# iden3/circom-witnesscalc

Measured on AMD Instinct MI355X. Metric: witnesses/sec, higher is better.
Workload: dtype u32

## Files before the change

circom-witnesscalc_amd/__init__.py:

```python
import ctypes
import os
import subprocess

import numpy as np

_HERE = os.path.dirname(os.path.abspath(__file__))
LIB_PATH = os.environ.get("CWC_LIB_PATH") or os.path.join(_HERE, "libcircom_witnesscalc_amd.so")
_lib = None


class GwStatus(ctypes.Structure):
    _fields_ = [("code", ctypes.c_int), ("error_msg", ctypes.c_void_p)]


class GraphInfo(ctypes.Structure):
    _fields_ = [(n, ctypes.c_uint64) for n in ("n_nodes", "n_op", "n_input_nodes", "n_const", "n_inputs",
                                                "n_witness", "depth", "algorithmic_bytes_per_set")]


class Timing(ctypes.Structure):
    _fields_ = [("tile_width", ctypes.c_uint32), ("n_launches", ctypes.c_uint32), ("n_bundles", ctypes.c_uint64),
                ("n_slots", ctypes.c_uint64), ("interp_ms", ctypes.c_float), ("pack_ms", ctypes.c_float),
                ("divider", ctypes.c_uint32), ("streams", ctypes.c_uint32)]


class ProgramStats(ctypes.Structure):
    _fields_ = [("tile_width", ctypes.c_uint32), ("divider", ctypes.c_uint32), ("streams", ctypes.c_uint32), ("n_classes", ctypes.c_uint32),
                ("n_bundles", ctypes.c_uint64), ("n_fused_nodes", ctypes.c_uint64), ("class_bundles", ctypes.c_uint64 * 16),
                ("class_nodes", ctypes.c_uint64 * 16), ("model_wave_cycles", ctypes.c_double), ("lanes_active_mean", ctypes.c_double),
                ("values_per_bundle_mean", ctypes.c_double), ("chain_floor_cycles", ctypes.c_double), ("n_scan_steps", ctypes.c_uint64), ("n_conv_products", ctypes.c_uint64)]


CLASS_NAMES = ["INPUT", "MUL", "LIN", "DIV", "CMPZ", "CMPS", "BIT", "IDIVMOD", "TERN", "DIVREQ", "DIVGET", "MULQ", "SYNC", "MULF", "SCAN"]


class E2eStats(ctypes.Structure):
    _fields_ = [("n_sets", ctypes.c_size_t), ("sub_batch", ctypes.c_size_t), ("parse_threads", ctypes.c_uint32), ("write_threads", ctypes.c_uint32),
                ("parse_seconds", ctypes.c_double), ("wait_for_drain_seconds", ctypes.c_double), ("total_seconds", ctypes.c_double),
                ("witness_bytes", ctypes.c_uint64), ("failed_sets", ctypes.c_uint64)]


class Handoff(ctypes.Structure):
    _fields_ = [("struct_size", ctypes.c_uint32), ("form", ctypes.c_uint32), ("hip_stream", ctypes.c_void_p), ("done_event", ctypes.c_void_p)]


FORM_CANONICAL, FORM_MONTGOMERY = 0, 1


class WitnessCalcError(RuntimeError):
    pass


def pinned_rows(shape):
    import weakref
    n = int(np.prod(shape))
    ptr = lib().gwb_host_alloc(n)
    if not ptr:
        raise WitnessCalcError("gwb_host_alloc(%d) failed" % n)
    buf = (ctypes.c_uint8 * max(n, 1)).from_address(ptr)
    weakref.finalize(buf, lib().gwb_host_free, ptr)
    return np.frombuffer(buf, dtype=np.uint8, count=n).reshape(shape)


EXPORTED_SYMBOLS = [
    "gw_calc_witness", "gwb_graph_load", "gwb_graph_free", "gwb_graph_info", "gwb_graph_serialize",
    "gwb_inputs_from_json", "gwb_set_tile_width", "gwb_calc_witness_batch_device", "gwb_calc_witness_batch_host",
    "gwb_last_timing", "gwb_wtns_size", "gwb_wtns_from_witness", "gwb_graph_export", "gwb_graph_import",
    "gwb_free_status", "gwb_profile_classes", "gwb_pick_tile_width", "gwb_inputs_from_json_batch", "gwb_wtns_save_batch",
    "gwb_host_alloc", "gwb_host_free", "gwb_timing_history", "gwb_calc_witness_batch_handoff", "gwb_ubench_modmul", "gwb_graph_pick_tile_width", "gwb_graph_broadcast",
    "gwb_builder_new", "gwb_builder_free", "gwb_builder_input", "gwb_builder_constant", "gwb_builder_uno", "gwb_builder_duo", "gwb_builder_tres",
    "gwb_builder_witness", "gwb_builder_input_signal", "gwb_builder_node_count", "gwb_builder_finish",
    "gwb_ubench_modmul_block", "gwb_program_stats", "gwb_calc_witness_json_to_wtns", "gwb_model_class_cycles",
    "gwb_graphgen_bigint_class", "gwb_graphgen_rsa_long_div_class", "gwb_graph_op_histogram",
    "gwb_kernel_source_hash", "gwb_pack_schedule", "gwb_pack_schedule_of_blob", "gwb_rccl_unique_id", "gwb_rccl_comm_init", "gwb_rccl_comm_ranks", "gwb_rccl_comm_destroy",
    "gwb_wave_census",
]


def build(verbose=False, diag=False):
    cmd = ["make", "-C", os.path.join(_HERE, "csrc"), "-j4"] + (["all", "diag"] if diag else [])
    if not verbose:
        cmd.insert(1, "-s")
    subprocess.check_call(cmd)
    subprocess.check_call(["make"] + ([] if verbose else ["-s"]) + ["-C", os.path.join(_HERE, "r1cs"), "-j4"])


DIAG_LIB_PATH = os.path.join(_HERE, "libcircom_witnesscalc_amd_diag.so")


def lib():
    global _lib
    if _lib is None:
        if not os.path.exists(LIB_PATH):
            raise WitnessCalcError("HIP extension %s is missing: run __graft_entry__.build() "
                                   "(there is no CPU fallback)" % LIB_PATH)
        try:
            import torch
        except ImportError:
            pass
        L = ctypes.CDLL(LIB_PATH)
        vp, sz, u32p = ctypes.c_void_p, ctypes.c_size_t, ctypes.POINTER(ctypes.c_uint32)
        stp = ctypes.POINTER(GwStatus)
        L.gw_calc_witness.restype = ctypes.c_int
        L.gw_calc_witness.argtypes = [ctypes.c_char_p, vp, sz, ctypes.POINTER(vp), ctypes.POINTER(sz), stp]
        L.gwb_graph_load.restype = ctypes.c_int
        L.gwb_graph_load.argtypes = [vp, sz, ctypes.POINTER(vp), stp]
        L.gwb_graph_free.argtypes = [vp]
        L.gwb_graph_info.argtypes = [vp, ctypes.POINTER(GraphInfo)]
        L.gwb_graph_serialize.argtypes = [vp, ctypes.POINTER(vp), ctypes.POINTER(sz), stp]
        L.gwb_inputs_from_json.argtypes = [vp, ctypes.c_char_p, vp, stp]
        L.gwb_set_tile_width.argtypes = [vp, ctypes.c_uint32]
        L.gwb_calc_witness_batch_device.argtypes = [vp, vp, sz, vp, vp, vp, stp]
        L.gwb_calc_witness_batch_host.argtypes = [vp, vp, sz, vp, vp, stp]
        L.gwb_last_timing.argtypes = [vp, ctypes.POINTER(Timing)]
        L.gwb_host_alloc.restype = ctypes.c_void_p
        L.gwb_host_alloc.argtypes = [sz]
        L.gwb_host_free.restype = None
        L.gwb_host_free.argtypes = [ctypes.c_void_p]
        L.gwb_timing_history.restype = ctypes.c_int
        L.gwb_timing_history.argtypes = [ctypes.c_void_p, sz, ctypes.c_void_p, ctypes.c_void_p, ctypes.POINTER(sz)]
        L.gwb_wtns_size.restype = sz
        L.gwb_wtns_size.argtypes = [sz]
        L.gwb_wtns_from_witness.argtypes = [vp, sz, vp]
        L.gwb_graph_export.argtypes = [vp, ctypes.c_uint32, ctypes.POINTER(vp), ctypes.POINTER(sz), stp]
        L.gwb_graph_import.argtypes = [vp, sz, ctypes.POINTER(vp), stp]
        L.gwb_free_status.argtypes = [stp]
        if hasattr(L, "gwb_graphgen_bigint_class"):
            L.gwb_graphgen_bigint_class.argtypes = [ctypes.c_uint32, ctypes.c_uint32, ctypes.c_uint32, ctypes.POINTER(vp), ctypes.POINTER(sz), stp]
            L.gwb_graphgen_rsa_long_div_class.argtypes = [ctypes.c_uint32, ctypes.c_uint32, ctypes.c_uint32, ctypes.c_int, ctypes.POINTER(vp), ctypes.POINTER(sz), stp]
            L.gwb_graph_op_histogram.argtypes = [vp, ctypes.POINTER(ctypes.c_uint64), sz]
        L.gwb_profile_classes.argtypes = [vp, vp, sz, vp, vp, vp, stp]
        if hasattr(L, "gwb_wave_census"):
            L.gwb_wave_census.argtypes = [vp, vp, sz, vp, vp, vp, sz, stp]
        L.gwb_inputs_from_json_batch.argtypes = [vp, ctypes.c_char_p, sz, vp, sz, ctypes.POINTER(sz), stp]
        L.gwb_wtns_save_batch.argtypes = [vp, sz, sz, ctypes.c_char_p, stp]
        L.gwb_calc_witness_batch_handoff.argtypes = [vp, vp, sz, vp, vp, ctypes.POINTER(Handoff), stp]
        L.gwb_ubench_modmul.restype = ctypes.c_double
        L.gwb_ubench_modmul.argtypes = [ctypes.c_uint32, ctypes.c_uint32]
        L.gwb_ubench_modmul_block.restype = ctypes.c_double
        L.gwb_model_class_cycles.restype = ctypes.c_double
        L.gwb_kernel_source_hash.restype = ctypes.c_char_p
        L.gwb_kernel_source_hash.argtypes = []
        L.gwb_model_class_cycles.argtypes = [ctypes.c_uint32]
        L.gwb_ubench_modmul_block.argtypes = [ctypes.c_uint32, ctypes.c_uint32]
        L.gwb_program_stats.argtypes = [vp, ctypes.c_uint32, ctypes.POINTER(ProgramStats)]
        if hasattr(L, "gwb_pack_schedule"):
            L.gwb_pack_schedule.argtypes = [vp, ctypes.c_uint32, vp, sz, vp, sz, u32p, u32p, u32p, stp]
            L.gwb_pack_schedule_of_blob.argtypes = [vp, sz, vp, sz, vp, sz, u32p, u32p, u32p, stp]
        L.gwb_calc_witness_json_to_wtns.argtypes = [vp, ctypes.c_char_p, sz, ctypes.c_char_p, sz, ctypes.POINTER(sz), vp, sz, ctypes.POINTER(E2eStats), stp]
        L.gwb_graph_pick_tile_width.restype = ctypes.c_uint32
        L.gwb_graph_pick_tile_width.argtypes = [vp, sz]
        L.gwb_pick_tile_width.restype = ctypes.c_uint32
        L.gwb_pick_tile_width.argtypes = [sz]
        u32 = ctypes.c_uint32
        L.gwb_builder_new.restype = vp
        L.gwb_builder_new.argtypes = []
        L.gwb_builder_free.restype = None
        L.gwb_builder_free.argtypes = [vp]
        for name, args in (("input", [u32]), ("constant", [ctypes.c_char_p, sz]), ("uno", [u32, u32]), ("duo", [u32, u32, u32]), ("tres", [u32, u32, u32, u32])):
            f = getattr(L, "gwb_builder_" + name)
            f.restype = u32
            f.argtypes = [vp] + args
        L.gwb_builder_witness.argtypes = [vp, u32]
        L.gwb_builder_input_signal.argtypes = [vp, ctypes.c_char_p, u32, u32]
        L.gwb_builder_node_count.restype = ctypes.c_uint64
        L.gwb_builder_node_count.argtypes = [vp]
        L.gwb_builder_finish.argtypes = [vp, ctypes.POINTER(vp), ctypes.POINTER(sz), stp]
        _lib = L
    return _lib


_libc = ctypes.CDLL(None)
_libc.free.argtypes = [ctypes.c_void_p]


def _take_status(st):
    msg = ctypes.string_at(st.error_msg).decode("utf-8", "replace") if st.error_msg else ""
    lib().gwb_free_status(ctypes.byref(st))
    return msg


def _check(rc, st):
    msg = _take_status(st)
    if rc != 0:
        raise WitnessCalcError(msg or "call failed")


def wtns_save_batch(witness, path_pattern):
    witness = np.ascontiguousarray(witness, dtype=np.uint8)
    st = GwStatus()
    rc = lib().gwb_wtns_save_batch(witness.ctypes.data, witness.shape[1], witness.shape[0], path_pattern.encode(), ctypes.byref(st))
    _check(rc, st)


def ubench_modmul(waves_per_simd=4, iters=2000, block=False):
    if block:
        return float(lib().gwb_ubench_modmul_block(waves_per_simd, iters))
    return float(lib().gwb_ubench_modmul(waves_per_simd, iters))


def kernel_source_hash():
    return lib().gwb_kernel_source_hash().decode()


def model_cycles():
    return {n: float(lib().gwb_model_class_cycles(c)) for c, n in enumerate(CLASS_NAMES)}


def graphgen_native(kind, **kw):
    out, n, st = ctypes.c_void_p(), ctypes.c_size_t(), GwStatus()
    L = lib()
    if kind == "bigint":
        rc = L.gwb_graphgen_bigint_class(int(kw.get("k", 8)), int(kw.get("n_bits", 64)), int(kw.get("rounds", 4)), ctypes.byref(out), ctypes.byref(n), ctypes.byref(st))
    elif kind == "rsa":
        rc = L.gwb_graphgen_rsa_long_div_class(int(kw.get("n", 121)), int(kw.get("k", 17)), int(kw.get("muls", 2)), 1 if kw.get("range_checks", True) else 0,
                                               ctypes.byref(out), ctypes.byref(n), ctypes.byref(st))
    else:
        raise ValueError(kind)
    _check(rc, st)
    data = ctypes.string_at(out.value, n.value)
    _libc.free(out)
    return data


def pick_tile_width(batch):
    return int(lib().gwb_pick_tile_width(batch))


def calc_witness_wtns(inputs_json, graph_data):
    if isinstance(inputs_json, str):
        inputs_json = inputs_json.encode("utf-8")
    graph_data = bytes(graph_data)
    out, n, st = ctypes.c_void_p(), ctypes.c_size_t(), GwStatus()
    rc = lib().gw_calc_witness(inputs_json, graph_data, len(graph_data), ctypes.byref(out), ctypes.byref(n),
                               ctypes.byref(st))
    _check(rc, st)
    data = ctypes.string_at(out.value, n.value)
    _libc.free(out)
    return data


def calc_witness(inputs_json, graph_data):
    w = calc_witness_wtns(inputs_json, graph_data)
    body = w[76:]
    return [int.from_bytes(body[i:i + 32], "little") for i in range(0, len(body), 32)]


def wtns_from_witness(witness):
    if not isinstance(witness, np.ndarray):
        witness = np.frombuffer(b"".join(int(x).to_bytes(32, "little") for x in witness), dtype=np.uint8)
    witness = np.ascontiguousarray(witness, dtype=np.uint8).reshape(-1, 32)
    n = witness.shape[0]
    out = np.zeros(lib().gwb_wtns_size(n), dtype=np.uint8)
    if lib().gwb_wtns_from_witness(witness.ctypes.data, n, out.ctypes.data) != 0:
        raise WitnessCalcError("gwb_wtns_from_witness failed")
    return out.tobytes()


class Graph:

    def __init__(self, graph_data=None, _handle=None):
        self._h = ctypes.c_void_p()
        if _handle is not None:
            self._h = _handle
        else:
            graph_data = bytes(graph_data)
            st = GwStatus()
            rc = lib().gwb_graph_load(graph_data, len(graph_data), ctypes.byref(self._h), ctypes.byref(st))
            _check(rc, st)
        info = GraphInfo()
        lib().gwb_graph_info(self._h, ctypes.byref(info))
        for name, _ in GraphInfo._fields_:
            setattr(self, name, int(getattr(info, name)))

    def close(self):
        if getattr(self, "_h", None) and _lib is not None:
            _lib.gwb_graph_free(self._h)
            self._h = None

    __del__ = close

    @classmethod
    def from_blob(cls, blob):
        blob = bytes(blob)
        h, st = ctypes.c_void_p(), GwStatus()
        rc = lib().gwb_graph_import(blob, len(blob), ctypes.byref(h), ctypes.byref(st))
        _check(rc, st)
        return cls(_handle=h)

    def op_histogram(self):
        h = (ctypes.c_uint64 * 24)()
        if lib().gwb_graph_op_histogram(self._h, h, 24) != 0:
            raise WitnessCalcError("gwb_graph_op_histogram failed")
        names = ["Mul", "Div", "Add", "Sub", "Pow", "Idiv", "Mod", "Eq", "Neq", "Lt", "Gt", "Leq", "Geq", "Land", "Lor", "Shl", "Shr", "Bor", "Band", "Bxor",
                 "Neg", "TernCond", "Input", "Const"]
        return dict(sorted(((nm, int(h[i])) for i, nm in enumerate(names) if h[i]), key=lambda kv: -kv[1]))

    def export_blob(self, tile_width):
        out, n, st = ctypes.c_void_p(), ctypes.c_size_t(), GwStatus()
        rc = lib().gwb_graph_export(self._h, tile_width, ctypes.byref(out), ctypes.byref(n), ctypes.byref(st))
        _check(rc, st)
        data = ctypes.string_at(out.value, n.value)
        _libc.free(out)
        return data

    def serialize(self):
        out, n, st = ctypes.c_void_p(), ctypes.c_size_t(), GwStatus()
        rc = lib().gwb_graph_serialize(self._h, ctypes.byref(out), ctypes.byref(n), ctypes.byref(st))
        _check(rc, st)
        data = ctypes.string_at(out.value, n.value)
        _libc.free(out)
        return data

    def pick_tile_width(self, batch):
        key = int(lib().gwb_graph_pick_tile_width(self._h, batch))
        if key == 0:
            raise WitnessCalcError("gwb_graph_pick_tile_width failed")
        return key

    def set_tile_width(self, t):
        if lib().gwb_set_tile_width(self._h, t) != 0:
            raise WitnessCalcError("tile width must be 0 or a power of two in 1..64")

    def inputs_from_json(self, inputs_json):
        if isinstance(inputs_json, str):
            inputs_json = inputs_json.encode("utf-8")
        row = np.zeros((self.n_inputs, 32), dtype=np.uint8)
        st = GwStatus()
        rc = lib().gwb_inputs_from_json(self._h, inputs_json, row.ctypes.data, ctypes.byref(st))
        _check(rc, st)
        return row

    def inputs_from_json_batch(self, text):
        if isinstance(text, str):
            text = text.encode("utf-8")
        n = ctypes.c_size_t()
        st = GwStatus()
        lib().gwb_inputs_from_json_batch(self._h, text, len(text), None, 0, ctypes.byref(n), ctypes.byref(st))
        msg = _take_status(st)
        if "rows buffer too small" not in msg and msg:
            raise WitnessCalcError(msg)
        rows = np.zeros((n.value, self.n_inputs, 32), dtype=np.uint8)
        st = GwStatus()
        rc = lib().gwb_inputs_from_json_batch(self._h, text, len(text), rows.ctypes.data, n.value, ctypes.byref(n), ctypes.byref(st))
        _check(rc, st)
        return rows

    def json_to_wtns(self, text, path_pattern, first_index=0, with_status=True):
        if isinstance(text, str):
            text = text.encode("utf-8")
        n = ctypes.c_size_t()
        cap = max(1, text.count(b"\n") + 1, text.count(b"{"))
        status = np.zeros(cap, dtype=np.uint32)
        es, st = E2eStats(), GwStatus()
        rc = lib().gwb_calc_witness_json_to_wtns(self._h, text, len(text), path_pattern.encode(), first_index, ctypes.byref(n),
                                                  status.ctypes.data if with_status else None, cap if with_status else 0,
                                                  ctypes.byref(es), ctypes.byref(st))
        _check(rc, st)
        return status[:n.value], {k: getattr(es, k) for k, _ in E2eStats._fields_}

    def calc_witness_batch(self, inputs, out=None):
        inputs = np.ascontiguousarray(inputs, dtype=np.uint8)
        b = inputs.shape[0]
        assert inputs.shape[1:] == (self.n_inputs, 32), inputs.shape
        if out is None:
            wit = np.empty((b, self.n_witness, 32), dtype=np.uint8)
        else:
            wit = out
            assert wit.dtype == np.uint8 and wit.shape == (b, self.n_witness, 32) and wit.flags["C_CONTIGUOUS"]
        status = np.zeros(b, dtype=np.uint32)
        st = GwStatus()
        rc = lib().gwb_calc_witness_batch_host(self._h, inputs.ctypes.data, b, wit.ctypes.data, status.ctypes.data,
                                               ctypes.byref(st))
        _check(rc, st)
        return wit, status

    def calc_witness_batch_device(self, d_inputs, d_witness, d_status, stream=None, montgomery=False, done_event=None):
        import torch
        b = d_inputs.shape[0]
        assert d_inputs.is_cuda and d_witness.is_cuda and d_status.is_cuda
        assert d_inputs.is_contiguous() and d_witness.is_contiguous() and d_status.is_contiguous()
        assert tuple(d_inputs.shape[1:]) == (self.n_inputs, 32) and tuple(d_witness.shape) == (b, self.n_witness, 32)
        s = stream if stream is not None else torch.cuda.current_stream()
        st = GwStatus()
        if montgomery or done_event is not None:
            if done_event is not None:
                done_event.record(s)
            h = Handoff(ctypes.sizeof(Handoff), FORM_MONTGOMERY if montgomery else FORM_CANONICAL, s.cuda_stream,
                        done_event.cuda_event if done_event is not None else None)
            rc = lib().gwb_calc_witness_batch_handoff(self._h, d_inputs.data_ptr(), b, d_witness.data_ptr(), d_status.data_ptr(),
                                                      ctypes.byref(h), ctypes.byref(st))
        else:
            rc = lib().gwb_calc_witness_batch_device(self._h, d_inputs.data_ptr(), b, d_witness.data_ptr(),
                                                     d_status.data_ptr(), s.cuda_stream, ctypes.byref(st))
        _check(rc, st)

    def timing_history(self, max_launches):
        a = np.zeros(max_launches, dtype=np.float32)
        b = np.zeros(max_launches, dtype=np.float32)
        n = ctypes.c_size_t(0)
        if lib().gwb_timing_history(self._h, max_launches, a.ctypes.data, b.ctypes.data, ctypes.byref(n)) != 0:
            raise WitnessCalcError("gwb_timing_history failed")
        return a[:n.value], b[:n.value]

    def profile_classes(self, d_inputs, d_witness, d_status):
        out = np.zeros(96, dtype=np.uint64)
        st = GwStatus()
        rc = lib().gwb_profile_classes(self._h, d_inputs.data_ptr(), d_inputs.shape[0], d_witness.data_ptr(),
                                       d_status.data_ptr(), out.ctypes.data, ctypes.byref(st))
        _check(rc, st)
        names = ["INPUT", "MUL", "LIN", "DIV", "CMPZ", "CMPS", "BIT", "IDIVMOD", "TERN", "DIVREQ", "DIVGET", "MULQ"]
        res = {n: tuple(int(x) for x in out[4 * i:4 * i + 4]) for i, n in enumerate(names)}
        res["MULF"] = tuple(int(x) for x in out[64:68])
        res["SCAN"] = tuple(int(x) for x in out[68:72])
        res["_scan_kinds"] = {k: tuple(int(x) for x in out[72 + 4 * i:76 + 4 * i]) for i, k in enumerate(("carry", "division", "convolution", "borrow", "comparison"))}
        res["_sections"] = {"MUL": tuple(int(x) for x in out[48:54]), "LIN": tuple(int(x) for x in out[56:62])}
        res["_issue_part"] = {"MUL": int(out[92]), "LIN": int(out[93])}
        res["_pack"] = {"cycles": int(out[94]), "passes": int(out[95])}
        n = int(out[63])
        res["_waves"] = {"n": n, "max_cycles": int(out[54]), "min_cycles": (1 << 40) - int(out[55]) if n else 0,
                         "mean_cycles": int(out[62]) // n if n else 0}
        return res

    def wave_census(self, d_inputs, d_witness, d_status):
        out = np.zeros(3 * 8192, dtype=np.uint64)
        st = GwStatus()
        rc = lib().gwb_wave_census(self._h, d_inputs.data_ptr(), d_inputs.shape[0], d_witness.data_ptr(),
                                   d_status.data_ptr(), out.ctypes.data, out.size, ctypes.byref(st))
        _check(rc, st)
        rec = out.reshape(-1, 3)
        idx = [i for i in range(rec.shape[0]) if rec[i, 1]]
        res = []
        for i in idx:
            w0 = int(rec[i, 0])
            role, wpw = (w0 >> 40) & 255, (w0 >> 48) & 255
            res.append({"workgroup": i // wpw, "wave": i % wpw, "xcc": (w0 >> 32) & 15, "se": (w0 >> 13) & 7, "sh": (w0 >> 12) & 1, "cu": (w0 >> 8) & 15, "simd": (w0 >> 4) & 3,
                        "divider": role & 1, "stream": (role >> 1) & 7, "has_tile": (role >> 4) & 1, "start": int(rec[i, 1]), "end": int(rec[i, 2])})
        return res

    def program_stats(self, key=0):
        ps = ProgramStats()
        if lib().gwb_program_stats(self._h, key, ctypes.byref(ps)) != 0:
            raise WitnessCalcError("gwb_program_stats: no such program")
        n = ps.n_classes
        return {"tile_width": ps.tile_width, "divider": ps.divider, "streams": ps.streams, "n_bundles": ps.n_bundles,
                "n_fused_nodes": ps.n_fused_nodes, "n_scan_steps": ps.n_scan_steps, "n_conv_products": ps.n_conv_products, "chain_floor_cycles": ps.chain_floor_cycles, "model_wave_cycles": ps.model_wave_cycles, "lanes_active_mean": ps.lanes_active_mean, "values_per_bundle_mean": ps.values_per_bundle_mean,
                "class_bundles": {CLASS_NAMES[c]: int(ps.class_bundles[c]) for c in range(n) if ps.class_bundles[c]},
                "class_nodes": {CLASS_NAMES[c]: int(ps.class_nodes[c]) for c in range(n) if ps.class_nodes[c]}}

    def pack_schedule(self, key):
        return _pack_schedule(lambda *a: lib().gwb_pack_schedule(self._h, key, *a))

    def last_timing(self):
        t = Timing()
        if lib().gwb_last_timing(self._h, ctypes.byref(t)) != 0:
            raise WitnessCalcError("gwb_last_timing failed")
        return {n: getattr(t, n) for n, _ in Timing._fields_}


def _pack_schedule(call):
    nw, nr, ni, st = ctypes.c_uint32(), ctypes.c_uint32(), ctypes.c_uint32(), GwStatus()
    _check(call(None, 0, None, 0, ctypes.byref(nw), ctypes.byref(nr), ctypes.byref(ni), ctypes.byref(st)), st)
    order, ready = np.zeros(nw.value, dtype=np.uint32), np.zeros(nr.value, dtype=np.uint32)
    _check(call(order.ctypes.data, order.size, ready.ctypes.data, ready.size, ctypes.byref(nw), ctypes.byref(nr), ctypes.byref(ni), ctypes.byref(st)), st)
    return order, ready, int(ni.value)


def pack_schedule_of_blob(blob):
    blob = bytes(blob)
    return _pack_schedule(lambda *a: lib().gwb_pack_schedule_of_blob(blob, len(blob), *a))


R1CS_LIB_PATH = os.environ.get("CWC_R1CS_LIB_PATH") or os.path.join(_HERE, "libcwc_r1cs.so")
R1CS_SATISFIED = 0xFFFFFFFF
_r1cs_lib = None


class R1csInfo(ctypes.Structure):
    _fields_ = [(n, ctypes.c_uint32) for n in ("n_wires", "n_pub_out", "n_pub_in", "n_prv_in", "n_constraints")] + \
               [(n, ctypes.c_uint64) for n in ("n_labels", "n_factors_a", "n_factors_b", "n_factors_c")]


class R1csQapInfo(ctypes.Structure):
    _fields_ = [("n_rows", ctypes.c_uint64), ("domain_power", ctypes.c_uint32), ("domain_size", ctypes.c_uint64),
                ("workspace_bytes_per_row", ctypes.c_uint64)]


class ZkeyInfo(ctypes.Structure):
    _fields_ = [("n_vars", ctypes.c_uint32), ("n_public", ctypes.c_uint32), ("domain_size", ctypes.c_uint32), ("n_coefs", ctypes.c_uint64)]


class PtauInfo(ctypes.Structure):
    _fields_ = [("power", ctypes.c_uint32), ("ceremony_power", ctypes.c_uint32), ("prepared", ctypes.c_uint32),
                ("n_contributions", ctypes.c_uint32)]


def r1cs_lib():
    global _r1cs_lib
    if _r1cs_lib is None:
        if not os.path.exists(R1CS_LIB_PATH):
            raise WitnessCalcError("R1CS library %s is missing: run __graft_entry__.build()" % R1CS_LIB_PATH)
        try:
            import torch
        except ImportError:
            pass
        L = ctypes.CDLL(R1CS_LIB_PATH)
        vp, sz, u32 = ctypes.c_void_p, ctypes.c_size_t, ctypes.c_uint32
        stp = ctypes.POINTER(GwStatus)
        L.gwb_r1cs_load.argtypes = [vp, sz, ctypes.POINTER(vp), stp]
        L.gwb_r1cs_free.restype = None
        L.gwb_r1cs_free.argtypes = [vp]
        L.gwb_r1cs_info.argtypes = [vp, ctypes.POINTER(R1csInfo)]
        L.gwb_r1cs_set_tile_width.argtypes = [vp, u32]
        L.gwb_r1cs_check_batch_device.argtypes = [vp, vp, sz, sz, u32, vp, vp, vp, stp]
        L.gwb_r1cs_check_batch_host.argtypes = [vp, vp, sz, sz, vp, vp, stp]
        L.gwb_r1cs_check_wtns.argtypes = [vp, vp, sz, vp, vp, stp]
        L.gwb_r1cs_qap_info.argtypes = [vp, ctypes.POINTER(R1csQapInfo), stp]
        L.gwb_r1cs_qap_batch_device.argtypes = [vp, vp, sz, sz, u32, vp, u32, vp, stp]
        L.gwb_r1cs_qap_batch_host.argtypes = [vp, vp, sz, sz, vp, u32, stp]
        L.gwb_r1cs_qap_wtns.argtypes = [vp, vp, sz, vp, u32, stp]
        L.gwb_r1cs_qap_time_phases.argtypes = [vp, ctypes.c_int]
        L.gwb_r1cs_qap_phase_ms.argtypes = [vp, ctypes.POINTER(ctypes.c_float)]
        L.gwb_r1cs_modmul_rate.argtypes = [ctypes.POINTER(ctypes.c_double)]
        L.gwb_zkey_load.argtypes = [vp, sz, ctypes.POINTER(vp), stp]
        L.gwb_zkey_free.restype = None
        L.gwb_zkey_free.argtypes = [vp]
        L.gwb_zkey_info.argtypes = [vp, ctypes.POINTER(ZkeyInfo)]
        L.gwb_groth16_prove_batch_device.argtypes = [vp, vp, vp, sz, sz, u32, vp, vp, vp, stp]
        L.gwb_groth16_prove_batch_host.argtypes = [vp, vp, vp, sz, sz, vp, vp, stp]
        L.gwb_groth16_prove_wtns.argtypes = [vp, vp, vp, sz, vp, vp, stp]
        L.gwb_groth16_time_phases.argtypes = [vp, ctypes.c_int]
        L.gwb_groth16_phase_ms.argtypes = [vp, ctypes.POINTER(ctypes.c_float)]
        L.gwb_zkey_qap_info.argtypes = [vp, ctypes.POINTER(R1csQapInfo), stp]
        L.gwb_zkey_qap_batch_device.argtypes = [vp, vp, sz, sz, u32, vp, u32, vp, stp]
        L.gwb_zkey_qap_batch_host.argtypes = [vp, vp, sz, sz, vp, u32, stp]
        L.gwb_zkey_set_tile_width.argtypes = [vp, u32]
        L.gwb_zkey_check_r1cs.argtypes = [vp, vp, stp]
        L.gwb_g16vk_from_zkey.argtypes = [vp, ctypes.POINTER(vp), stp]
        L.gwb_g16vk_load.argtypes = [vp, sz, u32, ctypes.POINTER(vp), stp]
        L.gwb_g16vk_info.argtypes = [vp, ctypes.POINTER(ctypes.c_uint32)]
        L.gwb_g16vk_points.argtypes = [vp, vp, sz]
        L.gwb_g16vk_alphabeta.argtypes = [vp, vp, stp]
        L.gwb_g16vk_free.restype = None
        L.gwb_g16vk_free.argtypes = [vp]
        L.gwb_groth16_verify_batch_device.argtypes = [vp, vp, vp, sz, sz, vp, vp, stp]
        L.gwb_groth16_verify_batch_host.argtypes = [vp, vp, vp, sz, sz, vp, stp]
        L.gwb_bn254_pairing_batch_device.argtypes = [vp, vp, sz, vp, vp, stp]
        L.gwb_groth16_setup.argtypes = [vp, vp, ctypes.POINTER(vp), ctypes.POINTER(sz), stp]
        L.gwb_groth16_setup_free.restype = None
        L.gwb_groth16_setup_free.argtypes = [vp]
        L.gwb_bn254_gen_mul_batch_device.argtypes = [vp, sz, u32, vp, vp, stp]
        L.gwb_groth16_setup_phase_ms.argtypes = [ctypes.POINTER(ctypes.c_float)]
        L.gwb_ptau_info.argtypes = [vp, sz, ctypes.POINTER(PtauInfo), stp]
        L.gwb_ptau_check.argtypes = [vp, sz, u32, u32, stp]
        L.gwb_groth16_setup_ptau.argtypes = [vp, vp, sz, vp, u32, ctypes.POINTER(vp), ctypes.POINTER(sz), stp]
        L.gwb_bn254_point_idft_batch_device.argtypes = [vp, u32, u32, vp, vp, stp]
        L.gwb_groth16_setup_ptau_phase_ms.argtypes = [ctypes.POINTER(ctypes.c_float)]
        L.gwb_bn254_g2_check_batch_device.argtypes = [vp, sz, u32, u32, vp, vp, stp]
        L.gwb_zkey_check_g2.argtypes = [vp, stp]
        L.gwb_zkey_check_wtns.argtypes = [vp, vp, sz, stp]
        L.gwb_ptau_check_g2.argtypes = [vp, sz, u32, u32, stp]
        L.gwb_groth16_contribute.argtypes = [vp, sz, ctypes.c_char_p, vp, ctypes.POINTER(vp), ctypes.POINTER(sz), vp, stp]
        L.gwb_groth16_contribute_phase_ms.argtypes = [ctypes.POINTER(ctypes.c_float)]
        L.gwb_zkey_verify_contributions.argtypes = [vp, sz, vp, ctypes.POINTER(sz), stp]
        L.gwb_zkey_verify_step.argtypes = [vp, sz, vp, sz, vp, stp]
        L.gwb_zkey_contributions.argtypes = [vp, sz, ctypes.POINTER(vp), ctypes.POINTER(sz), stp]
        L.gwb_blake2b512.restype = None
        L.gwb_blake2b512.argtypes = [vp, sz, vp]
        L.gwb_zkey_contribution_challenge.restype = None
        L.gwb_zkey_contribution_challenge.argtypes = [vp, vp]
        L.gwb_bn254_g1_scale_batch_device.argtypes = [vp, sz, vp, vp, vp, stp]
        L.gwb_bn254_g1_lincomb128_device.argtypes = [vp, vp, sz, vp, vp, stp]
        _r1cs_lib = L
    return _r1cs_lib


def _r1cs_check(rc, st):
    msg = ctypes.string_at(st.error_msg).decode("utf-8", "replace") if st.error_msg else ""
    if st.error_msg:
        _libc.free(st.error_msg)
    if rc != 0:
        raise WitnessCalcError(msg or "call failed")


def modmul_rate():
    rate = ctypes.c_double()
    if r1cs_lib().gwb_r1cs_modmul_rate(ctypes.byref(rate)) != 0:
        raise WitnessCalcError("gwb_r1cs_modmul_rate failed")
    return rate.value


def _qap_info(h, src):
    info = R1csQapInfo()
    st = GwStatus()
    rc = getattr(r1cs_lib(), "gwb_%s_qap_info" % src)(h, ctypes.byref(info), ctypes.byref(st))
    _r1cs_check(rc, st)
    return {n: int(getattr(info, n)) for n, _ in R1csQapInfo._fields_}


def _qap_batch(h, src, witness_rows, montgomery_out):
    if isinstance(witness_rows, tuple):
        witness_rows = witness_rows[0]
    w = np.ascontiguousarray(witness_rows, dtype=np.uint8)
    assert w.ndim == 3 and w.shape[2] == 32, w.shape
    b = w.shape[0]
    out = np.zeros((b, _qap_info(h, src)["domain_size"], 32), dtype=np.uint8)
    st = GwStatus()
    rc = getattr(r1cs_lib(), "gwb_%s_qap_batch_host" % src)(h, w.ctypes.data, w.shape[1], b, out.ctypes.data,
                                                            FORM_MONTGOMERY if montgomery_out else FORM_CANONICAL, ctypes.byref(st))
    _r1cs_check(rc, st)
    return out


def _qap_batch_device(h, src, d_witness, stream, montgomery, montgomery_out):
    import torch
    assert d_witness.is_cuda and d_witness.is_contiguous() and d_witness.dtype == torch.uint8
    assert d_witness.dim() == 3 and d_witness.shape[2] == 32, tuple(d_witness.shape)
    b = d_witness.shape[0]
    n = _qap_info(h, src)["domain_size"]
    s = stream if stream is not None else torch.cuda.current_stream(d_witness.device)
    out = torch.empty((b, n, 32), dtype=torch.uint8, device=d_witness.device)
    st = GwStatus()
    with torch.cuda.device(d_witness.device):
        rc = getattr(r1cs_lib(), "gwb_%s_qap_batch_device" % src)(h, d_witness.data_ptr(), d_witness.shape[1], b,
                                                                  FORM_MONTGOMERY if montgomery else FORM_CANONICAL, out.data_ptr(),
                                                                  FORM_MONTGOMERY if montgomery_out else FORM_CANONICAL, s.cuda_stream,
                                                                  ctypes.byref(st))
    _r1cs_check(rc, st)
    if b:
        out.record_stream(s)
    return out


class R1cs:

    def __init__(self, data):
        self._h = ctypes.c_void_p()
        data = bytes(data)
        st = GwStatus()
        rc = r1cs_lib().gwb_r1cs_load(data, len(data), ctypes.byref(self._h), ctypes.byref(st))
        _r1cs_check(rc, st)
        info = R1csInfo()
        r1cs_lib().gwb_r1cs_info(self._h, ctypes.byref(info))
        self.info = {n: int(getattr(info, n)) for n, _ in R1csInfo._fields_}

    def close(self):
        if getattr(self, "_h", None) and _r1cs_lib is not None:
            _r1cs_lib.gwb_r1cs_free(self._h)
            self._h = None

    __del__ = close

    def set_tile_width(self, t):
        if r1cs_lib().gwb_r1cs_set_tile_width(self._h, t) != 0:
            raise WitnessCalcError("tile width must be 0 or a power of two in 1..64")

    def check_batch(self, witness_rows):
        if isinstance(witness_rows, tuple):
            witness_rows = witness_rows[0]
        w = np.ascontiguousarray(witness_rows, dtype=np.uint8)
        assert w.ndim == 3 and w.shape[2] == 32, w.shape
        b = w.shape[0]
        first = np.zeros(b, dtype=np.uint32)
        nfail = np.zeros(b, dtype=np.uint32)
        st = GwStatus()
        rc = r1cs_lib().gwb_r1cs_check_batch_host(self._h, w.ctypes.data, w.shape[1], b, first.ctypes.data, nfail.ctypes.data, ctypes.byref(st))
        _r1cs_check(rc, st)
        return first, nfail

    def check_batch_device(self, d_witness, stream=None, montgomery=False):
        import torch
        assert d_witness.is_cuda and d_witness.is_contiguous() and d_witness.dtype == torch.uint8
        assert d_witness.dim() == 3 and d_witness.shape[2] == 32, tuple(d_witness.shape)
        b = d_witness.shape[0]
        s = stream if stream is not None else torch.cuda.current_stream(d_witness.device)
        first = torch.empty(b, dtype=torch.int32, device=d_witness.device)
        nfail = torch.empty(b, dtype=torch.int32, device=d_witness.device)
        st = GwStatus()
        with torch.cuda.device(d_witness.device):
            rc = r1cs_lib().gwb_r1cs_check_batch_device(self._h, d_witness.data_ptr(), d_witness.shape[1], b,
                                                        FORM_MONTGOMERY if montgomery else FORM_CANONICAL, first.data_ptr(),
                                                        nfail.data_ptr(), s.cuda_stream, ctypes.byref(st))
        _r1cs_check(rc, st)
        return first, nfail

    def check_wtns(self, wtns):
        wtns = bytes(wtns)
        first, nfail = ctypes.c_uint32(), ctypes.c_uint32()
        st = GwStatus()
        rc = r1cs_lib().gwb_r1cs_check_wtns(self._h, wtns, len(wtns), ctypes.byref(first), ctypes.byref(nfail), ctypes.byref(st))
        _r1cs_check(rc, st)
        return int(first.value), int(nfail.value)

    def qap_info(self):
        return _qap_info(self._h, "r1cs")

    def qap_batch(self, witness_rows, montgomery_out=False):
        return _qap_batch(self._h, "r1cs", witness_rows, montgomery_out)

    def qap_batch_device(self, d_witness, stream=None, montgomery=False, montgomery_out=False):
        return _qap_batch_device(self._h, "r1cs", d_witness, stream, montgomery, montgomery_out)

    def qap_time_phases(self, on=True):
        if r1cs_lib().gwb_r1cs_qap_time_phases(self._h, 1 if on else 0) != 0:
            raise WitnessCalcError("gwb_r1cs_qap_time_phases failed")

    def qap_phase_ms(self):
        ms = (ctypes.c_float * 4)()
        if r1cs_lib().gwb_r1cs_qap_phase_ms(self._h, ms) != 0:
            raise WitnessCalcError("no QAP phase times (qap_time_phases not on, or no QAP call yet)")
        return dict(zip(("evaluation", "inverse_outer", "fused_inner", "forward_outer"), (float(x) for x in ms)))

    def qap_wtns(self, wtns, montgomery_out=False):
        wtns = bytes(wtns)
        h = np.zeros((self.qap_info()["domain_size"], 32), dtype=np.uint8)
        st = GwStatus()
        rc = r1cs_lib().gwb_r1cs_qap_wtns(self._h, wtns, len(wtns), h.ctypes.data,
                                          FORM_MONTGOMERY if montgomery_out else FORM_CANONICAL, ctypes.byref(st))
        _r1cs_check(rc, st)
        return h



GROTH16_PROOF_BYTES = 256
GROTH16_PHASES = ("witness_map", "scalars_sort", "g1_msms", "g2_msm", "assembly")


def _rs_array(rs, b):
    if rs is None:
        return None
    if isinstance(rs, np.ndarray):
        a = np.ascontiguousarray(rs, dtype=np.uint8)
    else:
        a = np.frombuffer(b"".join(int(x).to_bytes(32, "little") for pair in rs for x in pair), dtype=np.uint8).copy()
    assert a.size == b * 64, "rs must hold [batch][2][32 B]"
    return a


def _dec(b):
    return str(int.from_bytes(bytes(b), "little"))


def proof_json(proof):
    p = bytes(proof)
    c = [_dec(p[32 * k:32 * k + 32]) for k in range(8)]
    z = lambda lo, hi: "1" if any(p[lo:hi]) else "0"
    return {"pi_a": [c[0], c[1], z(0, 64)], "pi_b": [[c[2], c[3]], [c[4], c[5]], [z(64, 192), "0"]],
            "pi_c": [c[6], c[7], z(192, 256)], "protocol": "groth16", "curve": "bn128"}


class Groth16:

    def __init__(self, zkey_bytes, r1cs=None, check_g2=False):
        self._h = ctypes.c_void_p()
# ... 596 lines not shown
```

circom-witnesscalc_amd/csrc/kernels.hip:

```cpp
#include <hip/hip_runtime.h>
#include <stdlib.h>

#include "fr_gfx950.hpp"
#include "scan_gfx950.hpp"
#include "program_dev.h"

namespace cwc {

__device__ __forceinline__ Fr fr_from_u4(const uint4& lo, const uint4& hi) {
    return Fr{{lo.x, lo.y, lo.z, lo.w, hi.x, hi.y, hi.z, hi.w}};
}

__device__ __forceinline__ bool wave_any(bool p) { return __ballot(p) != 0ull; }

struct InterpDims {
    uint32_t n_bundles, n_slots, n_inputs, batch, n_const, n_div_requests, trash_off;
    const uint32_t* div_lanes;
    uint32_t n_streams, stream_first[MAX_STREAMS], stream_count[MAX_STREAMS], stream_div_requests[MAX_STREAMS], stream_cref_first[MAX_STREAMS];
    uint4* pack_out;
    const uint2* pack_entries;
    const uint32_t* pack_ready;
    uint32_t n_inline, pack_mont, n_witness;
};
static const uint32_t ST_DIVIDER_TIMEOUT = 0x80000000u;
static const uint32_t ST_SYNC_TIMEOUT = 0x40000000u;

__device__ __forceinline__ bool mbox_wait(const volatile uint32_t* seq, uint32_t need) {
    for (uint32_t spins = 0; spins < (1u << 22); ++spins) {
        if (*seq >= need) return true;
        __builtin_amdgcn_s_sleep(8);
    }
    return false;
}
__device__ __noinline__ bool post_wait(uint32_t* word, uint32_t need) {
#pragma nounroll
    for (uint32_t spins = 0; spins < (1u << 22); ++spins) {
        if (__hip_atomic_load(word, __ATOMIC_ACQUIRE, __HIP_MEMORY_SCOPE_AGENT) >= need) return true;
        __builtin_amdgcn_s_sleep(8);
    }
    return false;
}
typedef uint32_t u32x4 __attribute__((ext_vector_type(4)));
typedef int i32x4 __attribute__((ext_vector_type(4)));
typedef __attribute__((address_space(3))) char lds_char;

__device__ __forceinline__ void dma16(uint32_t lds_addr, uint32_t voff, const i32x4& rsrc, uint32_t soff) {
    asm volatile("s_mov_b32 m0, %0\n\ts_nop 0\n\tbuffer_load_dwordx4 %1, %2, %3 offen lds"
                 :: "s"(lds_addr), "v"(voff), "s"(rsrc), "s"(soff) : "memory");
}
__device__ __forceinline__ i32x4 make_rsrc_words(const void* base, uint32_t bytes) {
    const uint64_t a = (uint64_t)base;
    return i32x4{(int)(uint32_t)a, (int)((uint32_t)(a >> 32) & 0xffffu), (int)bytes, 0x00020000};
}

template <int T, bool PROF, int W, int PACK, int MODE = 0>
__global__ __launch_bounds__((W > 0 ? (W + 1) * PACK : PACK) * 64) void interp_kernel(const uint32_t* __restrict__ hdr, const uint4* __restrict__ recs,
                                                    const uint32_t* __restrict__ crefs, InterpDims p, WsTable wst,
                                                    const uint4* __restrict__ inputs, uint32_t* __restrict__ status,
                                                    unsigned long long* __restrict__ prof) {
    constexpr int G = 64 / T;
    constexpr bool M2 = MODE == 2 || MODE == 3, WIDE = MODE == 3;
    constexpr uint32_t HI = 16u * T;
    constexpr bool DIVIDER = W > 0;
    constexpr uint32_t NW = (W > 0 ? (uint32_t)W : 1u) * (uint32_t)PACK;
    constexpr uint32_t WD = W > 0 ? (uint32_t)W : 1u;
    constexpr uint32_t AREA = lds_area_bytes((uint32_t)W, LDS_BYTES);
    constexpr uint32_t ML = mbox_lanes((uint32_t)W), MB = mbox_bytes((uint32_t)W);
    const uint32_t batch = p.batch;
    const uint32_t lane = threadIdx.x & 63u;
    const uint32_t wave = (uint32_t)__builtin_amdgcn_readfirstlane((int)(threadIdx.x >> 6));
    const uint32_t n_tiles = (batch + T - 1) / T;
    const uint32_t t = lane % T;
    const uint32_t j = (G == 1) ? 0u : lane / T;
    const uint32_t NS = p.n_streams;
    const uint32_t stream = wave < NW ? wave % NS : 0u;
    const uint32_t tile_raw = blockIdx.x * (NW / NS) + (wave < NW ? wave : 0u) / NS;
    const uint32_t tile = tile_raw < n_tiles ? tile_raw : n_tiles - 1;
    const uint32_t set = tile * T + t;
    const uint32_t set_c = set < batch ? set : batch - 1;
    [[maybe_unused]] auto census_slot = [&]() -> unsigned long long* {
        const uint32_t wv = blockIdx.x * (blockDim.x >> 6) + wave;
        return lane == 0 && wv < CENSUS_MAX_WAVES ? prof + PROF_WORDS + CENSUS_WORDS * wv : nullptr;
    };
    if constexpr (PROF) {
        if (unsigned long long* c = census_slot()) {
            const uint32_t w_of = wave < NW ? wave : (wave - NW) * WD;
            const uint32_t has_tile = blockIdx.x * (NW / NS) + w_of / NS < n_tiles ? 1u : 0u;
            const unsigned long long role = (wave >= NW ? 1u : 0u) | (w_of % NS) << 1 | has_tile << 4 | (blockDim.x >> 6) << 8;
            constexpr int HWREG_HW_ID = 4 | 31 << 11, HWREG_XCC_ID = 20 | 31 << 11;
            c[0] = (unsigned long long)__builtin_amdgcn_s_getreg(HWREG_HW_ID) | (unsigned long long)(__builtin_amdgcn_s_getreg(HWREG_XCC_ID) & 15u) << 32 | role << 40;
            c[1] = __builtin_amdgcn_s_memtime();
        }
    }
    const uint64_t tile_bytes = ws_tile_bytes(p.n_const, p.n_slots, T);
    const uint32_t chunk = tile / wst.tiles_per_chunk, tile_in_chunk = tile % wst.tiles_per_chunk;
    char* tile_base = reinterpret_cast<char*>(wst.base[chunk]) + (uint64_t)tile_in_chunk * tile_bytes;
    const __amdgpu_buffer_rsrc_t rsrc = __builtin_amdgcn_make_buffer_rsrc(tile_base, 0, (int)(uint32_t)tile_bytes, 0x00020000);
    const i32x4 rsrc_rec = make_rsrc_words(recs, (p.n_bundles + REC_AHEAD) * (uint32_t)G * 16u);
    uint32_t* const sync_words = reinterpret_cast<uint32_t*>(tile_base + ws_sync_offset(p.n_const, p.n_slots, T));
    static_assert(NW + PACK <= 16, "sequence words: 64 bytes");
    __shared__ uint4 lds[(NW * AREA + (DIVIDER ? NW * MB + 64u : 0u)) / 16];
    const uint32_t area = wave * AREA;
    const uint32_t lds0 = (uint32_t)(uintptr_t)(lds_char*)(char*)lds + area;
    const uint32_t t16 = 16u * t, lane16 = 16u * lane, j16 = 16u * j;
    char* const ldsb = reinterpret_cast<char*>(lds) + area;
    char* const mbox_all = reinterpret_cast<char*>(lds) + NW * AREA;
    char* const mbox = mbox_all + (wave < NW ? wave : 0u) * MB;
    volatile uint32_t* const seq = reinterpret_cast<volatile uint32_t*>(mbox_all + NW * MB);
    if (DIVIDER || NW > 1) {
        if (DIVIDER && threadIdx.x < NW + (uint32_t)PACK) seq[threadIdx.x] = 0;
        if (NS > 1 && wave < NW && stream == 0 && lane < MAX_STREAMS && tile_raw < n_tiles) {
            __hip_atomic_store(sync_words + lane, 0u, __ATOMIC_RELAXED, __HIP_MEMORY_SCOPE_AGENT);
            __builtin_amdgcn_fence(__ATOMIC_RELEASE, "agent");
        }
        if (wave < NW && stream == 0 && j == 0 && tile_raw < n_tiles && set < batch) status[set] = 0;
        __syncthreads();
    } else {
        if (j == 0 && tile_raw < n_tiles && set < batch) status[set] = 0;
    }
    if (DIVIDER) {
        if (wave >= NW) {
            const uint32_t first_w = (wave - NW) * WD, first_tile = blockIdx.x * (NW / NS) + first_w / NS;
            if (first_tile >= n_tiles) return;
            const uint32_t n_active = NS > 1 ? 1u : n_tiles - first_tile < WD ? n_tiles - first_tile : WD;
            char* const mbox_d = mbox_all + first_w * MB;
            const uint32_t n_requests = NS > 1 ? p.stream_div_requests[first_w % NS] : p.n_div_requests;
            uint32_t div_lanes_base = 0;
            for (uint32_t q = 0; NS > 1 && q < first_w % NS; ++q) div_lanes_base += p.stream_div_requests[q];
            [[maybe_unused]] uint32_t pk_next = 0;
            [[maybe_unused]] uint2 pk_e0 = make_uint2(0u, 0u), pk_e1 = pk_e0;
            [[maybe_unused]] unsigned long long pk_cycles = 0, pk_passes = 0;
            const bool inl = W == 1 && NS == 1 && p.n_inline > 0;
            const char* const pk_tile = reinterpret_cast<const char*>(wst.base[first_tile / wst.tiles_per_chunk]) + (uint64_t)(first_tile % wst.tiles_per_chunk) * tile_bytes;
            const uint32_t pk_set = first_tile * T + t;
            auto pk_load = [&](const uint2& e, uint4& lo, uint4& hi) {
                const uint32_t ref = e.y & ~REF_CANON;
                const uint32_t slot = (ref & REF_CONST) ? (ref & ~REF_CONST) : p.n_const + ref;
                const uint4* q = reinterpret_cast<const uint4*>(pk_tile) + (size_t)slot * (2 * T);
                lo = q[t];
                hi = q[T + t];
            };
            auto pk_store = [&](const uint2& e, const uint4& lo, const uint4& hi, uint32_t limit) {
                const bool valid = pk_next + j < limit && pk_set < batch, canon = (e.y & REF_CANON) != 0;
                const Fr v = fr_from_u4(lo, hi);
                Fr c = v;
                if (p.pack_mont) {
                    if (wave_any(both(valid, canon))) c = u256_select(canon, fr_mul(v, fr_r2()), v);
                } else {
                    if (wave_any(both(valid, !canon))) c = u256_select(canon, v, fr_from_mont(v));
                }
                if (valid) {
                    uint4* o = p.pack_out + ((size_t)pk_set * p.n_witness + e.x) * 2;
                    o[0] = make_uint4(c.v[0], c.v[1], c.v[2], c.v[3]);
                    o[1] = make_uint4(c.v[4], c.v[5], c.v[6], c.v[7]);
                }
            };
            auto pk_run = [&](uint32_t limit, uint32_t need) {
                if (pk_next >= limit) return;
                unsigned long long t0 = 0;
                if (PROF) t0 = __builtin_amdgcn_s_memtime();
                uint4 lo, hi;
                pk_load(pk_e0, lo, hi);
                for (;;) {
                    const uint32_t nb = pk_next + (uint32_t)G;
                    const bool more = nb < limit && seq[first_w] < need;
                    uint4 lo1 = lo, hi1 = hi;
                    if (more) pk_load(pk_e1, lo1, hi1);
                    const uint2 e2 = p.pack_entries[nb + (uint32_t)G + j];
                    pk_store(pk_e0, lo, hi, limit);
                    pk_next = nb;
                    pk_e0 = pk_e1;
                    pk_e1 = e2;
                    if (PROF) ++pk_passes;
                    if (!more) break;
                    lo = lo1;
                    hi = hi1;
                }
                if (PROF) pk_cycles += __builtin_amdgcn_s_memtime() - t0;
            };
            if constexpr (W == 1) {
                if (inl) {
                    pk_e0 = p.pack_entries[j];
                    pk_e1 = p.pack_entries[(uint32_t)G + j];
                }
            }
            for (uint32_t k = 0; k < n_requests; ++k) {
                if constexpr (W == 1) {
                    if (inl) {
                        const uint32_t lim = p.pack_ready[k] < p.n_inline ? p.pack_ready[k] : p.n_inline;
                        pk_run(lim / (uint32_t)G * (uint32_t)G, k + 1);
                    }
                }
                bool ok = true;
                for (uint32_t w = 0; w < n_active; ++w) ok = ok && mbox_wait(seq + first_w + w, k + 1);
                if (!ok) {
                    if (first_tile * T + t < batch) atomicOr(&status[first_tile * T + t], ST_DIVIDER_TIMEOUT);
                    break;
                }
                __builtin_amdgcn_fence(__ATOMIC_ACQUIRE, "workgroup");
                const uint32_t lanes_k = p.div_lanes[div_lanes_base + k];
                const uint32_t total = n_active * lanes_k;
                for (uint32_t g0 = 0; g0 < total; g0 += 64u) {
                    const uint32_t g = g0 + lane;
                    const bool valid = g < total;
                    const uint32_t w = valid ? g / lanes_k : 0u, i = valid ? g % lanes_k : 0u;
                    char* mb = mbox_d + w * MB + 16u * i;
                    const uint4* qa = reinterpret_cast<const uint4*>(mb);
                    const uint4* qb = reinterpret_cast<const uint4*>(mb + 32u * ML);
                    Fr a = fr_from_u4(qa[0], qa[ML]), b = fr_from_u4(qb[0], qb[ML]);
                    if (!valid) b = fr_zero();
                    const Fr inv = fr_inv(b);
                    const Fr r = u256_select(u256_is_zero(b), fr_zero(), fr_mul(a, inv));
                    if (valid) {
                        uint4* qr = reinterpret_cast<uint4*>(mb);
                        qr[0] = make_uint4(r.v[0], r.v[1], r.v[2], r.v[3]);
                        qr[ML] = make_uint4(r.v[4], r.v[5], r.v[6], r.v[7]);
                    }
                }
                __builtin_amdgcn_fence(__ATOMIC_RELEASE, "workgroup");
                if (lane == 0) seq[wave] = k + 1;
            }
            if constexpr (W == 1) {
                if (inl) {
                    pk_run(p.pack_ready[n_requests] < p.n_inline ? p.pack_ready[n_requests] : p.n_inline, 0xffffffffu);
                    if (PROF && lane == 0 && first_tile % 64u == 0) {
                        atomicAdd(&prof[94], pk_cycles);
                        atomicAdd(&prof[95], pk_passes);
                    }
                }
            }
            if constexpr (PROF) {
                if (unsigned long long* c = census_slot()) c[2] = __builtin_amdgcn_s_memtime();
            }
            return;
        }
    }
    if (tile_raw >= n_tiles) return;
    uint32_t div_seq = 0;
    uint32_t n_posts = 0, n_waits = 0;
    uint32_t cref_row = p.stream_cref_first[stream];

    auto ld = [&](uint32_t off) -> Fr {
        const u32x4 lo = __builtin_amdgcn_raw_buffer_load_b128(rsrc, (int)off, 0, 0);
        const u32x4 hi = __builtin_amdgcn_raw_buffer_load_b128(rsrc, (int)off + (int)HI, 0, 0);
        return Fr{{lo.x, lo.y, lo.z, lo.w, hi.x, hi.y, hi.z, hi.w}};
    };
    auto ld_lds = [&](uint32_t addr) -> Fr {
        const uint4* q = reinterpret_cast<const uint4*>(ldsb + addr);
        const uint4 lo = q[0], hi = q[LDS_HALF_BYTES / 16];
        return fr_from_u4(lo, hi);
    };
    auto ld_rec2 = [&](uint32_t bundle, uint32_t half) -> uint2 {
        return *reinterpret_cast<const uint2*>(ldsb + LDS_REC_OFF + (bundle % REC_AHEAD) * REC_BYTES + lane16 + 8u * half);
    };
    const uint32_t B0 = p.stream_first[stream], NBND = B0 + p.stream_count[stream];
    if (NBND == B0) return;
    auto clampb = [&](uint32_t b) { return b < NBND ? b : NBND - 1; };
    auto stage_rec = [&](uint32_t bundle) {
        dma16(lds0 + LDS_REC_OFF + (bundle % REC_AHEAD) * REC_BYTES, j16, rsrc_rec, bundle * (uint32_t)G * 16u);
    };
    constexpr uint32_t DMA_BIAS = 3u * LDS_HALF_BYTES;
    const i32x4 rsrc_dma = make_rsrc_words(tile_base - DMA_BIAS, (uint32_t)tile_bytes + DMA_BIAS);
    const uint32_t dma_soff0 = DMA_BIAS, dma_soff1 = DMA_BIAS + HI - LDS_HALF_BYTES, dma_soff2 = DMA_BIAS - 2u * LDS_HALF_BYTES,
                   dma_soff3 = DMA_BIAS + HI - 3u * LDS_HALF_BYTES;
    static_assert(LDS_HALF_BYTES == 1024, "instruction offsets below are written out");
    auto stage_operands = [&](uint32_t bundle, const uint2& offs) {
        const uint32_t s = lds0 + LDS_STAGE_OFF + (bundle % OPND_AHEAD) * STAGE_BYTES;
        const uint32_t ao = offs.x + t16, bo = offs.y + t16;
        asm volatile("s_mov_b32 m0, %0\n\ts_nop 0\n\t"
                     "buffer_load_dwordx4 %1, %3, %4 offen lds\n\t"
                     "buffer_load_dwordx4 %1, %3, %5 offen offset:1024 lds\n\t"
                     "buffer_load_dwordx4 %2, %3, %6 offen offset:2048 lds\n\t"
                     "buffer_load_dwordx4 %2, %3, %7 offen offset:3072 lds"
                     :: "s"(s), "v"(ao), "v"(bo), "s"(rsrc_dma), "s"(dma_soff0), "s"(dma_soff1), "s"(dma_soff2), "s"(dma_soff3) : "memory");
    };
    uint32_t err_bits = 0;
    Fr pv = fr_p();
#pragma unroll
    for (int i = 0; i < 8; ++i) asm volatile("" : "+v"(pv.v[i]));
    constexpr bool COOP = (uint32_t)T <= COOP_MAX_T;
    const uint32_t cq = lane & 3u, cv = lane >> 2;
    const uint32_t t16c = 16u * (cv % T);
    const uint32_t coop_chunk = (cq >> 1) * LDS_HALF_BYTES + (cq & 1u) * 8u;
    const uint32_t coop_ring_off = 16u * cv + coop_chunk;
    const uint32_t coop_dst_off = t16c + (cq >> 1) * HI + (cq & 1u) * 8u;
    uint32_t nq0 = cq == 0 ? CWC_P0 : cq == 1 ? CWC_P2 : cq == 2 ? CWC_P4 : CWC_P6;
    uint32_t nq1 = cq == 0 ? CWC_P1 : cq == 1 ? CWC_P3 : cq == 2 ? CWC_P5 : CWC_P7;
    asm volatile("" : "+v"(nq0), "+v"(nq1));
    const uint32_t trash_doff = p.trash_off | t16;
    constexpr int C_PROF = 12;
    unsigned long long pf[C_PROF][2], psec[2][7] = {{0, 0, 0, 0, 0, 0, 0}, {0, 0, 0, 0, 0, 0, 0}};
    unsigned long long pf_fused[2] = {0, 0};
    unsigned long long pf_scan[5][2] = {{0, 0}, {0, 0}, {0, 0}, {0, 0}, {0, 0}};
    if (PROF) {
#pragma unroll
        for (int c = 0; c < C_PROF; ++c) pf[c][0] = pf[c][1] = 0;
    }
#define CWC_STAMP(var) unsigned long long var = 0; if (PROF) asm volatile("s_memtime %0\n\ts_waitcnt lgkmcnt(0)" : "=s"(var)::"memory")
#define CWC_SHADOW_ISSUE()                                                                                                                  \
    stage_rec(b + 4);                                                                                                                       \
    __builtin_amdgcn_raw_buffer_store_b128(u32x4{r_prev.v[0], r_prev.v[1], r_prev.v[2], r_prev.v[3]}, rsrc, (int)doff_prev, 0, 0);          \
    __builtin_amdgcn_raw_buffer_store_b128(u32x4{r_prev.v[4], r_prev.v[5], r_prev.v[6], r_prev.v[7]}, rsrc, (int)doff_prev + (int)HI, 0, 0)
#define CWC_NEXT_HEADER(var)                                                                                                                 \
    asm volatile("s_mov_b32 %0, xnack_mask_lo\n\ts_load_dword xnack_mask_lo, %1, %2" : "=&s"(var) : "s"(hdr), "s"(hdr_off_n2) : "memory"); \
    hdr_off_n2 += 4u

    static_assert(OPND_AHEAD == 2 && REC_AHEAD == 4, "the counted waits below are written for this pipeline depth");
#pragma unroll
    for (uint32_t q = 0; q < REC_AHEAD; ++q) stage_rec(B0 + q);
    asm volatile("s_waitcnt vmcnt(0)" ::: "memory");
    stage_operands(B0, ld_rec2(B0, 0));
    stage_operands(B0 + 1, ld_rec2(B0 + 1, 0));
    uint2 rec_hi = ld_rec2(B0, 1);
    uint2 rec_hi_n1 = ld_rec2(B0 + 1, 1);
    uint32_t h_cur = hdr[B0], h_n1 = hdr[clampb(B0 + 1)];
    asm volatile("s_waitcnt vmcnt(0)" ::: "memory");
    const unsigned long long t_wave0 = PROF ? __builtin_amdgcn_s_memtime() : 0ull;
    asm volatile("s_load_dword xnack_mask_lo, %0, %1\n\ts_waitcnt lgkmcnt(0)" :: "s"(hdr), "s"(4u * B0 + 8u) : "memory");
    uint32_t hdr_off_n2 = 4u * B0 + 12u;
    Fr r_prev = fr_zero();
    uint32_t doff_prev = trash_doff;
    for (uint32_t b = B0; b < NBND; ++b) {
        CWC_STAMP(st0);
        const uint32_t h = h_cur;
        asm volatile("s_waitcnt vmcnt(7)" ::: "memory");
        CWC_STAMP(st1);
        if constexpr (COOP) {
            uint32_t cls_q = h & HDR_CLASS_MASK;
            asm volatile("" : "+s"(cls_q));
            static_assert(C_MULQ == 11 && C_SYNC == 12 && C_MULF == 13 && C_SCAN == 14 && C_COUNT == 15, "one compare (class >= C_MULQ) leads to the narrow classes");
            const bool narrow_cls = MODE == 1 ? cls_q >= C_MULQ : cls_q == C_MULQ;
            if (M2 ? __builtin_expect(narrow_cls, 0) : narrow_cls) {
            if (MODE != 1 || cls_q == C_MULQ) {
                const uint32_t la = rec_hi.y + (t16c | (t16c << 16));
                const Fr a_op = ld_lds(la & 0xffffu);
                const uint2 bq = *reinterpret_cast<const uint2*>(ldsb + (la >> 16) + coop_chunk);
                const uint2 aq = *reinterpret_cast<const uint2*>(ldsb + (la & 0xffffu) + coop_chunk);
                const uint4 rec_full_n2 = *reinterpret_cast<const uint4*>(ldsb + LDS_REC_OFF + ((b + 2) % REC_AHEAD) * REC_BYTES + lane16);
                const uint2 rec_n2 = make_uint2(rec_full_n2.x, rec_full_n2.y), rec_hi_n2 = make_uint2(rec_full_n2.z, rec_full_n2.w);
                CWC_SHADOW_ISSUE();
                asm volatile("s_waitcnt lgkmcnt(0)" :: "v"(a_op.v[0]), "v"(a_op.v[4]), "v"(bq.x), "v"(aq.x), "v"(rec_n2.x), "v"(rec_hi_n2.x) : "memory");
                uint32_t h_n2;
                CWC_NEXT_HEADER(h_n2);
                CWC_STAMP(st2);
                stage_operands(b + 2, rec_n2);
                CWC_STAMP(st3);
                uint32_t out[2];
                if (h & (HDR_LIN_ADD | HDR_LIN_SUB)) {
                    fr_mul_coop4r(a_op, aq.x, aq.y, bq.x, bq.y, nq0, nq1, rec_hi.x & CTRL_SUB_MASK, out);
                } else {
                    fr_mul_coop4(a_op, bq.x, bq.y, nq0, nq1, out);
                }
                CWC_STAMP(st4);
                *reinterpret_cast<uint2*>(ldsb + LDS_RING_OFF + (b % RING_BUNDLES) * RING_SLOT_BYTES + coop_ring_off) = make_uint2(out[0], out[1]);
                {
                    typedef uint32_t u32x2 __attribute__((ext_vector_type(2)));
                    __builtin_amdgcn_raw_buffer_store_b64(u32x2{out[0], out[1]}, rsrc, (int)((rec_hi.x & ~CTRL_MASK) + coop_dst_off), 0, 0);
                }
                doff_prev = trash_doff;
                rec_hi = rec_hi_n1;
                rec_hi_n1 = rec_hi_n2;
                h_cur = h_n1;
                h_n1 = h_n2;
                __builtin_amdgcn_fence(__ATOMIC_ACQ_REL, "wavefront");
                if (PROF) {
                    asm volatile("s_waitcnt lgkmcnt(0)" ::: "memory");
                    const unsigned long long t_now = __builtin_amdgcn_s_memtime();
                    pf[C_MULQ][0] += t_now - st0;
                    pf[C_MULQ][1] += 1;
                    (void)st2; (void)st3; (void)st4;
                }
                continue;
            }
            if constexpr (MODE == 1 && (uint32_t)T <= COOP_FUSE_MAX_T) {
            if (cls_q == C_MULF) {
                constexpr int QP_MAIN = T == 1 ? 0xA0  : 0x00 , QP_EXTRA = T == 1 ? 0xF5  : 0xAA ;
                const uint32_t mx = (uint32_t)__builtin_amdgcn_mov_dpp((int)rec_hi.x, QP_MAIN, 0xf, 0xf, false);
                const uint32_t my = (uint32_t)__builtin_amdgcn_mov_dpp((int)rec_hi.y, QP_MAIN, 0xf, 0xf, false);
                const uint32_t xx = (uint32_t)__builtin_amdgcn_mov_dpp((int)rec_hi.x, QP_EXTRA, 0xf, 0xf, false);
                const uint32_t xy = (uint32_t)__builtin_amdgcn_mov_dpp((int)rec_hi.y, QP_EXTRA, 0xf, 0xf, false);
                const uint32_t la = my + (t16c | (t16c << 16)), lx = xy + (t16c | (t16c << 16));
                const Fr a_op = ld_lds(la & 0xffffu);
                const uint2 bq = *reinterpret_cast<const uint2*>(ldsb + (la >> 16) + coop_chunk);
                const Fr x2_full = ld_lds(lx & 0xffffu);
                const uint2 x2q = *reinterpret_cast<const uint2*>(ldsb + (lx & 0xffffu) + coop_chunk);
                const uint2 x3q = *reinterpret_cast<const uint2*>(ldsb + (lx >> 16) + coop_chunk);
                const uint4 rec_full_n2 = *reinterpret_cast<const uint4*>(ldsb + LDS_REC_OFF + ((b + 2) % REC_AHEAD) * REC_BYTES + lane16);
                const uint2 rec_n2 = make_uint2(rec_full_n2.x, rec_full_n2.y), rec_hi_n2 = make_uint2(rec_full_n2.z, rec_full_n2.w);
                CWC_SHADOW_ISSUE();
                asm volatile("s_waitcnt lgkmcnt(0)" :: "v"(a_op.v[0]), "v"(a_op.v[4]), "v"(bq.x), "v"(x2_full.v[0]), "v"(x2_full.v[4]), "v"(x2q.x), "v"(x3q.x), "v"(rec_n2.x), "v"(rec_hi_n2.x) : "memory");
                uint32_t h_n2;
                CWC_NEXT_HEADER(h_n2);
                stage_operands(b + 2, rec_n2);
                uint32_t out[2];
                fr_mul_coop4(a_op, bq.x, bq.y, nq0, nq1, out);
                const uint32_t op2 = mx & CTRL_SUB_MASK, op3 = xx & CTRL_SUB_MASK;
                if (h & HDR_F_S2MUL) {
                    uint32_t o2[2];
                    fr_mul_coop4(x2_full, out[0], out[1], nq0, nq1, o2);
                    out[0] = op2 == FOP_MUL ? o2[0] : out[0];
                    out[1] = op2 == FOP_MUL ? o2[1] : out[1];
                }
                auto lin_stage = [&](uint32_t op, const uint2& xq) {
                    const bool rs = op == FOP_RSUB;
                    uint32_t o[2];
                    fr_addsub_coop4(rs ? xq.x : out[0], rs ? xq.y : out[1], rs ? out[0] : xq.x, rs ? out[1] : xq.y, nq0, nq1, op == FOP_ADD ? 0u : 1u, o);
                    out[0] = op >= FOP_ADD ? o[0] : out[0];
                    out[1] = op >= FOP_ADD ? o[1] : out[1];
                };
                if (h & HDR_F_S2LIN) lin_stage(op2, x2q);
                if (h & HDR_F_S3LIN) lin_stage(op3, x3q);
                *reinterpret_cast<uint2*>(ldsb + LDS_RING_OFF + (b % RING_BUNDLES) * RING_SLOT_BYTES + coop_ring_off) = make_uint2(out[0], out[1]);
                {
// ... 374 lines not shown
                        ds.v[0] |= dz ? 1u : 0u;
                        const bool small = !wave_any((x.v[2] | x.v[3] | x.v[4] | x.v[5] | x.v[6] | x.v[7] | acc0.v[2] | acc0.v[3] | acc0.v[4] | acc0.v[5] | acc0.v[6] | acc0.v[7] |
                                                      d.v[2] | d.v[3] | d.v[4] | d.v[5] | d.v[6] | d.v[7]) != 0u) && sh >= 1u && sh <= 64u;
                        Fr quo = fr_zero(), rem = fr_zero();
                        if (small) {
                            const uint64_t dv = ((uint64_t)ds.v[1] << 32) | ds.v[0];
                            const uint32_t s = clz64_nonzero(dv);
                            const uint64_t dn = dv << s, rv = recip64(dn);
                            const uint64_t xl = ((uint64_t)x.v[1] << 32) | x.v[0];
                            const uint64_t a0 = ((uint64_t)acc0.v[1] << 32) | acc0.v[0];
                            uint64_t r64 = 0, qh = 0, ql = 0;
                            const bool seg = start || !active;
                            const uint64_t d_prev = ((uint64_t)wave_shr_lanes<D>((uint32_t)(dv >> 32)) << 32) | wave_shr_lanes<D>((uint32_t)dv);
                            if (sh == 64u && iters > 2u && !wave_any(both(active, either(dz, start ? a0 >= dv : dv != d_prev)))) {
                                scan_div_parallel<T>(seg, lane, iters, active ? dv : 1ull, active ? xl : 0ull, active ? a0 : 0ull, ql, r64);
                            } else if (sh == 64u) {
                                const uint64_t xn = xl << s, xh = (xl >> 1) >> (63u - s);
                                for (uint32_t it = 0; it < iters; ++it) {
                                    const uint32_t s0 = wave_shr_lanes<D>((uint32_t)r64), s1 = wave_shr_lanes<D>((uint32_t)(r64 >> 32));
                                    const uint64_t in = start ? a0 : (((uint64_t)s1 << 32) | s0);
                                    uint64_t q_h = 0, q_l, rr;
                                    if (wave_any(in >= dv)) {
                                        u128_divrem_64_recip(in, xl, dv, s, dn, rv, true, q_h, q_l, rr);
                                    } else {
                                        uint64_t rn;
                                        div2by1((in << s) | xh, xn, dn, rv, q_l, rn);
                                        rr = rn >> s;
                                    }
                                    qh = dz ? 0ull : q_h;
                                    ql = dz ? 0ull : q_l;
                                    r64 = dz ? 0ull : rr;
                                }
                            } else {
                                for (uint32_t it = 0; it < iters; ++it) {
                                    const uint32_t s0 = wave_shr_lanes<D>((uint32_t)r64), s1 = wave_shr_lanes<D>((uint32_t)(r64 >> 32));
                                    const uint64_t in = start ? a0 : (((uint64_t)s1 << 32) | s0);
                                    const uint64_t lo = in << sh, hi = (in >> 1) >> (63u - sh);
                                    const uint64_t tl = lo + xl, th = hi + (tl < lo ? 1ull : 0ull);
                                    uint64_t q_h, q_l, rr;
                                    u128_divrem_64_recip(th, tl, dv, s, dn, rv, wave_any(th >= dv), q_h, q_l, rr);
                                    qh = dz ? 0ull : q_h;
                                    ql = dz ? 0ull : q_l;
                                    r64 = dz ? 0ull : rr;
                                }
                            }
                            quo.v[0] = (uint32_t)ql; quo.v[1] = (uint32_t)(ql >> 32); quo.v[2] = (uint32_t)qh; quo.v[3] = (uint32_t)(qh >> 32);
                            rem.v[0] = (uint32_t)r64; rem.v[1] = (uint32_t)(r64 >> 32);
                        } else {
                            for (uint32_t it = 0; it < iters; ++it) {
                                Fr in;
#pragma unroll
                                for (int k = 0; k < 8; ++k) {
                                    const uint32_t sft = wave_shr_lanes<D>(rem.v[k]);
                                    in.v[k] = start ? acc0.v[k] : sft;
                                }
                                const Fr t = fr_add_wave(fr_mul_wave(in, bm, pv), x, pv);
                                const uint32_t lx = u256_bitlen(t), ly = u256_bitlen(ds);
                                const uint32_t my_dig = lx >= ly ? (lx - ly + 32u) >> 5 : 0u;
                                uint32_t dig = 0;
#pragma unroll
                                for (uint32_t dd = 1; dd <= 8; ++dd) dig = wave_any(my_dig >= dd) ? dd : dig;
                                Fr q1, r1;
                                u256_divrem_digits(q1, r1, t, ds, dig, ly);
                                quo = u256_select(dz, fr_zero(), q1);
                                rem = u256_select(dz, fr_zero(), r1);
                            }
                        }
                        r = u256_select(role_acc, rem, quo);
                    }
                }
                finish(r);
                continue;
            }
        }
        switch (cls) {
            case C_INPUT: {
                const uint32_t idx = crefs[(size_t)cref_row * G + j];
                ++cref_row;
                const uint4* q = inputs + ((size_t)set_c * p.n_inputs + idx) * 2;
                r = fr_mul_wave(fr_from_u4(q[0], q[1]), (h & HDR_OUT_CANON) ? fr_one() : fr_r2(), pv);
                break;
            }
            case C_DIVREQ: {
                if (DIVIDER) {
                    if (lane < ML) {
                        uint4* qa = reinterpret_cast<uint4*>(mbox + lane16);
                        uint4* qb = reinterpret_cast<uint4*>(mbox + 32u * ML + lane16);
                        qa[0] = make_uint4(a_op.v[0], a_op.v[1], a_op.v[2], a_op.v[3]);
                        qa[ML] = make_uint4(a_op.v[4], a_op.v[5], a_op.v[6], a_op.v[7]);
                        qb[0] = make_uint4(b_op.v[0], b_op.v[1], b_op.v[2], b_op.v[3]);
                        qb[ML] = make_uint4(b_op.v[4], b_op.v[5], b_op.v[6], b_op.v[7]);
                    }
                    __builtin_amdgcn_fence(__ATOMIC_RELEASE, "workgroup");
                    if (lane == 0) seq[wave] = div_seq + 1;
                }
                r = fr_zero();
                break;
            }
            case C_DIVGET: {
                r = fr_zero();
                if (DIVIDER) {
                    ++div_seq;
                    if (!mbox_wait(seq + NW + wave / WD, div_seq)) err_bits |= ST_DIVIDER_TIMEOUT;
                    __builtin_amdgcn_fence(__ATOMIC_ACQUIRE, "workgroup");
                    if (lane < ML) {
                        const uint4* qr = reinterpret_cast<const uint4*>(mbox + lane16);
                        r = fr_from_u4(qr[0], qr[ML]);
                    }
                }
                break;
            }
            case C_DIV: {
                const Fr inv = fr_inv(b_op);
                r = u256_select(u256_is_zero(b_op), fr_zero(), fr_mul(a_op, inv));
                break;
            }
            case C_CMPZ: {
                const bool az = u256_is_zero(a_op), cz = u256_is_zero(b_op), eq = u256_eq(a_op, b_op);
                const bool v = either(either(both(sub == SUB_EQ, eq), both(sub == SUB_NEQ, !eq)), either(both(sub == SUB_LAND, !either(az, cz)), both(both(sub != SUB_EQ, both(sub != SUB_NEQ, sub != SUB_LAND)), !both(az, cz))));
                r = u256_select(v, one_out(), fr_zero());
                break;
            }
            case C_CMPS: {
                const Fr x = (h & HDR_A_CANON) ? a_op : fr_from_mont(a_op), y = (h & HDR_B_CANON) ? b_op : fr_from_mont(b_op);
                auto less = [](const Fr& a, const Fr& b) {
                    Fr t;
                    const uint32_t borrow = u256_sub(t, a, b);
                    if constexpr (M2) asm volatile("" ::"v"(t.v[7]));
                    return borrow != 0;
                };
                bool lt, gt;
                bool limb_sized = false;
                if constexpr (M2) limb_sized = !wave_any(both(active, (x.v[4] | x.v[5] | x.v[6] | x.v[7] | y.v[4] | y.v[5] | y.v[6] | y.v[7]) != 0u));
                if (M2 && limb_sized) {
                    uint32_t d[4], bw = 0;
#pragma unroll
                    for (int k = 0; k < 4; ++k) d[k] = sbb32(x.v[k], y.v[k], bw);
                    lt = bw != 0u;
                    gt = both(bw == 0u, (d[0] | d[1] | d[2] | d[3]) != 0u);
                } else {
                    const bool xn = less(fr_half(), x), yn = less(fr_half(), y);
                    const bool same = xn == yn, xy = less(x, y), yx = less(y, x);
                    lt = same ? xy : xn;
                    gt = same ? yx : yn;
                }
                const bool v = either(either(both(sub == SUB_LT, lt), both(sub == SUB_GT, gt)), either(both(sub == SUB_LEQ, !gt), both(both(sub != SUB_LT, both(sub != SUB_GT, sub != SUB_LEQ)), !lt)));
                r = u256_select(v, one_out(), fr_zero());
                break;
            }
            case C_BIT: {
                const Fr x = (h & HDR_A_CANON) ? a_op : fr_from_mont(a_op);
                const uint32_t kx = rec_hi.y >> 20;
                const bool is_x = sub == SUB_BITX;
                if (h & HDR_BITX_ALL) {
                    const Fr e = u256_shr(x, kx);
                    r = u256_select((e.v[0] & 1u) != 0u, one_out(), fr_zero());
                    break;
                }
                const Fr y = (h & HDR_B_CANON) ? b_op : fr_from_mont(b_op);
                auto bit_result = [&](const Fr& d) -> Fr {
                    if (h & HDR_OUT_CANON) return d;
                    const bool small = both(d.v[0] < 2u, (d.v[1] | d.v[2] | d.v[3] | d.v[4] | d.v[5] | d.v[6] | d.v[7]) == 0u);
                    if (wave_any(!small)) return fr_mul_wave(d, fr_r2(), pv);
                    return u256_select(d.v[0] != 0u, fr_one(), fr_zero());
                };
                if (h & (HDR_BIT_ALL_SHR | HDR_BIT_ALL_BAND)) {
                    Fr d;
#pragma unroll
                    for (int i = 0; i < 8; ++i) d.v[i] = x.v[i] & y.v[i];
                    if (h & HDR_BIT_ALL_SHR) {
                        const bool big = either((y.v[1] | y.v[2] | y.v[3] | y.v[4] | y.v[5] | y.v[6] | y.v[7]) != 0u, y.v[0] >= 254u);
                        const Fr sh = u256_select(big, fr_zero(), u256_shr(x, big ? 0u : y.v[0]));
                        d = u256_select(sub == SUB_SHR, sh, d);
                    }
                    r = bit_result(d);
                    break;
                }
                uint32_t hi_or = 0;
#pragma unroll
                for (int i = 1; i < 8; ++i) hi_or |= y.v[i];
                const bool big = either(hi_or != 0u, y.v[0] >= 254u);
                const uint32_t n = is_x ? kx : big ? 0u : y.v[0];
                const bool shifts = either(either(sub == SUB_SHL, sub == SUB_SHR), is_x);
                Fr d = u256_shr(x, n);
                if (wave_any(sub == SUB_SHL)) d = u256_select(sub == SUB_SHL, u256_shl(x, n), d);
                d = u256_select(both(big, !is_x), fr_zero(), d);
                d.v[0] &= is_x ? 1u : 0xffffffffu;
#pragma unroll
                for (int i = 1; i < 8; ++i) d.v[i] = is_x ? 0u : d.v[i];
                {
                    const bool over = both(sub == SUB_SHL, !u256_lt(d, fr_p()));
                    err_bits |= both(over, active) ? ST_SHL_OVERFLOW : 0u;
                    d = u256_select(over, fr_zero(), d);
                }
                {
                    const uint32_t m_and = sub == SUB_BAND ? 0xffffffffu : 0u, m_or = sub == SUB_BAND ? 0u : 0xffffffffu, m_xor = (sub == SUB_BAND || sub == SUB_BOR) ? 0u : 0xffffffffu;
                    Fr e;
#pragma unroll
                    for (int i = 0; i < 8; ++i) {
                        const uint32_t a = x.v[i] & y.v[i], o = x.v[i] | y.v[i];
                        e.v[i] = (a & m_and) | ((o & m_or) & ~(a & m_xor));
                    }
                    Fr em;
                    const uint32_t br = u256_sub(em, e, fr_p());
                    err_bits |= both(both(br == 0u, u256_is_zero(em)), both(active, !shifts)) ? ST_BITOP_EQ_R : 0u;
                    e = u256_select(br == 0u, em, e);
                    d = u256_select(shifts, d, e);
                }
                r = bit_result(d);
                break;
            }
            case C_IDIVMOD: {
                const Fr x = (h & HDR_A_CANON) ? a_op : fr_from_mont(a_op), y = (h & HDR_B_CANON) ? b_op : fr_from_mont(b_op);
                const bool yz = u256_is_zero(y);
                Fr ys = y;
                ys.v[0] |= yz ? 1u : 0u;
                Fr q, rem;
                bool two_words = false;
                if constexpr (WIDE) two_words = !wave_any(both(both(active, !yz), either((ys.v[2] | ys.v[3]) == 0u, (ys.v[4] | ys.v[5] | ys.v[6] | ys.v[7]) != 0u)));
                if (!wave_any((x.v[4] | x.v[5] | x.v[6] | x.v[7] | ys.v[2] | ys.v[3] | ys.v[4] | ys.v[5] | ys.v[6] | ys.v[7]) != 0u)) {
                    u128_divrem_64(q, rem, x, ys);
                } else if (WIDE && two_words) {
                    const bool sub = either(yz, !active);
                    Fr yy = ys;
                    yy.v[0] = sub ? 0u : ys.v[0];
                    yy.v[1] = sub ? 0u : ys.v[1];
                    yy.v[2] = sub ? 1u : ys.v[2];
                    yy.v[3] = sub ? 0u : ys.v[3];
#pragma unroll
                    for (int k = 4; k < 8; ++k) yy.v[k] = 0u;
                    u256_divrem_128(q, rem, x, yy);
                } else {
                    const uint32_t lx = u256_bitlen(x), ly = u256_bitlen(ys);
                    const uint32_t my_dig = lx >= ly ? (lx - ly + 32u) >> 5 : 0u;
                    uint32_t dig = 0;
#pragma unroll
                    for (uint32_t dd = 1; dd <= 8; ++dd) dig = wave_any(my_dig >= dd) ? dd : dig;
                    u256_divrem_digits(q, rem, x, ys, dig, ly);
                }
                const Fr d = u256_select(yz, fr_zero(), u256_select(sub == SUB_IDIV, q, rem));
                r = (h & HDR_OUT_CANON) ? d : fr_mul_wave(d, fr_r2(), pv);
                break;
            }
            case C_TERN: {
                const uint32_t cr = crefs[(size_t)cref_row * G + j];
                ++cref_row;
                const Fr y = ld(cr + t16);
                r = u256_select(u256_is_zero(a_op), y, b_op);
                break;
            }
            case C_SYNC: {
                r = fr_zero();
                if (h & HDR_POST) {
                    asm volatile("s_waitcnt vmcnt(0)" ::: "memory");
                    ++n_posts;
                    if (lane == 0) __hip_atomic_store(sync_words + stream, n_posts, __ATOMIC_RELEASE, __HIP_MEMORY_SCOPE_AGENT);
                }
                if (h & HDR_WAIT) {
                    ++n_waits;
                    if (!post_wait(sync_words, n_waits)) err_bits |= ST_SYNC_TIMEOUT;
                }
                break;
            }
            case C_SCAN: r = fr_zero(); break;
            default: r = fr_zero(); break;
        }
        finish(r);
    }
    __builtin_amdgcn_raw_buffer_store_b128(u32x4{r_prev.v[0], r_prev.v[1], r_prev.v[2], r_prev.v[3]}, rsrc, (int)doff_prev, 0, 0);
    __builtin_amdgcn_raw_buffer_store_b128(u32x4{r_prev.v[4], r_prev.v[5], r_prev.v[6], r_prev.v[7]}, rsrc, (int)doff_prev + (int)HI, 0, 0);
    if (PROF && lane == 0) {
        const unsigned long long cyc = __builtin_amdgcn_s_memtime() - t_wave0;
        atomicMax(&prof[54], cyc);
        atomicMax(&prof[55], (1ull << 40) - cyc);
        atomicAdd(&prof[62], cyc);
        atomicAdd(&prof[63], 1ull);
    }
    if constexpr (PROF) {
        if (unsigned long long* c = census_slot()) c[2] = __builtin_amdgcn_s_memtime();
    }
    if (PROF && lane == 0 && (tile % 64u) == 0u) {
#pragma unroll
        for (int c = 0; c < C_PROF; ++c) {
            atomicAdd(&prof[c * 4 + 0], pf[c][0]);
            atomicAdd(&prof[c * 4 + 3], pf[c][1]);
        }
        atomicAdd(&prof[M2 ? 68 : 64], pf_fused[0]);
        atomicAdd(&prof[M2 ? 71 : 67], pf_fused[1]);
        if (M2) {
#pragma unroll
            for (int q = 0; q < 5; ++q) {
                atomicAdd(&prof[72 + 4 * q], pf_scan[q][0]);
                atomicAdd(&prof[75 + 4 * q], pf_scan[q][1]);
            }
        }
#pragma unroll
        for (int k = 0; k < 2; ++k)
#pragma unroll
            for (int q = 0; q < 6; ++q) atomicAdd(&prof[48 + 8 * k + q], psec[k][q]);
        atomicAdd(&prof[92], psec[0][6]);
        atomicAdd(&prof[93], psec[1][6]);
    }
    if (err_bits && set < batch) atomicOr(&status[set], err_bits);
}

__global__ __launch_bounds__(256) void fill_consts_kernel(ProgramDev p, WsTable wst, uint32_t n_tiles, uint32_t T) {
    const uint32_t e = blockIdx.x * 256u + threadIdx.x;
    const uint32_t pieces = p.n_const * 2u * T;
    if (e >= pieces) return;
    const uint4 v = reinterpret_cast<const uint4*>(p.consts)[(size_t)(e / (2u * T)) * 2u + (e / T) % 2u];
    const uint64_t tile_bytes = ws_tile_bytes(p.n_const, p.n_slots, T);
    for (uint32_t tile = blockIdx.y; tile < n_tiles; tile += gridDim.y) {
        char* tb = reinterpret_cast<char*>(wst.base[tile / wst.tiles_per_chunk]) + (uint64_t)(tile % wst.tiles_per_chunk) * tile_bytes;
        reinterpret_cast<uint4*>(tb)[e] = v;
    }
}

template <bool MONT>
__device__ __forceinline__ Fr pack_form(const Fr& v, bool canon) {
    if (MONT) return canon ? fr_mul(v, fr_r2()) : v;
    return canon ? v : fr_from_mont(v);
}

template <bool MONT, int TT>
__global__ __launch_bounds__(256) void pack_kernel(ProgramDev p, WsTable wst, uint4* __restrict__ out, uint32_t batch, uint32_t T_, uint32_t first) {
    const uint32_t T = TT ? (uint32_t)TT : T_;
    const uint32_t wi = first + blockIdx.x * 256u + threadIdx.x;
    if (wi >= p.n_witness) return;
    const uint32_t w = first ? p.pack_order[wi] : wi;
    const uint32_t ref_raw = p.witness_refs[w];
    const bool canon = (ref_raw & REF_CANON) != 0;
    const uint32_t ref = ref_raw & ~REF_CANON;
    const uint32_t n_tiles = (batch + T - 1) / T;
    const uint64_t tile_bytes = ws_tile_bytes(p.n_const, p.n_slots, T);
    const uint32_t slot = (ref & REF_CONST) ? (ref & ~REF_CONST) : p.n_const + ref;
    for (uint32_t tile = blockIdx.y; tile < n_tiles; tile += gridDim.y) {
        const char* tb = reinterpret_cast<const char*>(wst.base[tile / wst.tiles_per_chunk]) + (uint64_t)(tile % wst.tiles_per_chunk) * tile_bytes;
        const uint4* q = reinterpret_cast<const uint4*>(tb) + (size_t)slot * (2 * T);
        if (TT != 0 && TT <= 4) {
            uint4 lo[TT ? TT : 1], hi[TT ? TT : 1];
#pragma unroll
            for (int t = 0; t < TT; ++t) {
                lo[t] = q[t];
                hi[t] = q[TT + t];
            }
#pragma unroll
            for (int t = 0; t < TT; ++t) {
                const uint32_t set = tile * TT + t;
                if (set >= batch) break;
                const Fr c = pack_form<MONT>(fr_from_u4(lo[t], hi[t]), canon);
                uint4* o = out + ((size_t)set * p.n_witness + w) * 2;
                o[0] = make_uint4(c.v[0], c.v[1], c.v[2], c.v[3]);
                o[1] = make_uint4(c.v[4], c.v[5], c.v[6], c.v[7]);
            }
        } else {
            for (uint32_t t = 0; t < T; ++t) {
                const uint32_t set = tile * T + t;
                if (set >= batch) break;
                const Fr c = pack_form<MONT>(fr_from_u4(q[t], q[T + t]), canon);
                uint4* o = out + ((size_t)set * p.n_witness + w) * 2;
                o[0] = make_uint4(c.v[0], c.v[1], c.v[2], c.v[3]);
                o[1] = make_uint4(c.v[4], c.v[5], c.v[6], c.v[7]);
            }
        }
    }
}

template <bool MONT, int TT>
__global__ __launch_bounds__(256) void pack_kernel_v3(ProgramDev p, WsTable wst, uint4* __restrict__ out, uint32_t batch, uint32_t first) {
    constexpr uint32_t T = TT, WPB = 256u / T;
    const uint32_t t = threadIdx.x % T, wi = first + blockIdx.x * WPB + threadIdx.x / T;
    if (wi >= p.n_witness) return;
    const uint32_t w = first ? p.pack_order[wi] : wi;
    const uint32_t ref_raw = p.witness_refs[w];
    const bool canon = (ref_raw & REF_CANON) != 0;
    const uint32_t ref = ref_raw & ~REF_CANON;
    const uint32_t n_tiles = (batch + T - 1) / T;
    const uint64_t tile_bytes = ws_tile_bytes(p.n_const, p.n_slots, T);
    const uint32_t slot = (ref & REF_CONST) ? (ref & ~REF_CONST) : p.n_const + ref;
    for (uint32_t tile = blockIdx.y; tile < n_tiles; tile += gridDim.y) {
        const uint32_t set = tile * T + t;
        if (set >= batch) continue;
        const char* tb = reinterpret_cast<const char*>(wst.base[tile / wst.tiles_per_chunk]) + (uint64_t)(tile % wst.tiles_per_chunk) * tile_bytes;
        const uint4* q = reinterpret_cast<const uint4*>(tb) + (size_t)slot * (2 * T);
        const Fr c = pack_form<MONT>(fr_from_u4(q[t], q[T + t]), canon);
        uint4* o = out + ((size_t)set * p.n_witness + w) * 2;
        o[0] = make_uint4(c.v[0], c.v[1], c.v[2], c.v[3]);
        o[1] = make_uint4(c.v[4], c.v[5], c.v[6], c.v[7]);
    }
}

template <bool MONT>
__global__ __launch_bounds__(256) void pack_kernel_v1(ProgramDev p, WsTable wst, uint4* __restrict__ out, uint32_t batch, uint32_t T, uint32_t first) {
    const uint32_t wi = first + blockIdx.x * 64u + threadIdx.x;
    if (wi >= p.n_witness) return;
    const uint32_t w = first ? p.pack_order[wi] : wi;
    const uint32_t ref_raw = p.witness_refs[w];
    const bool canon = (ref_raw & REF_CANON) != 0;
    const uint32_t ref = ref_raw & ~REF_CANON;
    const uint32_t n_tiles = (batch + T - 1) / T;
    const uint64_t tile_bytes = ws_tile_bytes(p.n_const, p.n_slots, T);
    const uint32_t slot = (ref & REF_CONST) ? (ref & ~REF_CONST) : p.n_const + ref;
    for (uint32_t tile = blockIdx.y; tile < n_tiles; tile += gridDim.y) {
        const char* tb = reinterpret_cast<const char*>(wst.base[tile / wst.tiles_per_chunk]) + (uint64_t)(tile % wst.tiles_per_chunk) * tile_bytes;
        const uint4* q0 = reinterpret_cast<const uint4*>(tb) + (size_t)slot * (2 * T);
        for (uint32_t t = threadIdx.y; t < T; t += blockDim.y) {
            const uint32_t set = tile * T + t;
            if (set >= batch) break;
            const uint4* q = q0 + t;
            const Fr c = pack_form<MONT>(fr_from_u4(q[0], q[T]), canon);
            uint4* o = out + ((size_t)set * p.n_witness + w) * 2;
            o[0] = make_uint4(c.v[0], c.v[1], c.v[2], c.v[3]);
            o[1] = make_uint4(c.v[4], c.v[5], c.v[6], c.v[7]);
        }
    }
}

hipError_t launch_interp(uint32_t T, uint32_t W, uint32_t pack, uint32_t n_div_requests, const uint32_t* div_lanes, const ProgramDev& p,
                         const WsTable& wst, const void* inputs, uint32_t* status, uint32_t batch, hipStream_t stream, unsigned long long* prof,
                         void* out, uint32_t n_inline, bool montgomery) {
    const uint32_t tiles = (batch + T - 1) / T, nw = (W ? W : 1u) * pack, ns = p.n_streams ? p.n_streams : 1u;
    if (nw == 0 || nw % ns != 0 || (ns > 1 && W > 1)) return hipErrorInvalidValue;
    const uint32_t tiles_per_wg = nw / ns;
    dim3 grid((tiles + tiles_per_wg - 1) / tiles_per_wg), block((W ? (W + 1) * pack : pack) * 64);
    const uint4* in = (const uint4*)inputs;
    InterpDims dims{p.n_bundles, p.n_slots, p.n_inputs, batch, p.n_const, n_div_requests, p.trash_off, div_lanes, ns, {0, 0, 0, 0}, {0, 0, 0, 0}, {0, 0, 0, 0}, {0, 0, 0, 0},
                    (uint4*)out, reinterpret_cast<const uint2*>(p.pack_entries), p.pack_ready, 0u, montgomery ? 1u : 0u, p.n_witness};
    if (W == 1 && ns == 1 && out && p.pack_entries && p.pack_ready) dims.n_inline = n_inline < p.n_ready_last ? n_inline : p.n_ready_last;
    for (uint32_t s = 0; s < MAX_STREAMS; ++s) {
        dims.stream_first[s] = p.stream_first[s];
        dims.stream_count[s] = p.stream_count[s];
        dims.stream_div_requests[s] = p.stream_div_requests[s];
        dims.stream_cref_first[s] = p.stream_cref_first[s];
    }
    if (ns == 1) {
        dims.stream_first[0] = 0;
        dims.stream_count[0] = p.n_bundles;
        dims.stream_div_requests[0] = n_div_requests;
    }
    const uint4* recs = reinterpret_cast<const uint4*>(p.recs);
    const uint32_t mode = p.has_fused;
    static_assert(SCAN_MAX_T == COOP_FUSE_MAX_T, "the instances with a MODE are made for tile widths up to COOP_FUSE_MAX_T");
    if (mode > 3 || (mode && (T > COOP_FUSE_MAX_T || W > 1))) return hipErrorInvalidValue;
#define CWC_LAUNCH3(TT, PP, WW, KK)                                                                                                     \
    do {                                                                                                                                \
        if constexpr ((uint32_t)(TT) <= COOP_FUSE_MAX_T && (WW) <= 1) {                                                                 \
            if (mode == 3) interp_kernel<TT, PP, WW, KK, 3><<<grid, block, 0, stream>>>(p.hdr, recs, p.crefs, dims, wst, in, status, prof); \
            else if (mode == 2) interp_kernel<TT, PP, WW, KK, 2><<<grid, block, 0, stream>>>(p.hdr, recs, p.crefs, dims, wst, in, status, prof); \
            else if (mode == 1) interp_kernel<TT, PP, WW, KK, 1><<<grid, block, 0, stream>>>(p.hdr, recs, p.crefs, dims, wst, in, status, prof); \
            else interp_kernel<TT, PP, WW, KK, 0><<<grid, block, 0, stream>>>(p.hdr, recs, p.crefs, dims, wst, in, status, prof);     \
        } else {                                                                                                                        \
            interp_kernel<TT, PP, WW, KK, 0><<<grid, block, 0, stream>>>(p.hdr, recs, p.crefs, dims, wst, in, status, prof);          \
        }                                                                                                                               \
    } while (0)
#define CWC_LAUNCH2(TT, PP)                                  \
    if (W == 0 && pack == 1) CWC_LAUNCH3(TT, PP, 0, 1);      \
    else if (W == 0 && pack == 4) CWC_LAUNCH3(TT, PP, 0, 4); \
    else if (W == 1 && pack == 1) CWC_LAUNCH3(TT, PP, 1, 1); \
    else if (W == 1 && pack == 2) CWC_LAUNCH3(TT, PP, 1, 2); \
    else if (W == 1 && pack == 4) CWC_LAUNCH3(TT, PP, 1, 4); \
    else if (W == 3 && pack == 1) CWC_LAUNCH3(TT, PP, 3, 1); \
    else if (W == 4 && pack == 1) CWC_LAUNCH3(TT, PP, 4, 1); \
    else return hipErrorInvalidValue;
#ifdef CWC_DIAG
#define CWC_LAUNCH_PROF(TT, WW, KK) CWC_LAUNCH3(TT, true, WW, KK)
#define CWC_LAUNCH2_PROF(TT) CWC_LAUNCH2(TT, true)
#else
#define CWC_LAUNCH_PROF(TT, WW, KK) return hipErrorNotSupported
#define CWC_LAUNCH2_PROF(TT) return hipErrorNotSupported;
#endif
#define CWC_LAUNCH(TT)                                    \
    case TT:                                              \
        if (prof) { CWC_LAUNCH2_PROF(TT) } else { CWC_LAUNCH2(TT, false) } \
        break;
    switch (T) {
        CWC_LAUNCH(1) CWC_LAUNCH(2) CWC_LAUNCH(4) CWC_LAUNCH(8) CWC_LAUNCH(16) CWC_LAUNCH(32)
        case 64:
            if (W != 0) return hipErrorInvalidValue;
            if (pack == 4) { if (prof) { CWC_LAUNCH_PROF(64, 0, 4); } else CWC_LAUNCH3(64, false, 0, 4); }
            else if (pack == 1) { if (prof) { CWC_LAUNCH_PROF(64, 0, 1); } else CWC_LAUNCH3(64, false, 0, 1); }
            else return hipErrorInvalidValue;
            break;
        default: return hipErrorInvalidValue;
    }
#undef CWC_LAUNCH_PROF
#undef CWC_LAUNCH2_PROF
#undef CWC_LAUNCH
#undef CWC_LAUNCH2
#undef CWC_LAUNCH3
    return hipGetLastError();
}

#ifndef CWC_KSRC_HASH
#define CWC_KSRC_HASH "unstamped"
#endif
extern "C" const char* gwb_kernel_source_hash() { return CWC_KSRC_HASH; }
extern "C" int gwb_kernels_have_diagnostics() {
#ifdef CWC_DIAG
    return 1;
#else
    return 0;
#endif
}

__global__ void warm_kernel() {}
hipError_t launch_warm(hipStream_t stream) {
    warm_kernel<<<1, 64, 0, stream>>>();
    return hipGetLastError();
}

hipError_t launch_fill_consts(uint32_t T, const ProgramDev& p, const WsTable& wst, uint32_t n_tiles, hipStream_t stream) {
    if (n_tiles == 0 || p.n_const == 0) return hipSuccess;
    dim3 grid((p.n_const * 2u * T + 255u) / 256u, n_tiles < 16384u ? n_tiles : 16384u), block(256);
    fill_consts_kernel<<<grid, block, 0, stream>>>(p, wst, n_tiles, T);
    return hipGetLastError();
}

hipError_t launch_pack(uint32_t T, const ProgramDev& p, const WsTable& wst, void* out, uint32_t batch, hipStream_t stream, bool montgomery, uint32_t first) {
    if (p.n_witness == 0 || batch == 0 || first >= p.n_witness) return hipSuccess;
    const uint32_t count = p.n_witness - first;
    const uint32_t n_tiles = (batch + T - 1) / T;
    static const bool v1 = getenv("CWC_PACK_V1") != nullptr;
    if (v1 || T > 4) {
        dim3 grid((count + 63) / 64, n_tiles < 32768u ? n_tiles : 32768u), block(64, T < 4 ? T : 4);
        if (montgomery) pack_kernel_v1<true><<<grid, block, 0, stream>>>(p, wst, (uint4*)out, batch, T, first);
        else pack_kernel_v1<false><<<grid, block, 0, stream>>>(p, wst, (uint4*)out, batch, T, first);
        return hipGetLastError();
    }
    static const int pack_shape = getenv("CWC_PACK") ? atoi(getenv("CWC_PACK")) : 3;
    if (pack_shape == 3 && T >= 2) {
        dim3 grid3((count + 256 / T - 1) / (256 / T), n_tiles < 32768u ? n_tiles : 32768u), block3(256);
#define CWC_PACK3(MM, TT) pack_kernel_v3<MM, TT><<<grid3, block3, 0, stream>>>(p, wst, (uint4*)out, batch, first)
        if (montgomery) {
            if (T == 2) CWC_PACK3(true, 2); else CWC_PACK3(true, 4);
        } else {
            if (T == 2) CWC_PACK3(false, 2); else CWC_PACK3(false, 4);
        }
#undef CWC_PACK3
        return hipGetLastError();
    }
    dim3 grid((count + 255) / 256, n_tiles < 32768u ? n_tiles : 32768u), block(256);
#define CWC_PACK(MM, TT) pack_kernel<MM, TT><<<grid, block, 0, stream>>>(p, wst, (uint4*)out, batch, T, first)
    if (montgomery) {
        if (T == 1) CWC_PACK(true, 1); else if (T == 2) CWC_PACK(true, 2); else CWC_PACK(true, 4);
    } else {
        if (T == 1) CWC_PACK(false, 1); else if (T == 2) CWC_PACK(false, 2); else CWC_PACK(false, 4);
    }
#undef CWC_PACK
    return hipGetLastError();
}

__global__ __launch_bounds__(1024) void modmul_ubench_kernel(uint32_t* sink, uint32_t iters) {
    Fr a = fr_r2(), b = fr_one();
    a.v[0] ^= threadIdx.x + blockIdx.x * 977u;
    for (uint32_t it = 0; it < iters; ++it) {
        a = fr_mul(a, b);
        b = fr_mul(b, a);
    }
    if (a.v[0] == 0x1234567u && b.v[3] == 7u) sink[0] = a.v[1];
}
__global__ __launch_bounds__(512) void modmul_block_ubench_kernel(uint32_t* sink, uint32_t iters) {
    Fr a = fr_r2(), b = fr_one(), pv = fr_p();
#pragma unroll
    for (int i = 0; i < 8; ++i) asm volatile("" : "+v"(pv.v[i]));
    a.v[0] ^= threadIdx.x + blockIdx.x * 977u;
    for (uint32_t it = 0; it < iters; ++it) {
        a = fr_mul_wave(a, b, pv);
        b = fr_mul_wave(b, a, pv);
    }
    if (a.v[0] == 0x1234567u && b.v[3] == 7u) sink[0] = a.v[1];
}
hipError_t launch_modmul_ubench(uint32_t n_cus, uint32_t waves_per_simd, uint32_t iters, uint32_t* sink, hipStream_t stream, bool block_multiplier) {
    if (block_multiplier) {
        if (waves_per_simd > 2) return hipErrorInvalidValue;
        modmul_block_ubench_kernel<<<n_cus, 256 * waves_per_simd, 0, stream>>>(sink, iters);
    } else {
        modmul_ubench_kernel<<<n_cus, 256 * waves_per_simd, 0, stream>>>(sink, iters);
    }
    return hipGetLastError();
}

}
```

circom-witnesscalc_amd/csrc/pack_schedule.cc:

```cpp
#include "runtime_internal.hpp"

namespace cwcrt {

static const double kCyclesDividerServe = 52200, kCyclesPackPass = 2300;

std::string make_pack_schedule(const Program& p, PackSchedule& out) {
    const uint32_t nw = p.n_witness, G = p.G, nreq = p.n_div_requests;
    out.order.resize(nw);
    out.ready.assign((size_t)nreq + 1, 0u);
    out.n_inline = 0;
    for (uint32_t i = 0; i < nw; ++i) out.order[i] = i;
    if (p.divider != 1 || p.n_streams != 1 || nreq == 0 || nw == 0 || G == 0) return "";
    if (p.hdr.size() < p.n_bundles || p.recs.size() < (size_t)p.n_bundles * G * 4 || p.witness_refs.size() < nw) return "pack schedule: truncated program";
    const uint64_t slot_bytes = 32ull * p.T, first_off = (uint64_t)p.n_const * slot_bytes, end_off = ((uint64_t)p.n_const + p.n_slots) * slot_bytes;
    const uint32_t kNever = 0xffffffffu;
    std::vector<uint32_t> producer(p.n_slots, kNever), req_bundle;
    req_bundle.reserve(nreq);
    for (uint32_t b = 0; b < p.n_bundles; ++b) {
        if ((p.hdr[b] & HDR_CLASS_MASK) == C_DIVREQ) req_bundle.push_back(b);
        for (uint32_t i = 0; i < G; ++i) {
            const uint64_t dst = p.recs[((size_t)b * G + i) * 4 + 2] & ~CTRL_MASK;
            if (dst >= first_off && dst < end_off) producer[(dst - first_off) / slot_bytes] = b;
        }
    }
    if (req_bundle.size() != nreq) return "pack schedule: the program has " + std::to_string(req_bundle.size()) + " request bundles, its header says " + std::to_string(nreq);
    std::vector<uint32_t> at(nw);
    for (uint32_t w = 0; w < nw; ++w) {
        const uint32_t ref = p.witness_refs[w];
        if (ref & REF_CONST) {
            at[w] = 0;
            continue;
        }
        const uint32_t slot = ref & ~REF_CANON;
        if (slot >= p.n_slots || producer[slot] == kNever) return "pack schedule: witness " + std::to_string(w) + " names a slot that no bundle writes";
        const uint32_t k = (uint32_t)(std::upper_bound(req_bundle.begin(), req_bundle.end(), producer[slot]) - req_bundle.begin());
        at[w] = k + 2;
    }
    std::stable_sort(out.order.begin(), out.order.end(), [&](uint32_t a, uint32_t b) { return at[a] < at[b]; });
    for (uint32_t w = 0; w < nw; ++w)
        if (at[w] <= nreq) out.ready[at[w]]++;
    for (uint32_t k = 1; k <= nreq; ++k) out.ready[k] += out.ready[k - 1];
    double pass_cycles = kCyclesPackPass;
    if (const char* e = getenv("CWC_PACK_PASS_CYCLES")) pass_cycles = std::max(1.0, atof(e));
    double clock = 0, div_free = 0, served = 0;
    uint32_t next = 0, k = 0;
    for (uint32_t b = 0; b < p.n_bundles && k <= nreq; ++b) {
        const uint32_t cls = p.hdr[b] & HDR_CLASS_MASK;
        clock += model_class_cycles((int)cls);
        if (cls == C_DIVREQ) {
            const uint32_t limit = std::min(out.ready[k], nw) / G * G;
            const double gap = clock - div_free;
            if (gap > 0 && limit > next) next += (uint32_t)std::min<double>(std::floor(gap / pass_cycles) * G, limit - next);
            served = std::max(clock, div_free) + kCyclesDividerServe;
            div_free = served;
            ++k;
        } else if (cls == C_DIVGET) {
            clock = std::max(clock, served);
        }
    }
    out.n_inline = std::min(next, out.ready[nreq]);
    return "";
}

}

static int schedule_out(const Program& p, uint32_t* pack_order, size_t order_cap, uint32_t* pack_ready, size_t ready_cap, uint32_t* n_witness, uint32_t* n_ready,
                        uint32_t* n_inline, gw_status_t* status) {
    PackSchedule s;
    const std::string err = make_pack_schedule(p, s);
    if (!err.empty()) return fail(status, err);
    if (n_witness) *n_witness = (uint32_t)s.order.size();
    if (n_ready) *n_ready = (uint32_t)s.ready.size();
    if (n_inline) *n_inline = s.n_inline;
    if (pack_order && order_cap >= s.order.size() && !s.order.empty()) memcpy(pack_order, s.order.data(), s.order.size() * 4);
    if (pack_ready && ready_cap >= s.ready.size()) memcpy(pack_ready, s.ready.data(), s.ready.size() * 4);
    set_status(status, OK, "");
    return 0;
}

extern "C" int gwb_pack_schedule_of_blob(const void* blob, size_t len, uint32_t* pack_order, size_t order_cap, uint32_t* pack_ready, size_t ready_cap,
                                         uint32_t* n_witness, uint32_t* n_ready, uint32_t* n_inline, gw_status_t* status) {
    return guarded(status, [&]() -> int {
        if (!blob) return fail(status, "null argument");
        if (len < 24 + 8) return fail(status, "bad blob: too short");
        const uint8_t* b = (const uint8_t*)blob;
        uint64_t tr[3];
        memcpy(tr, b + len - 24, 24);
        if (tr[2] != blob_checksum(b, len - 24)) return fail(status, "bad blob: checksum mismatch (truncated or corrupted)");
        if (tr[0] > tr[1] || tr[1] > len - 24) return fail(status, "bad blob trailer");
        Program p;
        std::string err;
        if (!program_from_blob(b, (size_t)tr[0], p, err) || !validate_program(p, err)) return fail(status, "bad program blob: " + err);
        return schedule_out(p, pack_order, order_cap, pack_ready, ready_cap, n_witness, n_ready, n_inline, status);
    });
}

extern "C" int gwb_pack_schedule(gwb_graph_t* g, uint32_t program_key, uint32_t* pack_order, size_t order_cap, uint32_t* pack_ready, size_t ready_cap,
                                 uint32_t* n_witness, uint32_t* n_ready, uint32_t* n_inline, gw_status_t* status) {
    return guarded(status, [&]() -> int {
        if (!g) return fail(status, "null argument");
        std::lock_guard<std::mutex> lk(g->mu);
        Program tmp;
        const Program* p = nullptr;
        if ((program_key & ~KEY_MODE_MASK) == 64) program_key = 64;
        auto it = g->progs.find(program_key);
        auto pre = g->compiled.find(program_key);
        std::string err;
        if (it != g->progs.end()) {
            p = &it->second->host;
        } else if (pre != g->compiled.end()) {
            p = pre->second.get();
        } else {
            if (!g->has_graph) return fail(status, "imported handle has no program for that key");
            if (!compile_program(g->graph, program_key & ~KEY_MODE_MASK, key_divider_waves(program_key), tmp, err, key_streams(program_key))) return fail(status, err);
            p = &tmp;
        }
        return schedule_out(*p, pack_order, order_cap, pack_ready, ready_cap, n_witness, n_ready, n_inline, status);
    });
}
```

circom-witnesscalc_amd/csrc/pipeline.cc:

```cpp
#include "runtime_internal.hpp"

namespace cwcrt {


void set_status(gw_status_t* st, GW_ERROR_CODE code, const std::string& msg) {
    if (!st) return;
    st->code = code;
    if (code == OK && msg.empty()) {
        st->error_msg = nullptr;
        return;
    }
    st->error_msg = (char*)malloc(msg.size() + 1);
    if (st->error_msg) memcpy(st->error_msg, msg.c_str(), msg.size() + 1);
}
int fail(gw_status_t* st, const std::string& msg) {
    set_status(st, ERROR, msg);
    return 1;
}
std::string upload_program(DeviceProgram& dp) {
    const Program& p = dp.host;
    auto al = [](size_t x) { return (x + 255) & ~(size_t)255; };
    const size_t o_hdr = 0, o_recs = o_hdr + al(p.hdr.size() * 4 + 16), o_crefs = o_recs + al(p.recs.size() * 4 + REC_AHEAD * 1024u),
                 o_consts = o_crefs + al(p.crefs.size() * 4 + 256), o_wit = o_consts + al(p.consts.size() * 4 + 32),
                 o_div = o_wit + al(p.witness_refs.size() * 4 + 4), o_order = o_div + al(p.div_lanes.size() * 4 + 4),
                 o_entries = o_order + al(p.witness_refs.size() * 4 + 4), o_ready = o_entries + al((p.witness_refs.size() + PACK_ENTRY_PAD) * 8),
                 total = o_ready + al(((size_t)p.n_div_requests + 1) * 4);
    {
        const std::string serr = make_pack_schedule(p, dp.sched);
        if (!serr.empty()) return serr;
    }
    HIP_TRY(hipMalloc(&dp.d_blob, total));
    char* d = (char*)dp.d_blob;
    HIP_TRY(hipMemset(d, 0, total));
    if (!p.hdr.empty()) HIP_TRY(hipMemcpy(d + o_hdr, p.hdr.data(), p.hdr.size() * 4, hipMemcpyHostToDevice));
    if (!p.recs.empty()) HIP_TRY(hipMemcpy(d + o_recs, p.recs.data(), p.recs.size() * 4, hipMemcpyHostToDevice));
    if (!p.crefs.empty()) HIP_TRY(hipMemcpy(d + o_crefs, p.crefs.data(), p.crefs.size() * 4, hipMemcpyHostToDevice));
    if (!p.consts.empty()) HIP_TRY(hipMemcpy(d + o_consts, p.consts.data(), p.consts.size() * 4, hipMemcpyHostToDevice));
    if (!p.witness_refs.empty()) HIP_TRY(hipMemcpy(d + o_wit, p.witness_refs.data(), p.witness_refs.size() * 4, hipMemcpyHostToDevice));
    dp.dev.hdr = (const uint32_t*)(d + o_hdr);
    dp.dev.recs = (const uint32_t*)(d + o_recs);
    dp.dev.crefs = (const uint32_t*)(d + o_crefs);
    dp.dev.consts = (const uint32_t*)(d + o_consts);
    if (!p.div_lanes.empty()) HIP_TRY(hipMemcpy(d + o_div, p.div_lanes.data(), p.div_lanes.size() * 4, hipMemcpyHostToDevice));
    dp.dev.witness_refs = (const uint32_t*)(d + o_wit);
    dp.dev.div_lanes = (const uint32_t*)(d + o_div);
    dp.dev.n_bundles = p.n_bundles;
    dp.dev.n_slots = p.n_slots;
    dp.dev.n_inputs = p.n_inputs;
    dp.dev.n_witness = p.n_witness;
    dp.dev.n_const = p.n_const;
    dp.dev.trash_off = p.trash_off;
    dp.dev.has_fused = 0;
    for (uint32_t h : p.hdr) dp.dev.has_fused |= (h & HDR_CLASS_MASK) == C_MULF ? 1u : ((h & HDR_CLASS_MASK) == C_SCAN || ((h & HDR_CLASS_MASK) == C_MUL && (h & HDR_MUL_CC))) ? 2u : 0u;
    if (dp.dev.has_fused == 2u && getenv("CWC_FORCE_MODE3")) dp.dev.has_fused = 3u;
    if (dp.dev.has_fused == 2u)
        for (uint32_t h : p.hdr)
            if ((h & HDR_CLASS_MASK) == C_SCAN && !(h & HDR_SCAN_CONV) &&
                ((h & (HDR_SCAN_BORROW | HDR_SCAN_LEX)) || (!(h & HDR_SCAN_DIV) && ((h >> HDR_SCAN_SHIFT_SHIFT) & 0xffu) != 64u))) {
                dp.dev.has_fused = 3u;
                break;
            }
    {
        const PackSchedule& sc = dp.sched;
        std::vector<uint32_t> entries(sc.order.size() * 2);
        for (size_t i = 0; i < sc.order.size(); ++i) {
            entries[2 * i] = sc.order[i];
            entries[2 * i + 1] = p.witness_refs[sc.order[i]];
        }
        if (!sc.order.empty()) HIP_TRY(hipMemcpy(d + o_order, sc.order.data(), sc.order.size() * 4, hipMemcpyHostToDevice));
        if (!entries.empty()) HIP_TRY(hipMemcpy(d + o_entries, entries.data(), entries.size() * 4, hipMemcpyHostToDevice));
        HIP_TRY(hipMemcpy(d + o_ready, sc.ready.data(), sc.ready.size() * 4, hipMemcpyHostToDevice));
        dp.dev.pack_order = (const uint32_t*)(d + o_order);
        dp.dev.pack_entries = (const uint32_t*)(d + o_entries);
        dp.dev.pack_ready = (const uint32_t*)(d + o_ready);
        dp.dev.n_inline = sc.n_inline;
        dp.dev.n_ready_last = sc.ready.back();
    }
    dp.dev.n_streams = p.n_streams;
    for (uint32_t s = 0; s < MAX_STREAMS; ++s) {
        dp.dev.stream_first[s] = p.stream_first[s];
        dp.dev.stream_count[s] = p.stream_count[s];
        dp.dev.stream_div_requests[s] = p.stream_div_requests[s];
        dp.dev.stream_cref_first[s] = p.stream_cref_first[s];
    }
    return "";
}

static bool stream_pair_workgroups(uint32_t divider, uint64_t tiles, uint32_t streams) {
    if (streams != 2 || divider != 1) return false;
    if (const char* e = getenv("CWC_STREAM_TILES_PER_WORKGROUP")) return atoi(e) == 2;
    return tiles > 256;
}
uint32_t waves_per_workgroup(uint32_t divider, uint64_t tiles, uint32_t streams) {
    if (stream_pair_workgroups(divider, tiles, streams)) return 4u;
    if (streams > 1) return divider ? streams : 4u;
    const char* e = getenv("CWC_WAVES_PER_WORKGROUP");
    if (divider == 1) return e ? (atoi(e) >= 4 ? 2u : 1u) : (tiles > 256 ? 2u : 1u);
    if (divider) return 1;
    if (e) return atoi(e) == 4 ? 4u : 1u;
    return tiles > 512 ? 4u : 1u;
}

uint64_t workspace_budget() {
    const char* e = getenv("CWC_WORKSPACE_GB");
    double gb = e ? atof(e) : 8.0;
    if (gb < 1e-4) gb = 1e-4;
    return (uint64_t)(gb * (double)(1ull << 30));
}
}

extern "C" uint32_t gwb_pick_tile_width(size_t batch) {
    size_t target = 2048, divider_tiles = 1024;
    if (const char* e = getenv("CWC_TARGET_WAVES")) {
        long v = atol(e);
        if (v > 0) target = (size_t)v;
    }
    if (const char* e = getenv("CWC_DIVIDER_TILES")) divider_tiles = (size_t)atol(e);
    uint32_t t = batch <= 256 ? 1 : batch <= 1024 ? 2 : 4;
    while (t < 64 && (batch + t - 1) / t > target) t *= 2;
    const size_t tiles = (batch + t - 1) / t;
    return t | (tiles <= divider_tiles && t < 64 ? KEY_DIVIDER : 0u);
}

namespace cwcrt {

std::string check_device() {
    int n = 0;
    hipError_t e = hipGetDeviceCount(&n);
    if (e != hipSuccess || n <= 0)
        return std::string("no HIP device available (") + (e != hipSuccess ? hipGetErrorString(e) : "device count 0") +
               "); this library has no CPU fallback";
    static const std::string xnack_refusal = []() -> std::string {
        int dev = 0;
        hipDeviceProp_t prop;
        if (hipGetDevice(&dev) != hipSuccess || hipGetDeviceProperties(&prop, dev) != hipSuccess) {
            (void)hipGetLastError();
            return "";
        }
        return strstr(prop.gcnArchName, "xnack+") ? std::string("device ") + prop.gcnArchName + ": XNACK-enabled devices are not supported (run with HSA_XNACK=0)" : "";
    }();
    return xnack_refusal;
}

double estimate_cycles(const Program& p, size_t batch) {
    const double wide = p.T >= 8 ? 1.10 : 1.0;
    if (p.n_streams > 1) {
        const double tiles = (double)((batch + p.T - 1) / p.T);
        if (stream_pair_workgroups(p.divider, (uint64_t)tiles, p.n_streams)) {
            constexpr double kTwoWaves = 0.62, kPackCyclesPerValue = 0.028;
            double t = 0;
            for (uint32_t s = 0; s < p.n_streams; ++s) {
                const double own = std::max(p.stream_cycles[s], p.stream_chain_cycles[s]);
                const double simd = (p.stream_cycles[s] + model_class_cycles(C_DIV) * p.stream_div_requests[s]) * kTwoWaves;
                t = std::max(t, std::max(own, simd));
            }
            const double rounds = std::max(1.0, tiles / 512.0);
            return t * (p.T >= 4 ? 1.2 * wide : 1.0) * rounds + kPackCyclesPerValue * (double)p.n_witness * (double)batch;
        }
        const double t = program_wave_cycles(p);
        double busy = 0;
        for (uint32_t s = 0; s < p.n_streams; ++s) busy += (p.stream_cycles[s] + model_class_cycles(C_DIV) * p.stream_div_requests[s]) / t;
        const double wgs = p.divider ? tiles : std::ceil(tiles * p.n_streams / 4.0);
        const double wg_per_cu = p.divider ? (p.n_streams == 4 ? 1.0 : 3.0) : 2.0;
        const double rounds = std::max(1.0, wgs / (256.0 * wg_per_cu));
        const double crowd = std::max(1.0, 1.1 * (tiles / rounds) * busy / 1024.0);
        return t * (p.T >= 4 ? 1.2 * wide : p.T == 2 ? 1.08 : 1.0) * crowd * rounds;
    }
    const double per_wave = program_wave_cycles(p) * wide;
    const double heavy = program_wave_cycles_mul_div(p) * wide;
    const double waves = (double)((batch + p.T - 1) / p.T);
    const double two_per_simd = (1.3 * heavy + 1.9 * (per_wave - heavy)) / per_wave;
    if (p.divider == 4) return per_wave * 1.30 * (waves <= 1024 ? 1.0 : waves / 1024);
    if (p.divider == 3) return per_wave * 1.08 * (waves <= 768 ? 1.0 : two_per_simd * (waves <= 1536 ? 1.0 : waves / 1536));
    const double resident = waves * (p.divider == 1 ? 2.0 : 1.0);
    double crowd = resident <= 1024 ? 1.0 : two_per_simd;
    if (p.divider == 1 && resident > 1024) crowd = 1.0 + 0.75 * (crowd - 1.0);
    const double rounds = resident <= 2048 ? 1.0 : resident / 2048;
    return per_wave * crowd * rounds;
}

std::vector<uint32_t> candidate_keys(const ProgramStats& stats, size_t batch, uint32_t rule, uint32_t min_t) {
    size_t divider_tiles = 1024;
    if (const char* e = getenv("CWC_DIVIDER_TILES")) divider_tiles = (size_t)atol(e);
    const bool has_div = stats.class_nodes[C_DIV] > 0;
    const uint32_t t0 = rule & ~KEY_MODE_MASK;
    std::vector<uint32_t> keys;
    for (uint32_t t = std::max(min_t, t0 >= 4 ? t0 / 4 : 1u); t <= t0 * 2 && t <= 32 && (batch >= 64 || t == t0); t *= 2)
        for (uint32_t mode : {0u, KEY_DIVIDER, KEY_TRIPLE, KEY_GROUP}) {
            const size_t tiles = (batch + t - 1) / t;
            if (tiles > 4 * 2048) continue;
            const bool divider_fits = has_div && tiles <= divider_tiles;
            if (mode == 0 && divider_fits) continue;
            if (mode == KEY_DIVIDER && !divider_fits) continue;
            if (mode == KEY_TRIPLE && !(has_div && tiles > 512 && tiles <= 768 && !getenv("CWC_NO_GROUP_DIVIDER"))) continue;
            if (mode == KEY_GROUP && !(has_div && tiles > 512 && tiles <= 1024 && !getenv("CWC_NO_GROUP_DIVIDER"))) continue;
            keys.push_back(t | mode);
            if ((mode == 0 || mode == KEY_DIVIDER) && t < 64 && !getenv("CWC_NO_STREAMS")) {
                if (tiles <= 256) keys.push_back(t | mode | KEY_STREAMS4);
                else if (tiles <= 340) keys.push_back(t | mode | KEY_STREAMS2);
                else if (mode == KEY_DIVIDER && t >= 2 && tiles <= 512 && !getenv("CWC_INLINE_PACK") && !getenv("CWC_INLINE_PACK_ROWS"))
                    keys.push_back(t | mode | KEY_STREAMS2);
            }
        }
    return keys;
}

gwb_graph::Refined refine_choice(const Graph& graph, const ProgramStats& stats, size_t batch, uint32_t rule, uint32_t min_t) {
    gwb_graph::Refined r;
    try {
        double best_cost = -1;
        std::unique_ptr<SharedRewrites, void (*)(SharedRewrites*)> rewrites(make_shared_rewrites(), free_shared_rewrites);
        for (uint32_t key : candidate_keys(stats, batch, rule, min_t)) {
            std::unique_ptr<Program> p(new Program());
            std::string err;
            if (!compile_program(graph, key & ~KEY_MODE_MASK, key_divider_waves(key), *p, err, key_streams(key), false, rewrites.get())) continue;
            const double cost = estimate_cycles(*p, batch);
            if (best_cost < 0 || cost < best_cost) {
                best_cost = cost;
                r.best = key;
            }
            r.programs[key] = std::move(p);
        }
    } catch (...) {
        r.best = 0;
        r.programs.clear();
    }
    return r;
}

uint32_t pick_tile_width(gwb_graph* g, size_t batch, bool allow_quick) {
    if (!g->has_graph && !g->progs.empty()) return g->progs.begin()->first;
    if (g->forced_T) return g->forced_T;
    if (const char* e = getenv("CWC_TILE_WIDTH")) {
        const uint32_t key = (uint32_t)atoi(e), t = key & ~KEY_MODE_MASK;
        if (t >= 1 && t <= 64 && !(t & (t - 1))) return key;
    }
    uint32_t rule = gwb_pick_tile_width(batch);
    uint32_t min_t = 1;
    {
        double budget = 960.0;
        if (const char* e = getenv("CWC_PROGRAM_MB")) budget = atof(e);
        const double per_bundle_t1 = 4.0 + 64.0 * 16.0;
        auto levels = [&](uint32_t t) { return (double)(t <= SCAN_MAX_T && !getenv("CWC_NO_SCAN") && g->stats.depth_scan ? g->stats.depth_scan : g->stats.depth); };
        while (min_t < 16 && levels(min_t) * 1.25 * (4.0 + (per_bundle_t1 - 4.0) / min_t) > budget * 1048576.0) min_t *= 2;
        if ((rule & ~KEY_MODE_MASK) < min_t) rule = min_t | ((rule & KEY_MODE_MASK) && min_t < 64 ? (rule & KEY_MODE_MASK) : 0u);
    }
    if (getenv("CWC_STATIC_TILE_RULE") || !g->has_graph) return rule;
    auto hit = g->chosen.find(batch);
    if (hit != g->chosen.end()) return hit->second;
    if (batch < 64 && g->graph.nodes.size() <= 2000000 && !getenv("CWC_NO_QUICK_FIRST_CALL")) {
        auto job = g->refining.find(batch);
        if (job != g->refining.end()) {
            if (!allow_quick) {
                if (g->refine_gate) g->refine_gate->store(true);
                job->second.wait();
            }
            if (job->second.wait_for(std::chrono::seconds(0)) != std::future_status::ready) return g->provisional[batch];
            gwb_graph::Refined r = job->second.get();
            g->refining.erase(job);
            const uint32_t quick_key = g->provisional[batch];
            g->provisional.erase(batch);
            if (r.best == 0) {
                g->chosen[batch] = quick_key;
                return quick_key;
            }
            for (auto& kv : r.programs) {
                if (g->progs.count(kv.first)) {
                    if (g->filled_prog == g->progs[kv.first].get()) g->filled_prog = nullptr;
                    g->progs.erase(kv.first);
                }
                g->compiled[kv.first] = std::move(kv.second);
            }
            g->chosen[batch] = r.best;
            return r.best;
        }
        const bool has_div0 = g->stats.class_nodes[C_DIV] > 0;
        const uint32_t t1 = std::max(1u, min_t);
        const uint32_t quick_key = t1 | (has_div0 && t1 < 64 ? KEY_DIVIDER : 0u) | (t1 < 64 && !getenv("CWC_NO_STREAMS") ? KEY_STREAMS4 : 0u);
        if (allow_quick && !g->progs.count(quick_key) && !g->compiled.count(quick_key)) {
            std::unique_ptr<Program> p(new Program());
            std::string err;
            if (compile_program(g->graph, quick_key & ~KEY_MODE_MASK, key_divider_waves(quick_key), *p, err, key_streams(quick_key), true)) g->compiled[quick_key] = std::move(p);
        }
        if (allow_quick && (g->progs.count(quick_key) || g->compiled.count(quick_key))) {
            const Graph* graph = &g->graph;
            const ProgramStats stats = g->stats;
            g->provisional[batch] = quick_key;
            const std::string cache_file = batch == 1 && !g->cache_written ? g->cache_path : std::string();
            const std::vector<InputSignal> inputs = cache_file.empty() ? std::vector<InputSignal>() : g->inputs;
            if (!cache_file.empty()) g->cache_written = true;
            if (!g->refine_gate) g->refine_gate = std::make_shared<std::atomic<bool>>(false);
            g->refine_gate->store(false);
            std::shared_ptr<std::atomic<bool>> gate = g->refine_gate;
            g->refining[batch] = std::async(std::launch::async, [graph, stats, batch, rule, min_t, cache_file, inputs, gate]() {
                for (int waited = 0; !gate->load() && waited < 2000; ++waited) std::this_thread::sleep_for(std::chrono::milliseconds(1));
                gwb_graph::Refined r = refine_choice(*graph, stats, batch, rule, min_t);
                auto best = r.programs.find(r.best);
                if (!cache_file.empty() && r.best && best != r.programs.end()) {
                    try {
                        const std::vector<uint8_t> b0 = exported_bytes(*best->second, inputs), b = cache_wrap(cache_file, b0.data(), b0.size());
                        write_file_atomically(cache_file, b.data(), b.size());
                        if (getenv("CWC_DEBUG_CACHE")) fprintf(stderr, "program cache: wrote %s (program key %#x, %zu bytes)\n", cache_file.c_str(), r.best, b.size());
                    } catch (...) {
                    }
                }
                return r;
            });
            return quick_key;
        }
    }
    const bool debug = getenv("CWC_DEBUG_COST") != nullptr;
    uint32_t best = rule;
    double best_cost = -1;
    const std::vector<uint32_t> keys = candidate_keys(g->stats, batch, rule, min_t);
    std::unique_ptr<SharedRewrites, void (*)(SharedRewrites*)> rewrites(make_shared_rewrites(), free_shared_rewrites);
    std::vector<std::pair<uint32_t, std::future<std::unique_ptr<Program>>>> jobs;
    for (uint32_t key : keys)
        if (!g->progs.count(key) && !g->compiled.count(key)) {
            const Graph* graph = &g->graph;
            SharedRewrites* shared = rewrites.get();
            jobs.emplace_back(key, std::async(std::launch::async, [graph, key, shared]() {
                                  std::unique_ptr<Program> p(new Program());
                                  std::string err;
                                  if (!compile_program(*graph, key & ~KEY_MODE_MASK, key_divider_waves(key), *p, err, key_streams(key), false, shared)) p.reset();
                                  return p;
                              }));
        }
    for (auto& j : jobs) {
        std::unique_ptr<Program> p = j.second.get();
        if (p) g->compiled[j.first] = std::move(p);
    }
    for (uint32_t key : keys) {
        const Program* p = nullptr;
        auto up = g->progs.find(key);
        auto pre = g->compiled.find(key);
        if (up != g->progs.end()) p = &up->second->host;
        else if (pre != g->compiled.end()) p = pre->second.get();
        else continue;
        const double cost = estimate_cycles(*p, batch);
        if (debug) fprintf(stderr, "cost model: batch %zu key %#x -> %.1f Mcycles\n", batch, key, cost / 1e6);
        if (best_cost < 0 || cost < best_cost) {
            best_cost = cost;
            best = key;
        }
    }
    g->chosen[batch] = best;
    return best;
}

std::string get_program(gwb_graph* g, uint32_t key, DeviceProgram** out) {
    const uint32_t T = key & ~KEY_MODE_MASK;
    if (T == 64) key = T;
    auto it = g->progs.find(key);
    if (it != g->progs.end()) {
        *out = it->second.get();
        return "";
    }
    if (!g->has_graph) return "imported graph handle has no program for tile width " + std::to_string(T);
    std::unique_ptr<DeviceProgram> dp(new DeviceProgram());
    std::string err;
    auto pre = g->compiled.find(key);
    if (pre != g->compiled.end()) {
        dp->host = std::move(*pre->second);
        g->compiled.erase(pre);
    } else if (!compile_program(g->graph, T, key_divider_waves(key), dp->host, err, key_streams(key))) {
        return err;
    }
    err = upload_program(*dp);
    if (!err.empty()) return err;
    *out = dp.get();
    g->progs[key] = std::move(dp);
    return "";
}

static const bool kInlinePackDefault = true;
std::string run_device(gwb_graph* g, const void* d_inputs, size_t batch, void* d_witness, uint32_t* d_status,
                       hipStream_t stream, bool montgomery, hipEvent_t done_event) {
    if (batch == 0) return "";
    if (batch > 0x7fffffffull) return "batch too large";
    static const bool dbg_steps = getenv("CWC_DEBUG_SINGLE") != nullptr;
    auto now_ms = []() { return std::chrono::duration<double, std::milli>(std::chrono::steady_clock::now().time_since_epoch()).count(); };
    const double t_0 = dbg_steps ? now_ms() : 0.0;
    const uint32_t key = pick_tile_width(g, batch);
    struct OpenGate {
        gwb_graph* g;
        ~OpenGate() {
            if (g->refine_gate) g->refine_gate->store(true);
        }
    } open_gate{g};
    const double t_1 = dbg_steps ? now_ms() : 0.0;
    DeviceProgram* dp = nullptr;
    std::string err = get_program(g, key, &dp);
    if (!err.empty()) return err;
    const double t_2 = dbg_steps ? now_ms() : 0.0;
    g->last_key = (key & ~KEY_MODE_MASK) == 64 ? 64u : key;
    const Program& p = dp->host;
    const uint32_t T = p.T;
    if (!g->last_done) HIP_TRY(hipEventCreateWithFlags(&g->last_done, hipEventDisableTiming));
    if (g->has_last && g->last_stream != stream) HIP_TRY(hipStreamWaitEvent(stream, g->last_done, 0));
    struct OrderGuard {
        gwb_graph* g;
        hipStream_t stream;
        ~OrderGuard() {
            if (hipEventRecord(g->last_done, stream) == hipSuccess) {
                g->last_stream = stream;
                g->has_last = true;
            } else {
                (void)hipGetLastError();
                g->has_last = false;
                (void)hipDeviceSynchronize();
            }
        }
    } order_guard{g, stream};
    const uint64_t bytes_per_tile = ws_tile_bytes(p.n_const, p.n_slots, T);
    const uint64_t budget = workspace_budget();
    if (bytes_per_tile > 0xffffffffull) return "graph too large for the 4 GiB tile window";
    uint64_t max_tiles = budget / bytes_per_tile;
    if (max_tiles == 0) max_tiles = 1;
    const uint64_t tiles_total = (batch + T - 1) / T;
    const uint64_t chunk_tiles = tiles_total < max_tiles ? tiles_total : max_tiles;
    const size_t need = (size_t)(chunk_tiles * bytes_per_tile);
    const size_t chunk_sets = (size_t)chunk_tiles * T;
    const size_t n_chunks = (batch + chunk_sets - 1) / chunk_sets;
    size_t per_launch = n_chunks < WS_MAX_CHUNKS ? n_chunks : WS_MAX_CHUNKS;
    if (const char* e = getenv("CWC_STREAMS")) {
        const long v = atol(e);
        if (v >= 1 && (size_t)v < per_launch) per_launch = (size_t)v;
    }
    bool refill = g->filled_prog != dp || g->filled_tiles_per_chunk != chunk_tiles || g->filled_chunks < per_launch;
    for (size_t l = 0; l < per_launch; ++l) {
        if (need > g->vals_bytes[l]) {
            if (g->d_vals[l]) HIP_TRY(hipFree(g->d_vals[l]));
            g->d_vals[l] = nullptr;
            g->vals_bytes[l] = 0;
            g->filled_prog = nullptr;
            refill = true;
            HIP_TRY(hipMalloc(&g->d_vals[l], need));
            g->vals_bytes[l] = need;
        }
    }
    if (refill) {
        WsTable all;
        memset(&all, 0, sizeof all);
        all.tiles_per_chunk = (uint32_t)chunk_tiles;
        all.n_chunks = (uint32_t)per_launch;
        for (size_t l = 0; l < per_launch; ++l) all.base[l] = g->d_vals[l];
        HIP_TRY(launch_fill_consts(T, dp->dev, all, (uint32_t)(per_launch * chunk_tiles), stream));
        g->filled_prog = dp;
        g->filled_tiles_per_chunk = chunk_tiles;
        g->filled_chunks = per_launch;
    }
    const double t_3 = dbg_steps ? now_ms() : 0.0;
    g->last_call_launches = 0;
    g->timing = gwb_timing_t{};
    g->timing.tile_width = T;
    g->timing.divider = p.divider;
    g->timing.streams = p.n_streams;
    g->timing.n_bundles = p.n_bundles;
    g->timing.n_slots = p.n_slots;
    uint32_t n_inline = kInlinePackDefault ? dp->dev.n_inline : 0u;
    if (const char* e = getenv("CWC_INLINE_PACK")) n_inline = atoi(e) >= 2 ? dp->dev.n_ready_last : atoi(e) == 1 ? dp->dev.n_inline : 0u;
    if (const char* e = getenv("CWC_INLINE_PACK_ROWS")) n_inline = std::min<uint32_t>(n_inline, (uint32_t)atol(e));
    const size_t launch_sets = per_launch * chunk_sets;
    for (size_t s0 = 0; s0 < batch; s0 += launch_sets) {
        const uint32_t nb = (uint32_t)((batch - s0) < launch_sets ? (batch - s0) : launch_sets);
        WsTable wst;
        memset(&wst, 0, sizeof wst);
        wst.tiles_per_chunk = (uint32_t)chunk_tiles;
        wst.n_chunks = (uint32_t)((nb + chunk_sets - 1) / chunk_sets);
        for (uint32_t l = 0; l < wst.n_chunks; ++l) wst.base[l] = g->d_vals[l];
        hipEvent_t e0, e1, e2;
        if (g->pending.size() >= gwb_graph::kHistory) {
            e0 = g->pending.front().start, e1 = g->pending.front().after_interp, e2 = g->pending.front().after_pack;
            g->pending.pop_front();
        } else {
            e0 = e1 = e2 = nullptr;
            const bool ok = hipEventCreate(&e0) == hipSuccess && hipEventCreate(&e1) == hipSuccess && hipEventCreate(&e2) == hipSuccess;
            if (!ok) {
                for (hipEvent_t e : {e0, e1, e2})
                    if (e) (void)hipEventDestroy(e);
                return "hipEventCreate failed";
            }
        }
        g->pending.push_back(gwb_graph::ChunkEvents{e0, e1, e2});
        HIP_TRY(hipEventRecord(e0, stream));
        void* const out = (char*)d_witness + s0 * (size_t)p.n_witness * 32;
        HIP_TRY(launch_interp(T, p.divider, waves_per_workgroup(p.divider, (nb + T - 1) / T, p.n_streams), p.n_div_requests, dp->dev.div_lanes, dp->dev, wst, (const char*)d_inputs + s0 * p.n_inputs * 32, d_status + s0, nb, stream, g->d_prof,
                              out, n_inline, montgomery));
        HIP_TRY(hipEventRecord(e1, stream));
        HIP_TRY(launch_pack(T, dp->dev, wst, out, nb, stream, montgomery, n_inline));
        HIP_TRY(hipEventRecord(e2, stream));
        g->last_call_launches++;
        g->timing.n_launches++;
    }
    g->timing_pending = true;
    if (done_event) HIP_TRY(hipEventRecord(done_event, stream));
    if (g->refine_gate) g->refine_gate->store(true);
    if (dbg_steps && now_ms() - t_0 > 20.0)
        fprintf(stderr, "run_device: program choice %.1f ms, program on the device %.1f ms, workspace + constants %.1f ms, launches %.1f ms\n", t_1 - t_0, t_2 - t_1, t_3 - t_2, now_ms() - t_3);
    return "";
}

bool is_pinned_host(const void* p) {
    hipPointerAttribute_t a;
    memset(&a, 0, sizeof a);
    if (hipPointerGetAttributes(&a, p) != hipSuccess) {
        (void)hipGetLastError();
        return false;
    }
    return a.type == hipMemoryTypeHost;
}

unsigned env_threads(const char* name, unsigned cap) {
    long v = 0;
    if (const char* e = getenv(name)) v = atol(e);
    if (v <= 0) {
        v = (long)std::thread::hardware_concurrency();
        if (cap && v > (long)cap) v = cap;
    }
    return v < 1 ? 1u : (unsigned)v;
}

unsigned copy_threads() {
    long v = 0;
    if (const char* e = getenv("CWC_COPY_THREADS")) v = atol(e);
    if (v <= 0) {
        v = (long)std::thread::hardware_concurrency();
        if (v > 16) v = 16;
    }
    return v < 1 ? 1u : (unsigned)v;
}

std::string device_to_host_rows(gwb_graph* g, void* dst, const void* d_src, size_t bytes) {
    if (bytes == 0) return "";
    if (!g->copy_stream) HIP_TRY(hipStreamCreateWithFlags(&g->copy_stream, hipStreamNonBlocking));
    if (is_pinned_host(dst)) {
        HIP_TRY(hipMemcpyAsync(dst, d_src, bytes, hipMemcpyDeviceToHost, g->copy_stream));
        HIP_TRY(hipStreamSynchronize(g->copy_stream));
        return "";
    }
    size_t slice = 32u << 20;
    if (const char* e = getenv("CWC_COPY_SLICE_MB")) {
        const long v = atol(e);
        if (v >= 1 && v <= 1024) slice = (size_t)v << 20;
    }
    if (bytes < slice) slice = std::max<size_t>(g->stage_bytes, (bytes + (1u << 20) - 1) & ~(size_t)((1u << 20) - 1));
    const int n_stage = bytes > slice ? 2 : 1;
    if (g->stage_bytes < slice) {
        for (int i = 0; i < 2; ++i) {
            if (g->stage[i]) HIP_TRY(hipHostFree(g->stage[i]));
            g->stage[i] = nullptr;
        }
        g->stage_bytes = 0;
        for (int i = 0; i < n_stage; ++i) HIP_TRY(hipHostMalloc(&g->stage[i], slice, hipHostMallocDefault));
        g->stage_bytes = slice;
    }
    if (n_stage == 2 && !g->stage[1]) HIP_TRY(hipHostMalloc(&g->stage[1], g->stage_bytes, hipHostMallocDefault));
    for (int i = 0; i < 2; ++i)
        if (!g->stage_done[i]) HIP_TRY(hipEventCreateWithFlags(&g->stage_done[i], hipEventDisableTiming));
    const size_t n_slices = (bytes + slice - 1) / slice;
    const unsigned n_workers = bytes < (8u << 20) ? 1u : copy_threads();
    std::atomic<long> ready{0};
    std::atomic<bool> abort{false};
    std::vector<std::atomic<unsigned>> consumed(n_slices);
    for (auto& c : consumed) c.store(0);
    auto stripe_copy = [&](unsigned w, size_t k) {
        const size_t off = k * slice, len = bytes - off < slice ? bytes - off : slice;
        const size_t per = ((len + n_workers - 1) / n_workers + 4095) & ~(size_t)4095;
        const size_t a = (size_t)w * per, b = a + per < len ? a + per : len;
        if (a < b) memcpy((char*)dst + off + a, (const char*)g->stage[k & 1] + a, b - a);
    };
    std::vector<std::thread> workers;
    for (unsigned w = 1; w < n_workers; ++w)
        workers.emplace_back([&, w]() {
            for (size_t k = 0; k < n_slices; ++k) {
                while (ready.load(std::memory_order_acquire) <= (long)k) {
                    if (abort.load()) return;
                    std::this_thread::yield();
                }
                stripe_copy(w, k);
                consumed[k].fetch_add(1, std::memory_order_release);
            }
        });
    std::string err;
    auto issue = [&](size_t k) -> std::string {
        const size_t off = k * slice, len = bytes - off < slice ? bytes - off : slice;
        HIP_TRY(hipMemcpyAsync(g->stage[k & 1], (const char*)d_src + off, len, hipMemcpyDeviceToHost, g->copy_stream));
        HIP_TRY(hipEventRecord(g->stage_done[k & 1], g->copy_stream));
        return "";
    };
    err = issue(0);
    for (size_t k = 0; k < n_slices && err.empty(); ++k) {
        if (k + 1 < n_slices) {
            if (k >= 1)
                while (consumed[k - 1].load(std::memory_order_acquire) < n_workers) std::this_thread::yield();
            err = issue(k + 1);
            if (!err.empty()) break;
        }
        if (hipEventSynchronize(g->stage_done[k & 1]) != hipSuccess) {
            err = "hipEventSynchronize failed in the witness copy";
            break;
        }
        ready.store((long)k + 1, std::memory_order_release);
        stripe_copy(0, k);
        consumed[k].fetch_add(1, std::memory_order_release);
    }
    if (!err.empty()) abort.store(true);
    for (auto& t : workers) t.join();
    if (!err.empty()) (void)hipStreamSynchronize(g->copy_stream);
    return err;
}

std::string run_host(gwb_graph* g, const void* inputs, size_t batch, void* witness, uint32_t* set_status) {
    if (batch == 0) return "";
    const size_t in_b = batch * (size_t)g->n_inputs * 32, out_b = batch * (size_t)g->n_witness * 32;
    auto grow = [](void*& p, size_t& have, size_t need) -> std::string {
        if (need <= have) return "";
        if (p) HIP_TRY(hipFree(p));
        p = nullptr;
        have = 0;
        HIP_TRY(hipMalloc(&p, need));
        have = need;
        return "";
    };
    static const bool dbg_steps = getenv("CWC_DEBUG_SINGLE") != nullptr;
    auto now_ms = []() { return std::chrono::duration<double, std::milli>(std::chrono::steady_clock::now().time_since_epoch()).count(); };
    const double t0 = dbg_steps ? now_ms() : 0.0;
    std::string err = grow(g->h_in, g->h_in_bytes, in_b ? in_b : 32);
    if (err.empty()) err = grow(g->h_out, g->h_out_bytes, out_b ? out_b : 32);
    if (err.empty()) err = grow(g->h_st, g->h_st_bytes, batch * 4);
    if (!err.empty()) return err;
    HIP_TRY(hipMemcpy(g->h_in, inputs, in_b, hipMemcpyHostToDevice));
    const double t1 = dbg_steps ? now_ms() : 0.0;
    err = run_device(g, g->h_in, batch, g->h_out, (uint32_t*)g->h_st, nullptr);
    if (!err.empty()) return err;
    const double t2 = dbg_steps ? now_ms() : 0.0;
    HIP_TRY(hipDeviceSynchronize());
    const double t3 = dbg_steps ? now_ms() : 0.0;
    err = device_to_host_rows(g, witness, g->h_out, out_b);
    if (!err.empty()) return err;
    HIP_TRY(hipMemcpy(set_status, g->h_st, batch * 4, hipMemcpyDeviceToHost));
    if (dbg_steps && now_ms() - t0 > 20.0)
        fprintf(stderr, "run_host: device buffers + rows in %.1f ms, run_device (choice, upload, workspace, launches) %.1f ms, wait for the device %.1f ms, rows out %.1f ms\n", t1 - t0, t2 - t1, t3 - t2, now_ms() - t3);
    return "";
}

std::string set_status_text(uint32_t bits) {
    std::string s;
    if (bits & ST_SHL_OVERFLOW) s += "Shl result does not fit the field (reference panics at graph.rs:634)";
    if (bits & 0x80000000u) s += std::string(s.empty() ? "" : "; ") + "internal error: divider mailbox wait timed out";
    if (bits & 0x40000000u) s += std::string(s.empty() ? "" : "; ") + "internal error: wait for another stream's post timed out";
    if (bits & ST_BITOP_EQ_R) s += std::string(s.empty() ? "" : "; ") + "bit operation result equals the modulus (reference panics at graph.rs:686/701/716)";
    return s;
}

void warm_device() {
    struct Joined {
        std::thread t;
        ~Joined() {
            if (t.joinable()) t.join();
        }
    };
    static Joined warm;
    static std::once_flag once;
    std::call_once(once, []() {
        if (getenv("CWC_NO_WARM_THREAD")) return;
        warm.t = std::thread([]() {
            int n = 0;
            if (hipGetDeviceCount(&n) != hipSuccess || n <= 0) {
                (void)hipGetLastError();
                return;
            }
            void* p = nullptr;
            if (hipMalloc(&p, 4096) == hipSuccess) (void)hipFree(p);
            else (void)hipGetLastError();
            if (launch_warm(nullptr) != hipSuccess) (void)hipGetLastError();
        });
    });
}

}
```

circom-witnesscalc_amd/csrc/program_dev.h:

```cpp
#pragma once
#include <stdint.h>

#include "ops.h"

#if defined(__HIPCC__)
#define CWC_HD __host__ __device__ static inline
#define CWC_HDC __host__ __device__ static constexpr
#else
#define CWC_HD static inline
#define CWC_HDC static constexpr
#endif

namespace cwc {

enum BundleClass : uint32_t {
    C_INPUT = 0,
    C_MUL = 1,
    C_LIN = 2,
    C_DIV = 3,
    C_CMPZ = 4,
    C_CMPS = 5,
    C_BIT = 6,
    C_IDIVMOD = 7,
    C_TERN = 8,
    C_DIVREQ = 9,
    C_DIVGET = 10,
    C_MULQ = 11,
    C_SYNC = 12,
    C_MULF = 13,
    C_SCAN = 14,
    C_COUNT = 15
};
static const uint32_t COOP_LANES = 4, COOP_MAX_T = 4, COOP_FUSE_MAX_T = 2, SCAN_MAX_T = 2;
static const uint32_t HDR_SCAN_DIV = 1u << 11, HDR_SCAN_CONV = 1u << 12;
enum SelCode : uint32_t { SEL_LT = 1, SEL_GT = 2, SEL_LEQ = 3, SEL_GEQ = 4, SEL_NEZ = 5, SEL_OUT_MONT = 8 };
static const uint32_t HDR_SCAN_BORROW = 1u << 13, HDR_SCAN_LEX = 1u << 14, HDR_SCAN_KG = 1u << 15, HDR_SCAN_KL = 1u << 16;
static const int HDR_SCAN_SHIFT_SHIFT = 19, HDR_SCAN_ITER_SHIFT = 27;
static const uint32_t SCAN_ROLE_ACC = 1u, SCAN_START = 2u;
enum FusedOp : uint32_t { FOP_NONE = 0, FOP_MUL = 1, FOP_ADD = 2, FOP_SUB = 3 , FOP_RSUB = 4  };
static const uint32_t HDR_F_S2MUL = 1u << 11, HDR_F_S2LIN = 1u << 12, HDR_F_S3LIN = 1u << 13;
CWC_HDC uint32_t coop_nodes(uint32_t T) { return T <= COOP_MAX_T ? 64u / (COOP_LANES * T) : 0u; }

static const uint32_t OFF_NOWHERE = 0xffff0000u;
static const uint32_t HDR_CLASS_MASK = 0xfu;
static const int HDR_COUNT_SHIFT = 4;
static const uint32_t HDR_LIN_SUB = 1u << 11, HDR_LIN_ADD = 1u << 12, HDR_BITX_ALL = 1u << 13;
static const uint32_t HDR_MUL_CC = 1u << 13;
static const uint32_t HDR_BIT_ALL_SHR = 1u << 11, HDR_BIT_ALL_BAND = 1u << 12;
static const uint32_t HDR_B_CANON = 1u << 14, HDR_A_CANON = 1u << 17, HDR_OUT_CANON = 1u << 18;
static const uint32_t HDR_POST = 1u << 15, HDR_WAIT = 1u << 16;
static const uint32_t MAX_STREAMS = 4;
static const uint32_t PROF_WORDS = 96, CENSUS_MAX_WAVES = 8192, CENSUS_WORDS = 3;
static const uint32_t CTRL_SUB_MASK = 7u, CTRL_ACTIVE = 8u, CTRL_MASK = 15u;
static const uint32_t RING_BUNDLES = 4, OPND_AHEAD = 2, REC_AHEAD = 4;
static const uint32_t RING_SLOT_BYTES = 2048, LDS_HALF_BYTES = 1024, STAGE_BYTES = 4096, REC_BYTES = 1024;
CWC_HDC uint32_t mbox_lanes(uint32_t W) { return W <= 1u ? 64u : 32u; }
CWC_HDC uint32_t mbox_bytes(uint32_t W) { return mbox_lanes(W) * 64u; }
CWC_HDC uint32_t lds_area_bytes(uint32_t W, uint32_t lds_bytes) { return (void)W, lds_bytes; }
static const uint32_t LDS_RING_OFF = 0, LDS_STAGE_OFF = LDS_RING_OFF + RING_BUNDLES * RING_SLOT_BYTES,
                      LDS_REC_OFF = LDS_STAGE_OFF + OPND_AHEAD * STAGE_BYTES, LDS_BYTES = LDS_REC_OFF + REC_AHEAD * REC_BYTES;
enum SubOp : uint32_t {
    SUB_ADD = 0, SUB_SUB = 1, SUB_MULT = 2,
    SUB_EQ = 0, SUB_NEQ = 1, SUB_LAND = 2, SUB_LOR = 3,
    SUB_LT = 0, SUB_GT = 1, SUB_LEQ = 2, SUB_GEQ = 3,
    SUB_SHL = 0, SUB_SHR = 1, SUB_BOR = 2, SUB_BAND = 3, SUB_BXOR = 4,
    SUB_BITX = 5,
    SUB_IDIV = 0, SUB_MOD = 1,
};

static const uint32_t REF_CONST = 0x80000000u;
static const uint32_t REF_CANON = 0x40000000u;

enum SetStatus : uint32_t {
    ST_SHL_OVERFLOW = 1u,
    ST_BITOP_EQ_R = 2u,
};

struct ProgramDev {
    const uint32_t* hdr;
    const uint32_t* recs;
    const uint32_t* crefs;
    const uint32_t* consts;
    const uint32_t* witness_refs;
    const uint32_t* div_lanes;
    uint32_t n_bundles, n_slots, n_inputs, n_witness, n_const;
    uint32_t trash_off;
    uint32_t has_fused;
    uint32_t n_streams, stream_first[4], stream_count[4], stream_div_requests[4], stream_cref_first[4];
    const uint32_t* pack_order;
    const uint32_t* pack_entries;
    const uint32_t* pack_ready;
    uint32_t n_inline, n_ready_last;
};
static const uint32_t PACK_ENTRY_PAD = 192;

static const uint32_t WS_MAX_CHUNKS = 32;
struct WsTable {
    void* base[WS_MAX_CHUNKS];
    uint32_t tiles_per_chunk;
    uint32_t n_chunks;
};

CWC_HD uint64_t ws_tile_bytes(uint32_t n_const, uint32_t n_slots, uint32_t T) { return ((uint64_t)n_const + n_slots + 3u) * 32u * T; }
CWC_HD uint64_t ws_sync_offset(uint32_t n_const, uint32_t n_slots, uint32_t T) { return ((uint64_t)n_const + n_slots + 2u) * 32u * T; }

}
```

circom-witnesscalc_amd/csrc/runtime_internal.hpp:

```cpp
#pragma once
#include <dlfcn.h>
#include <sys/stat.h>
#include <sys/types.h>
#include <unistd.h>
#include <hip/hip_runtime_api.h>
#include <stdio.h>
#include <stdlib.h>
#include <string.h>

#include <chrono>
#include <cmath>
#include <condition_variable>
#include <map>
#include <memory>
#include <mutex>
#include <algorithm>
#include <atomic>
#include <deque>
#include <future>
#include <string>
#include <thread>
#include <vector>

#define GW_NO_INLINE_FREE_STATUS
#ifndef CWC_TREE_HASH
#define CWC_TREE_HASH "unstamped"
#endif
#include "../../include/graph_witness_batch.h"
#include "graph.hpp"
#include "program.hpp"

namespace cwc {
hipError_t launch_interp(uint32_t T, uint32_t W, uint32_t pack, uint32_t n_div_requests, const uint32_t* div_lanes, const ProgramDev& p,
                         const WsTable& wst, const void* inputs, uint32_t* status, uint32_t batch, hipStream_t stream, unsigned long long* prof,
                         void* out = nullptr, uint32_t n_inline = 0, bool montgomery = false);
hipError_t launch_pack(uint32_t T, const ProgramDev& p, const WsTable& wst, void* out, uint32_t batch, hipStream_t stream, bool montgomery, uint32_t first = 0);
hipError_t launch_modmul_ubench(uint32_t n_cus, uint32_t waves_per_simd, uint32_t iters, uint32_t* sink, hipStream_t stream, bool block_multiplier);
hipError_t launch_fill_consts(uint32_t T, const ProgramDev& p, const WsTable& wst, uint32_t n_tiles, hipStream_t stream);
hipError_t launch_warm(hipStream_t stream);
}

using namespace cwc;

namespace cwcrt {

void set_status(gw_status_t* st, GW_ERROR_CODE code, const std::string& msg);
int fail(gw_status_t* st, const std::string& msg);
template <class F>
int guarded(gw_status_t* st, F&& f) {
    try {
        return f();
    } catch (const std::bad_alloc&) {
        return fail(st, "out of memory");
    } catch (const std::exception& e) {
        return fail(st, std::string("internal error: ") + e.what());
    } catch (...) {
        return fail(st, "internal error");
    }
}
#define HIP_TRY(expr)                                                                      \
    do {                                                                                   \
        hipError_t e_ = (expr);                                                            \
        if (e_ != hipSuccess) return std::string(#expr) + ": " + hipGetErrorString(e_);    \
    } while (0)

struct PackSchedule {
    std::vector<uint32_t> order;
    std::vector<uint32_t> ready;
    uint32_t n_inline = 0;
};
std::string make_pack_schedule(const Program& p, PackSchedule& out);

struct DeviceProgram {
    Program host;
    PackSchedule sched;
    void* d_blob = nullptr;
    ProgramDev dev{};
    DeviceProgram() = default;
    DeviceProgram(const DeviceProgram&) = delete;
    DeviceProgram& operator=(const DeviceProgram&) = delete;
    ~DeviceProgram() {
        if (d_blob) (void)hipFree(d_blob);
    }
};

}
using namespace cwcrt;

struct gwb_graph {
    Graph graph;
    bool has_graph = false;
    std::vector<InputSignal> inputs;
    std::unordered_map<std::string, uint32_t> input_index;
    uint32_t n_inputs = 0, n_witness = 0;
    ProgramStats stats;
    std::map<uint32_t, std::unique_ptr<DeviceProgram>> progs;
    std::map<uint32_t, std::unique_ptr<Program>> compiled;
    std::map<size_t, uint32_t> chosen;
    uint32_t forced_T = 0;
    uint32_t last_key = 0;
    struct Refined {
        uint32_t best = 0;
        std::map<uint32_t, std::unique_ptr<Program>> programs;
    };
    std::map<size_t, std::future<Refined>> refining;
    std::map<size_t, uint32_t> provisional;
    std::shared_ptr<std::atomic<bool>> refine_gate;
    bool cache_written = false;
    std::string cache_path;
    struct E2eBufs {
        void* h_rows[2] = {nullptr, nullptr};
        void* d_in[2] = {nullptr, nullptr};
        void* d_out[2] = {nullptr, nullptr};
        void* d_st[2] = {nullptr, nullptr};
        void* stage[2][3] = {{nullptr, nullptr, nullptr}, {nullptr, nullptr, nullptr}};
        hipStream_t compute = nullptr, copy[2] = {nullptr, nullptr};
        hipEvent_t done[2] = {nullptr, nullptr}, slice_done[2][3] = {{nullptr, nullptr, nullptr}, {nullptr, nullptr, nullptr}};
        size_t in_bytes = 0, out_bytes = 0, st_bytes = 0, stage_bytes = 0;
        void release() {
            for (int i = 0; i < 2; ++i) {
                if (h_rows[i]) (void)hipHostFree(h_rows[i]);
                if (d_in[i]) (void)hipFree(d_in[i]);
                if (d_out[i]) (void)hipFree(d_out[i]);
                if (d_st[i]) (void)hipFree(d_st[i]);
                h_rows[i] = d_in[i] = d_out[i] = d_st[i] = nullptr;
                for (int b = 0; b < 3; ++b) {
                    if (stage[i][b]) (void)hipHostFree(stage[i][b]);
                    stage[i][b] = nullptr;
                }
            }
            in_bytes = out_bytes = st_bytes = stage_bytes = 0;
        }
    } e2e;
    static const int kMaxLanes = (int)WS_MAX_CHUNKS;
    void* d_vals[kMaxLanes] = {nullptr};
    size_t vals_bytes[kMaxLanes] = {0};
    const DeviceProgram* filled_prog = nullptr;
    uint64_t filled_tiles_per_chunk = 0;
    size_t filled_chunks = 0;
    bool timing_pending = false;
    gwb_timing_t timing{};
    unsigned long long* d_prof = nullptr;
    struct ChunkEvents { hipEvent_t start, after_interp, after_pack; };
    static const size_t kHistory = 256;
    std::deque<ChunkEvents> pending;
    size_t last_call_launches = 0;
    void *h_in = nullptr, *h_out = nullptr, *h_st = nullptr;
    size_t h_in_bytes = 0, h_out_bytes = 0, h_st_bytes = 0;
    void* stage[2] = {nullptr, nullptr};
    size_t stage_bytes = 0;
    hipEvent_t stage_done[2] = {nullptr, nullptr};
    hipStream_t copy_stream = nullptr;
    hipEvent_t last_done = nullptr;
    hipStream_t last_stream = nullptr;
    bool has_last = false;
    std::mutex mu;

    void drop_events() {
        for (auto& c : pending) { (void)hipEventDestroy(c.start); (void)hipEventDestroy(c.after_interp); (void)hipEventDestroy(c.after_pack); }
        pending.clear();
    }

    ~gwb_graph() {
        progs.clear();
        for (int i = 0; i < kMaxLanes; ++i)
            if (d_vals[i]) (void)hipFree(d_vals[i]);
        drop_events();
        for (void* p : {h_in, h_out, h_st})
            if (p) (void)hipFree(p);
        for (int i = 0; i < 2; ++i) {
            if (stage[i]) (void)hipHostFree(stage[i]);
            if (stage_done[i]) (void)hipEventDestroy(stage_done[i]);
        }
        if (copy_stream) (void)hipStreamDestroy(copy_stream);
        if (last_done) (void)hipEventDestroy(last_done);
        e2e.release();
        for (int i = 0; i < 2; ++i) {
            if (e2e.copy[i]) (void)hipStreamDestroy(e2e.copy[i]);
            if (e2e.done[i]) (void)hipEventDestroy(e2e.done[i]);
            for (int b = 0; b < 3; ++b)
                if (e2e.slice_done[i][b]) (void)hipEventDestroy(e2e.slice_done[i][b]);
        }
        if (e2e.compute) (void)hipStreamDestroy(e2e.compute);
    }
};

namespace cwcrt {
std::string upload_program(DeviceProgram& dp);
uint32_t waves_per_workgroup(uint32_t divider, uint64_t tiles, uint32_t streams = 1);
uint64_t workspace_budget();
std::string check_device();
double estimate_cycles(const Program& p, size_t batch);
uint32_t pick_tile_width(gwb_graph* g, size_t batch, bool allow_quick = true);
std::string get_program(gwb_graph* g, uint32_t key, DeviceProgram** out);
std::string run_device(gwb_graph* g, const void* d_inputs, size_t batch, void* d_witness, uint32_t* d_status, hipStream_t stream, bool montgomery = false,
                       hipEvent_t done_event = nullptr);
std::string run_host(gwb_graph* g, const void* inputs, size_t batch, void* witness, uint32_t* set_status);
unsigned env_threads(const char* name, unsigned cap);
std::string set_status_text(uint32_t bits);
void warm_device();
uint64_t fnv1a(const uint8_t* p, size_t n);
uint64_t blob_checksum(const uint8_t* p, size_t n);
uint64_t sampled_fingerprint(const uint8_t* p, size_t n);
size_t exported_size(const Program& p, const std::vector<InputSignal>& inputs);
void exported_write(const Program& p, const std::vector<InputSignal>& inputs, uint8_t* dst);
std::vector<uint8_t> exported_bytes(const Program& p, const std::vector<InputSignal>& inputs);
void write_file_atomically(const std::string& path, const void* data, size_t n);
std::vector<uint8_t> cache_wrap(const std::string& path, const void* blob, size_t n);
bool quirks();
int load_graph(const void* data, size_t len, gwb_graph** out, std::string& err);
}
extern "C" int gwb_kernels_have_diagnostics();
```

include/graph_witness_batch.h:

```cpp
#ifndef CWC_AMD_GRAPH_WITNESS_BATCH_H
#define CWC_AMD_GRAPH_WITNESS_BATCH_H

#include <stddef.h>
#include <stdint.h>

#include "graph_witness.h"

#ifdef __cplusplus
extern "C" {
#endif

typedef struct gwb_graph gwb_graph_t;

typedef struct {
  uint64_t n_nodes;
  uint64_t n_op;
  uint64_t n_input_nodes;
  uint64_t n_const;
  uint64_t n_inputs;
  uint64_t n_witness;
  uint64_t depth;
  uint64_t algorithmic_bytes_per_set;
} gwb_graph_info_t;

typedef struct {
  uint32_t tile_width;
  uint32_t n_launches;
  uint64_t n_bundles;
  uint64_t n_slots;
  float interp_ms;
  float pack_ms;
  uint32_t divider;
  uint32_t streams;
} gwb_timing_t;

int gwb_graph_load(const void *graph_data, size_t graph_data_len, gwb_graph_t **out, gw_status_t *status);
void gwb_graph_free(gwb_graph_t *g);
int gwb_graph_info(const gwb_graph_t *g, gwb_graph_info_t *info);
int gwb_graph_serialize(const gwb_graph_t *g, void **out, size_t *out_len, gw_status_t *status);

typedef struct gwb_builder gwb_builder_t;
#define GWB_BUILDER_BAD 0xffffffffu
gwb_builder_t *gwb_builder_new(void);
void gwb_builder_free(gwb_builder_t *b);
uint32_t gwb_builder_input(gwb_builder_t *b, uint32_t input_index);
uint32_t gwb_builder_constant(gwb_builder_t *b, const void *value_le, size_t value_len);
uint32_t gwb_builder_uno(gwb_builder_t *b, uint32_t op, uint32_t a);
uint32_t gwb_builder_duo(gwb_builder_t *b, uint32_t op, uint32_t a, uint32_t b_idx);
uint32_t gwb_builder_tres(gwb_builder_t *b, uint32_t op, uint32_t a, uint32_t b_idx, uint32_t c);
int gwb_builder_witness(gwb_builder_t *b, uint32_t node);
int gwb_builder_input_signal(gwb_builder_t *b, const char *name, uint32_t offset, uint32_t len);
uint64_t gwb_builder_node_count(const gwb_builder_t *b);
int gwb_builder_finish(const gwb_builder_t *b, void **out, size_t *out_len, gw_status_t *status);

int gwb_graphgen_bigint_class(uint32_t k, uint32_t n_bits, uint32_t rounds, void **out, size_t *out_len, gw_status_t *status);
int gwb_graphgen_rsa_long_div_class(uint32_t n, uint32_t k, uint32_t muls, int range_checks, void **out, size_t *out_len, gw_status_t *status);
int gwb_graph_op_histogram(const gwb_graph_t *g, uint64_t *out, size_t n);

int gwb_inputs_from_json(const gwb_graph_t *g, const char *inputs_json, void *row, gw_status_t *status);

int gwb_inputs_from_json_batch(const gwb_graph_t *g, const char *text, size_t text_len, void *rows, size_t max_rows,
                               size_t *n_rows, gw_status_t *status);
int gwb_wtns_save_batch(const void *witness, size_t n_witness, size_t batch, const char *path_pattern, gw_status_t *status);

typedef struct {
  size_t n_sets, sub_batch;
  uint32_t parse_threads, write_threads;
  double parse_seconds;
  double wait_for_drain_seconds;
  double total_seconds;
  uint64_t witness_bytes;
  uint64_t failed_sets;
} gwb_e2e_stats_t;
int gwb_calc_witness_json_to_wtns(gwb_graph_t *g, const char *text, size_t text_len, const char *path_pattern, size_t first_index,
                                  size_t *n_sets, uint32_t *set_status, size_t max_sets, gwb_e2e_stats_t *stats, gw_status_t *status);

#define GWB_TILE_ASYNC_DIVIDER 0x100u
#define GWB_TILE_GROUP_DIVIDER 0x200u
#define GWB_TILE_TRIPLE_DIVIDER 0x400u
#define GWB_TILE_STREAMS2 0x800u
#define GWB_TILE_STREAMS4 0x1000u
int gwb_set_tile_width(gwb_graph_t *g, uint32_t tile_width);
uint32_t gwb_pick_tile_width(size_t batch);
uint32_t gwb_graph_pick_tile_width(gwb_graph_t *g, size_t batch);

int gwb_calc_witness_batch_device(gwb_graph_t *g, const void *d_inputs, size_t batch, void *d_witness,
                                  uint32_t *d_set_status, void *hip_stream, gw_status_t *status);
#define GWB_FORM_CANONICAL 0u
#define GWB_FORM_MONTGOMERY 1u
typedef struct {
  uint32_t struct_size;
  uint32_t form;
  void *hip_stream;
  void *done_event;
} gwb_handoff_t;
int gwb_calc_witness_batch_handoff(gwb_graph_t *g, const void *d_inputs, size_t batch, void *d_witness,
                                   uint32_t *d_set_status, const gwb_handoff_t *handoff, gw_status_t *status);

int gwb_calc_witness_batch_host(gwb_graph_t *g, const void *inputs, size_t batch, void *witness,
                                uint32_t *set_status, gw_status_t *status);
void *gwb_host_alloc(size_t bytes);
void gwb_host_free(void *p);
int gwb_last_timing(gwb_graph_t *g, gwb_timing_t *t);
int gwb_timing_history(gwb_graph_t *g, size_t max_launches, float *interp_ms, float *pack_ms, size_t *n_out);

int gwb_profile_classes(gwb_graph_t *g, const void *d_inputs, size_t batch, void *d_witness,
                        uint32_t *d_set_status, uint64_t *out64, gw_status_t *status);
int gwb_wave_census(gwb_graph_t *g, const void *d_inputs, size_t batch, void *d_witness,
                    uint32_t *d_set_status, uint64_t *out64, size_t out_words, gw_status_t *status);

double gwb_ubench_modmul(uint32_t waves_per_simd, uint32_t iters);

double gwb_ubench_modmul_block(uint32_t waves_per_simd, uint32_t iters);
double gwb_model_class_cycles(uint32_t bundle_class);
const char* gwb_kernel_source_hash(void);

typedef struct {
  uint32_t tile_width, divider, streams, n_classes;
  uint64_t n_bundles, n_fused_nodes;
  uint64_t class_bundles[16];
  uint64_t class_nodes[16];
  double model_wave_cycles;
  double lanes_active_mean;
  double values_per_bundle_mean;
  double chain_floor_cycles;
  uint64_t n_scan_steps;
  uint64_t n_conv_products;
} gwb_program_stats_t;
int gwb_program_stats(gwb_graph_t *g, uint32_t program_key, gwb_program_stats_t *out);

int gwb_pack_schedule(gwb_graph_t *g, uint32_t program_key, uint32_t *pack_order, size_t order_cap, uint32_t *pack_ready, size_t ready_cap,
                      uint32_t *n_witness, uint32_t *n_ready, uint32_t *n_inline, gw_status_t *status);
int gwb_pack_schedule_of_blob(const void *blob, size_t blob_len, uint32_t *pack_order, size_t order_cap, uint32_t *pack_ready, size_t ready_cap,
                              uint32_t *n_witness, uint32_t *n_ready, uint32_t *n_inline, gw_status_t *status);

size_t gwb_wtns_size(size_t n_witness);
int gwb_wtns_from_witness(const void *witness_row, size_t n_witness, void *out);

int gwb_graph_export(gwb_graph_t *g, uint32_t tile_width, void **blob, size_t *blob_len, gw_status_t *status);
int gwb_graph_import(const void *blob, size_t blob_len, gwb_graph_t **out, gw_status_t *status);

#define GWB_RCCL_UNIQUE_ID_BYTES 128
int gwb_rccl_unique_id(void *id128, gw_status_t *status);
int gwb_rccl_comm_init(const void *id128, int n_ranks, int rank, void **comm, gw_status_t *status);
int gwb_rccl_comm_ranks(void *comm);
void gwb_rccl_comm_destroy(void *comm);
int gwb_graph_broadcast(gwb_graph_t *g, uint32_t tile_width, size_t batch_per_rank, int root, int rank, void *nccl_comm,
                        void *hip_stream, gwb_graph_t **out, gw_status_t *status);

void gwb_free_status(gw_status_t *status);

#ifdef __cplusplus
}
#endif
#endif
```

Measured before the change: 93120.

## Pack witness rows in idle stream tails inside the interpreter kernel

When the interpreter runs several streams with one divider and four waves per workgroup, streams that finish before the slowest stream now pack witness rows they alone wrote, reading a per-stream tail table. A cost model estimates each stream's end time and picks how many rows fit in the idle gap. The separate pack kernel then covers only the remaining rows. This aims to overlap pack work with the critical stream's tail, at the cost of extra device tables, kernarg pointer smuggling through LDS, and more complex scheduling logic.

```diff
diff --git a/circom-witnesscalc_amd/__init__.py b/circom-witnesscalc_amd/__init__.py
--- a/circom-witnesscalc_amd/__init__.py
+++ b/circom-witnesscalc_amd/__init__.py
@@ -72,7 +72,7 @@
     "gwb_builder_witness", "gwb_builder_input_signal", "gwb_builder_node_count", "gwb_builder_finish",
     "gwb_ubench_modmul_block", "gwb_program_stats", "gwb_calc_witness_json_to_wtns", "gwb_model_class_cycles",
     "gwb_graphgen_bigint_class", "gwb_graphgen_rsa_long_div_class", "gwb_graph_op_histogram",
-    "gwb_kernel_source_hash", "gwb_pack_schedule", "gwb_pack_schedule_of_blob", "gwb_rccl_unique_id", "gwb_rccl_comm_init", "gwb_rccl_comm_ranks", "gwb_rccl_comm_destroy",
+    "gwb_kernel_source_hash", "gwb_pack_schedule", "gwb_pack_schedule_of_blob", "gwb_pack_tails", "gwb_rccl_unique_id", "gwb_rccl_comm_init", "gwb_rccl_comm_ranks", "gwb_rccl_comm_destroy",
     "gwb_wave_census",
 ]
 
@@ -147,6 +147,8 @@
         if hasattr(L, "gwb_pack_schedule"):
             L.gwb_pack_schedule.argtypes = [vp, ctypes.c_uint32, vp, sz, vp, sz, u32p, u32p, u32p, stp]
             L.gwb_pack_schedule_of_blob.argtypes = [vp, sz, vp, sz, vp, sz, u32p, u32p, u32p, stp]
+        if hasattr(L, "gwb_pack_tails"):
+            L.gwb_pack_tails.argtypes = [vp, ctypes.c_uint32, ctypes.c_int, vp, sz, vp, vp, stp]
         L.gwb_calc_witness_json_to_wtns.argtypes = [vp, ctypes.c_char_p, sz, ctypes.c_char_p, sz, ctypes.POINTER(sz), vp, sz, ctypes.POINTER(E2eStats), stp]
         L.gwb_graph_pick_tile_width.restype = ctypes.c_uint32
         L.gwb_graph_pick_tile_width.argtypes = [vp, sz]
@@ -450,6 +452,12 @@
 
     def pack_schedule(self, key):
         return _pack_schedule(lambda *a: lib().gwb_pack_schedule(self._h, key, *a))
+
+    def pack_tails(self, key, all=False):
+        st = GwStatus()
+        order, off, end = np.zeros(self.n_witness, dtype=np.uint32), np.zeros(5, dtype=np.uint32), np.zeros(4, dtype=np.float64)
+        _check(lib().gwb_pack_tails(self._h, key, 1 if all else 0, order.ctypes.data, order.size, off.ctypes.data, end.ctypes.data, ctypes.byref(st)), st)
+        return order, off, end
 
     def last_timing(self):
         t = Timing()
diff --git a/circom-witnesscalc_amd/csrc/kernels.hip b/circom-witnesscalc_amd/csrc/kernels.hip
--- a/circom-witnesscalc_amd/csrc/kernels.hip
+++ b/circom-witnesscalc_amd/csrc/kernels.hip
@@ -51,6 +51,93 @@
 __device__ __forceinline__ i32x4 make_rsrc_words(const void* base, uint32_t bytes) {
     const uint64_t a = (uint64_t)base;
     return i32x4{(int)(uint32_t)a, (int)((uint32_t)(a >> 32) & 0xffffu), (int)bytes, 0x00020000};
+}
+
+struct InterpArgs {
+    const uint32_t* hdr;
+    const uint4* recs;
+    const uint32_t* crefs;
+    InterpDims p;
+    WsTable wst;
+    const uint4* inputs;
+    uint32_t* status;
+    unsigned long long* prof;
+};
+typedef const __attribute__((address_space(4))) InterpArgs* kernarg_ptr;
+typedef const __attribute__((address_space(1))) u32x4* gconst_u32x4;
+typedef const __attribute__((address_space(1))) unsigned long long* gconst_u64;
+typedef const __attribute__((address_space(1))) uint32_t* gconst_u32;
+typedef __attribute__((address_space(1))) u32x4* gout_u32x4;
+
+template <int T, bool PROF>
+__device__ __noinline__ void tail_pack(kernarg_ptr ka_, uint32_t nbnd_, uint32_t set) {
+    constexpr uint32_t G = 64u / T;
+    const kernarg_ptr ka = (kernarg_ptr)((uint64_t)(uint32_t)__builtin_amdgcn_readfirstlane((int)(uint32_t)(uintptr_t)ka_) |
+                                         (uint64_t)(uint32_t)__builtin_amdgcn_readfirstlane((int)(uint32_t)((uintptr_t)ka_ >> 32)) << 32);
+    const uint32_t nbnd = (uint32_t)__builtin_amdgcn_readfirstlane((int)nbnd_);
+    const uint32_t NS = ka->p.n_streams;
+    if (NS <= 1) return;
+    uint32_t stream = 0;
+    for (uint32_t s = 1; s < MAX_STREAMS; ++s)
+        if (s < NS && ka->p.stream_count[s] != 0 && ka->p.stream_first[s] + ka->p.stream_count[s] == nbnd) stream = s;
+    const gconst_u32 table = (gconst_u32)(uintptr_t)ka->p.pack_ready;
+    const uint32_t count = table[MAX_STREAMS + stream];
+    if (count == 0) return;
+    const unsigned long long t0 = PROF ? __builtin_amdgcn_s_memtime() : 0ull;
+    asm volatile("s_waitcnt vmcnt(0)" ::: "memory");
+    __builtin_amdgcn_fence(__ATOMIC_ACQUIRE, "agent");
+    const uint32_t lane = __builtin_amdgcn_mbcnt_hi(~0u, __builtin_amdgcn_mbcnt_lo(~0u, 0u)), t = lane % T, j = (G == 1) ? 0u : lane / T;
+    const uint32_t tile = (uint32_t)__builtin_amdgcn_readfirstlane((int)set) / T;
+    const uint32_t n_const = ka->p.n_const, batch = ka->p.batch, n_witness = ka->p.n_witness, mont = ka->p.pack_mont;
+    const uint64_t tile_bytes = ws_tile_bytes(n_const, ka->p.n_slots, T);
+    const uint32_t tpc = ka->wst.tiles_per_chunk;
+    const gconst_u32x4 tile_base = (gconst_u32x4)((uintptr_t)ka->wst.base[tile / tpc] + (uint64_t)(tile % tpc) * tile_bytes);
+    const gconst_u64 entries = (gconst_u64)(uintptr_t)ka->p.pack_entries + table[stream];
+    const gout_u32x4 out = (gout_u32x4)(uintptr_t)ka->p.pack_out;
+    constexpr uint32_t U = 4;
+    auto entry = [&](uint32_t i) {
+        const unsigned long long e = entries[i < count ? i : count - 1u];
+        return make_uint2((uint32_t)e, (uint32_t)(e >> 32));
+    };
+    uint2 e[U];
+#pragma unroll
+    for (uint32_t u = 0; u < U; ++u) e[u] = entry(u * G + j);
+    for (uint32_t next = 0; next < count; next += U * G) {
+        u32x4 lo[U], hi[U];
+#pragma unroll
+        for (uint32_t u = 0; u < U; ++u) {
+            const uint32_t ref = e[u].y & ~REF_CANON;
+            const uint32_t slot = (ref & REF_CONST) ? (ref & ~REF_CONST) : n_const + ref;
+            const gconst_u32x4 q = tile_base + (size_t)slot * (2 * T);
+            lo[u] = q[t];
+            hi[u] = q[T + t];
+        }
+        uint2 en[U];
+#pragma unroll
+        for (uint32_t u = 0; u < U; ++u) en[u] = entry(next + (U + u) * G + j);
+#pragma unroll
+        for (uint32_t u = 0; u < U; ++u) {
+            const bool valid = next + u * G + j < count && set < batch, canon = (e[u].y & REF_CANON) != 0;
+            const Fr v = Fr{{lo[u].x, lo[u].y, lo[u].z, lo[u].w, hi[u].x, hi[u].y, hi[u].z, hi[u].w}};
+            Fr c = v;
+            if (mont) {
+                if (wave_any(both(valid, canon))) c = u256_select(canon, fr_mul(v, fr_r2()), v);
+            } else {
+                if (wave_any(both(valid, !canon))) c = u256_select(canon, v, fr_from_mont(v));
+            }
+            if (valid) {
+                const gout_u32x4 o = out + ((size_t)set * n_witness + e[u].x) * 2;
+                o[0] = u32x4{c.v[0], c.v[1], c.v[2], c.v[3]};
+                o[1] = u32x4{c.v[4], c.v[5], c.v[6], c.v[7]};
+            }
+        }
+#pragma unroll
+        for (uint32_t u = 0; u < U; ++u) e[u] = en[u];
+    }
+    if (PROF && lane == 0 && (tile % 64u) == 0u) {
+        atomicAdd(&ka->prof[94], __builtin_amdgcn_s_memtime() - t0);
+        atomicAdd(&ka->prof[95], (unsigned long long)((count + G - 1u) / G));
+    }
 }
 
 template <int T, bool PROF, int W, int PACK, int MODE = 0>
@@ -109,6 +196,9 @@
     volatile uint32_t* const seq = reinterpret_cast<volatile uint32_t*>(mbox_all + NW * MB);
     if (DIVIDER || NW > 1) {
         if (DIVIDER && threadIdx.x < NW + (uint32_t)PACK) seq[threadIdx.x] = 0;
+        if constexpr (W == 1 && PACK == 4) {
+            if (threadIdx.x == 0) *reinterpret_cast<volatile uint64_t*>(const_cast<uint32_t*>(seq) + 8) = (uint64_t)(uintptr_t)__builtin_amdgcn_kernarg_segment_ptr();
+        }
         if (NS > 1 && wave < NW && stream == 0 && lane < MAX_STREAMS && tile_raw < n_tiles) {
             __hip_atomic_store(sync_words + lane, 0u, __ATOMIC_RELAXED, __HIP_MEMORY_SCOPE_AGENT);
             __builtin_amdgcn_fence(__ATOMIC_RELEASE, "agent");
@@ -1089,6 +1179,10 @@
         atomicAdd(&prof[93], psec[1][6]);
     }
     if (err_bits && set < batch) atomicOr(&status[set], err_bits);
+    if constexpr (W == 1 && PACK == 4) {
+        const uint64_t ka = *reinterpret_cast<volatile uint64_t*>(const_cast<uint32_t*>(seq) + 8);
+        tail_pack<T, PROF>((kernarg_ptr)(uintptr_t)ka, NBND, set);
+    }
 }
 
 __global__ __launch_bounds__(256) void fill_consts_kernel(ProgramDev p, WsTable wst, uint32_t n_tiles, uint32_t T) {
@@ -1205,7 +1299,7 @@
 
 hipError_t launch_interp(uint32_t T, uint32_t W, uint32_t pack, uint32_t n_div_requests, const uint32_t* div_lanes, const ProgramDev& p,
                          const WsTable& wst, const void* inputs, uint32_t* status, uint32_t batch, hipStream_t stream, unsigned long long* prof,
-                         void* out, uint32_t n_inline, bool montgomery) {
+                         void* out, uint32_t n_inline, bool montgomery, int tail) {
     const uint32_t tiles = (batch + T - 1) / T, nw = (W ? W : 1u) * pack, ns = p.n_streams ? p.n_streams : 1u;
     if (nw == 0 || nw % ns != 0 || (ns > 1 && W > 1)) return hipErrorInvalidValue;
     const uint32_t tiles_per_wg = nw / ns;
@@ -1214,6 +1308,11 @@
     InterpDims dims{p.n_bundles, p.n_slots, p.n_inputs, batch, p.n_const, n_div_requests, p.trash_off, div_lanes, ns, {0, 0, 0, 0}, {0, 0, 0, 0}, {0, 0, 0, 0}, {0, 0, 0, 0},
                     (uint4*)out, reinterpret_cast<const uint2*>(p.pack_entries), p.pack_ready, 0u, montgomery ? 1u : 0u, p.n_witness};
     if (W == 1 && ns == 1 && out && p.pack_entries && p.pack_ready) dims.n_inline = n_inline < p.n_ready_last ? n_inline : p.n_ready_last;
+    if (W == 1 && pack == 4 && ns > 1 && p.tail_table) {
+        const uint32_t m = out && tail >= 0 && tail < 2 ? (uint32_t)tail : 2u;
+        dims.pack_ready = p.tail_table + m * 2u * MAX_STREAMS;
+        dims.pack_entries = reinterpret_cast<const uint2*>(m < 2 ? p.tail_entries[m] : p.pack_entries);
+    }
     for (uint32_t s = 0; s < MAX_STREAMS; ++s) {
         dims.stream_first[s] = p.stream_first[s];
         dims.stream_count[s] = p.stream_count[s];
diff --git a/circom-witnesscalc_amd/csrc/pack_schedule.cc b/circom-witnesscalc_amd/csrc/pack_schedule.cc
--- a/circom-witnesscalc_amd/csrc/pack_schedule.cc
+++ b/circom-witnesscalc_amd/csrc/pack_schedule.cc
@@ -3,6 +3,102 @@
 namespace cwcrt {
 
 static const double kCyclesDividerServe = 52200, kCyclesPackPass = 2300;
+
+static const double kTwoWavesOnOneSimd = 0.62, kTailMargin = 0.5;
+
+static void tail_layout(const std::vector<std::vector<uint32_t>>& lists, uint32_t nw, std::vector<uint32_t>& order, uint32_t* off) {
+    std::vector<uint8_t> taken(nw, 0);
+    order.clear();
+    order.reserve(nw);
+    for (uint32_t s = 0; s < MAX_STREAMS; ++s) {
+        off[s] = (uint32_t)order.size();
+        if (s < lists.size())
+            for (uint32_t w : lists[s]) {
+                order.push_back(w);
+                taken[w] = 1;
+            }
+    }
+    off[MAX_STREAMS] = (uint32_t)order.size();
+    for (uint32_t w = 0; w < nw; ++w)
+        if (!taken[w]) order.push_back(w);
+}
+
+static std::string make_tail_lists(const Program& p, PackSchedule& out) {
+    const uint32_t nw = p.n_witness, G = p.G, NS = p.n_streams;
+    for (int m = 0; m < 2; ++m) {
+        out.tail_order[m].clear();
+        for (uint32_t s = 0; s <= MAX_STREAMS; ++s) out.tail_off[m][s] = 0;
+    }
+    for (uint32_t s = 0; s < MAX_STREAMS; ++s) out.stream_end[s] = 0;
+    if (NS <= 1 || NS > MAX_STREAMS || p.divider != 1 || nw == 0 || G == 0) return "";
+    if (p.hdr.size() < p.n_bundles || p.recs.size() < (size_t)p.n_bundles * G * 4 || p.witness_refs.size() < nw) return "pack schedule: truncated program";
+    const uint64_t slot_bytes = 32ull * p.T, first_off = (uint64_t)p.n_const * slot_bytes, end_off = ((uint64_t)p.n_const + p.n_slots) * slot_bytes;
+    std::vector<uint8_t> stream_of(p.n_bundles, 5), writers(p.n_slots, 0);
+    for (uint32_t s = 0; s < NS; ++s)
+        for (uint32_t b = p.stream_first[s]; b < p.stream_first[s] + p.stream_count[s] && b < p.n_bundles; ++b) stream_of[b] = (uint8_t)s;
+    uint32_t post = p.stream_first[0];
+    while (post < p.stream_first[0] + p.stream_count[0] && post < p.n_bundles && !(p.hdr[post] & HDR_POST)) ++post;
+    if (post < p.stream_first[0] + p.stream_count[0] && post < p.n_bundles)
+        for (uint32_t b = p.stream_first[0]; b < post; ++b) stream_of[b] = 4;
+    else
+        post = p.stream_first[0];
+    for (uint32_t b = 0; b < p.n_bundles; ++b)
+        for (uint32_t i = 0; i < G; ++i) {
+            const uint64_t dst = p.recs[((size_t)b * G + i) * 4 + 2] & ~CTRL_MASK;
+            if (dst >= first_off && dst < end_off) writers[(dst - first_off) / slot_bytes] |= (uint8_t)(1u << stream_of[b]);
+        }
+    double prologue = 0, slowest_end = -1;
+    for (uint32_t b = p.stream_first[0]; b <= post && post != p.stream_first[0]; ++b) prologue += model_class_cycles((int)(p.hdr[b] & HDR_CLASS_MASK));
+    uint32_t slowest = 0, earliest = MAX_STREAMS;
+    for (uint32_t s = 0; s < NS; ++s) {
+        if (p.stream_count[s] == 0) continue;
+        double clock = s ? prologue : 0, sum = 0, div_free = 0, served = 0, nreq = 0;
+        for (uint32_t b = p.stream_first[s]; b < p.stream_first[s] + p.stream_count[s] && b < p.n_bundles; ++b) {
+            const uint32_t cls = p.hdr[b] & HDR_CLASS_MASK;
+            const double c = model_class_cycles((int)cls);
+            clock += c;
+            sum += c;
+            if (cls == C_DIVREQ) {
+                served = div_free = std::max(clock, div_free) + kCyclesDividerServe;
+                ++nreq;
+            } else if (cls == C_DIVGET) {
+                clock = std::max(clock, served);
+            }
+        }
+        out.stream_end[s] = std::max(clock, (sum + kCyclesDividerServe * nreq) * kTwoWavesOnOneSimd);
+        if (out.stream_end[s] > slowest_end) slowest_end = out.stream_end[s], slowest = s;
+        if (earliest == MAX_STREAMS || out.stream_end[s] < out.stream_end[earliest]) earliest = s;
+    }
+    if (earliest == MAX_STREAMS) return "";
+    std::vector<std::vector<uint32_t>> all(NS), chosen(NS);
+    for (uint32_t w = 0; w < nw; ++w) {
+        const uint32_t ref = p.witness_refs[w];
+        uint32_t wr = 0;
+        if (!(ref & REF_CONST)) {
+            const uint32_t slot = ref & ~REF_CANON;
+            if (slot >= p.n_slots || writers[slot] == 0) return "pack schedule: witness " + std::to_string(w) + " names a slot that no bundle writes";
+            wr = writers[slot] & ~(1u << 4);
+        }
+        uint32_t s = earliest;
+        if (wr) {
+            if (wr & (wr - 1)) continue;
+            for (s = 0; !(wr >> s & 1u); ++s) {}
+            if (s >= NS || p.stream_count[s] == 0) continue;
+        }
+        all[s].push_back(w);
+    }
+    double pass_cycles = kCyclesPackPass;
+    if (const char* e = getenv("CWC_PACK_PASS_CYCLES")) pass_cycles = std::max(1.0, atof(e));
+    for (uint32_t s = 0; s < NS; ++s) {
+        if (s == slowest || p.stream_count[s] == 0) continue;
+        const double passes = std::floor(std::max(0.0, (slowest_end - out.stream_end[s]) * (1.0 - kTailMargin)) / pass_cycles);
+        const size_t rows = passes * G >= (double)all[s].size() ? all[s].size() : (size_t)passes * G;
+        chosen[s].assign(all[s].begin(), all[s].begin() + rows);
+    }
+    tail_layout(chosen, nw, out.tail_order[kTailReplay], out.tail_off[kTailReplay]);
+    tail_layout(all, nw, out.tail_order[kTailAll], out.tail_off[kTailAll]);
+    return "";
+}
 
 std::string make_pack_schedule(const Program& p, PackSchedule& out) {
     const uint32_t nw = p.n_witness, G = p.G, nreq = p.n_div_requests;
@@ -10,6 +106,10 @@
     out.ready.assign((size_t)nreq + 1, 0u);
     out.n_inline = 0;
     for (uint32_t i = 0; i < nw; ++i) out.order[i] = i;
+    {
+        const std::string terr = make_tail_lists(p, out);
+        if (!terr.empty()) return terr;
+    }
     if (p.divider != 1 || p.n_streams != 1 || nreq == 0 || nw == 0 || G == 0) return "";
     if (p.hdr.size() < p.n_bundles || p.recs.size() < (size_t)p.n_bundles * G * 4 || p.witness_refs.size() < nw) return "pack schedule: truncated program";
     const uint64_t slot_bytes = 32ull * p.T, first_off = (uint64_t)p.n_const * slot_bytes, end_off = ((uint64_t)p.n_const + p.n_slots) * slot_bytes;
@@ -62,6 +162,11 @@
     return "";
 }
 
+int tail_pack_mode() {
+    const char* e = getenv("CWC_TAIL_PACK");
+    return !e || !*e ? kTailReplay : atoi(e) >= 2 ? kTailAll : atoi(e) == 0 ? kTailOff : kTailReplay;
+}
+
 }
 
 static int schedule_out(const Program& p, uint32_t* pack_order, size_t order_cap, uint32_t* pack_ready, size_t ready_cap, uint32_t* n_witness, uint32_t* n_ready,
@@ -92,6 +197,37 @@
         std::string err;
         if (!program_from_blob(b, (size_t)tr[0], p, err) || !validate_program(p, err)) return fail(status, "bad program blob: " + err);
         return schedule_out(p, pack_order, order_cap, pack_ready, ready_cap, n_witness, n_ready, n_inline, status);
+    });
+}
+
+static int tails_out(const Program& p, int all, uint32_t* order, size_t order_cap, uint32_t* offsets, double* stream_end, gw_status_t* status) {
+    PackSchedule s;
+    const std::string err = make_pack_schedule(p, s);
+    if (!err.empty()) return fail(status, err);
+    const int m = all ? kTailAll : kTailReplay;
+    if (offsets) memcpy(offsets, s.tail_off[m], sizeof s.tail_off[m]);
+    if (stream_end) memcpy(stream_end, s.stream_end, sizeof s.stream_end);
+    if (order)
+        for (size_t i = 0; i < order_cap && i < p.n_witness; ++i) order[i] = s.tail_order[m].empty() ? (uint32_t)i : s.tail_order[m][i];
+    set_status(status, OK, "");
+    return 0;
+}
+
+extern "C" int gwb_pack_tails(gwb_graph_t* g, uint32_t program_key, int all, uint32_t* order, size_t order_cap, uint32_t* offsets, double* stream_end,
+                              gw_status_t* status) {
+    return guarded(status, [&]() -> int {
+        if (!g) return fail(status, "null argument");
+        std::lock_guard<std::mutex> lk(g->mu);
+        Program tmp;
+        if ((program_key & ~KEY_MODE_MASK) == 64) program_key = 64;
+        auto it = g->progs.find(program_key);
+        auto pre = g->compiled.find(program_key);
+        std::string err;
+        if (it != g->progs.end()) return tails_out(it->second->host, all, order, order_cap, offsets, stream_end, status);
+        if (pre != g->compiled.end()) return tails_out(*pre->second, all, order, order_cap, offsets, stream_end, status);
+        if (!g->has_graph) return fail(status, "imported handle has no program for that key");
+        if (!compile_program(g->graph, program_key & ~KEY_MODE_MASK, key_divider_waves(program_key), tmp, err, key_streams(program_key))) return fail(status, err);
+        return tails_out(tmp, all, order, order_cap, offsets, stream_end, status);
     });
 }
 
diff --git a/circom-witnesscalc_amd/csrc/pipeline.cc b/circom-witnesscalc_amd/csrc/pipeline.cc
--- a/circom-witnesscalc_amd/csrc/pipeline.cc
+++ b/circom-witnesscalc_amd/csrc/pipeline.cc
@@ -24,11 +24,15 @@
                  o_consts = o_crefs + al(p.crefs.size() * 4 + 256), o_wit = o_consts + al(p.consts.size() * 4 + 32),
                  o_div = o_wit + al(p.witness_refs.size() * 4 + 4), o_order = o_div + al(p.div_lanes.size() * 4 + 4),
                  o_entries = o_order + al(p.witness_refs.size() * 4 + 4), o_ready = o_entries + al((p.witness_refs.size() + PACK_ENTRY_PAD) * 8),
-                 total = o_ready + al(((size_t)p.n_div_requests + 1) * 4);
+                 o_tail = o_ready + al(((size_t)p.n_div_requests + 1) * 4);
+    size_t total = o_tail;
     {
         const std::string serr = make_pack_schedule(p, dp.sched);
         if (!serr.empty()) return serr;
     }
+    const bool tails = !dp.sched.tail_order[kTailReplay].empty();
+    const size_t tail_layout_bytes = al(p.witness_refs.size() * 4 + 4) + al((p.witness_refs.size() + PACK_ENTRY_PAD) * 8);
+    if (tails) total += al(3 * 2 * MAX_STREAMS * 4) + 2 * tail_layout_bytes;
     HIP_TRY(hipMalloc(&dp.d_blob, total));
     char* d = (char*)dp.d_blob;
     HIP_TRY(hipMemset(d, 0, total));
@@ -75,6 +79,28 @@
         dp.dev.pack_ready = (const uint32_t*)(d + o_ready);
         dp.dev.n_inline = sc.n_inline;
         dp.dev.n_ready_last = sc.ready.back();
+        if (tails) {
+            uint32_t table[3][2 * MAX_STREAMS] = {};
+            for (int m = 0; m < 2; ++m) {
+                const size_t o_o = o_tail + al(sizeof table) + m * tail_layout_bytes, o_e = o_o + al(p.witness_refs.size() * 4 + 4);
+                const std::vector<uint32_t>& ord = sc.tail_order[m];
+                for (size_t i = 0; i < ord.size(); ++i) {
+                    entries[2 * i] = ord[i];
+                    entries[2 * i + 1] = p.witness_refs[ord[i]];
+                }
+                HIP_TRY(hipMemcpy(d + o_o, ord.data(), ord.size() * 4, hipMemcpyHostToDevice));
+                HIP_TRY(hipMemcpy(d + o_e, entries.data(), entries.size() * 4, hipMemcpyHostToDevice));
+                dp.dev.tail_order[m] = (const uint32_t*)(d + o_o);
+                dp.dev.tail_entries[m] = (const uint32_t*)(d + o_e);
+                dp.dev.tail_rows[m] = sc.tail_off[m][MAX_STREAMS];
+                for (uint32_t s = 0; s < MAX_STREAMS; ++s) {
+                    table[m][s] = sc.tail_off[m][s];
+                    table[m][MAX_STREAMS + s] = sc.tail_off[m][s + 1] - sc.tail_off[m][s];
+                }
+            }
+            HIP_TRY(hipMemcpy(d + o_tail, table, sizeof table, hipMemcpyHostToDevice));
+            dp.dev.tail_table = (const uint32_t*)(d + o_tail);
+        }
     }
     dp.dev.n_streams = p.n_streams;
     for (uint32_t s = 0; s < MAX_STREAMS; ++s) {
@@ -155,7 +181,12 @@
                 t = std::max(t, std::max(own, simd));
             }
             const double rounds = std::max(1.0, tiles / 512.0);
-            return t * (p.T >= 4 ? 1.2 * wide : 1.0) * rounds + kPackCyclesPerValue * (double)p.n_witness * (double)batch;
+            double pack_rows = (double)p.n_witness;
+            if (const int mode = tail_pack_mode(); mode != kTailOff) {
+                PackSchedule sc;
+                if (make_pack_schedule(p, sc).empty()) pack_rows -= (double)sc.tail_off[mode][MAX_STREAMS];
+            }
+            return t * (p.T >= 4 ? 1.2 * wide : 1.0) * rounds + kPackCyclesPerValue * pack_rows * (double)batch;
         }
         const double t = program_wave_cycles(p);
         double busy = 0;
@@ -461,6 +492,7 @@
     uint32_t n_inline = kInlinePackDefault ? dp->dev.n_inline : 0u;
     if (const char* e = getenv("CWC_INLINE_PACK")) n_inline = atoi(e) >= 2 ? dp->dev.n_ready_last : atoi(e) == 1 ? dp->dev.n_inline : 0u;
     if (const char* e = getenv("CWC_INLINE_PACK_ROWS")) n_inline = std::min<uint32_t>(n_inline, (uint32_t)atol(e));
+    const int tail_mode = dp->dev.tail_table ? tail_pack_mode() : (int)kTailOff;
     const size_t launch_sets = per_launch * chunk_sets;
     for (size_t s0 = 0; s0 < batch; s0 += launch_sets) {
         const uint32_t nb = (uint32_t)((batch - s0) < launch_sets ? (batch - s0) : launch_sets);
@@ -485,10 +517,18 @@
         g->pending.push_back(gwb_graph::ChunkEvents{e0, e1, e2});
         HIP_TRY(hipEventRecord(e0, stream));
         void* const out = (char*)d_witness + s0 * (size_t)p.n_witness * 32;
-        HIP_TRY(launch_interp(T, p.divider, waves_per_workgroup(p.divider, (nb + T - 1) / T, p.n_streams), p.n_div_requests, dp->dev.div_lanes, dp->dev, wst, (const char*)d_inputs + s0 * p.n_inputs * 32, d_status + s0, nb, stream, g->d_prof,
-                              out, n_inline, montgomery));
+        const uint32_t wpw = waves_per_workgroup(p.divider, (nb + T - 1) / T, p.n_streams);
+        const int tail = p.divider == 1 && p.n_streams > 1 && wpw == 4 ? tail_mode : (int)kTailOff;
+        HIP_TRY(launch_interp(T, p.divider, wpw, p.n_div_requests, dp->dev.div_lanes, dp->dev, wst, (const char*)d_inputs + s0 * p.n_inputs * 32, d_status + s0, nb, stream, g->d_prof,
+                              out, n_inline, montgomery, tail));
         HIP_TRY(hipEventRecord(e1, stream));
-        HIP_TRY(launch_pack(T, dp->dev, wst, out, nb, stream, montgomery, n_inline));
+        if (tail != kTailOff && dp->dev.tail_rows[tail]) {
+            ProgramDev rest = dp->dev;
+            rest.pack_order = rest.tail_order[tail];
+            HIP_TRY(launch_pack(T, rest, wst, out, nb, stream, montgomery, rest.tail_rows[tail]));
+        } else {
+            HIP_TRY(launch_pack(T, dp->dev, wst, out, nb, stream, montgomery, n_inline));
+        }
         HIP_TRY(hipEventRecord(e2, stream));
         g->last_call_launches++;
         g->timing.n_launches++;
diff --git a/circom-witnesscalc_amd/csrc/program_dev.h b/circom-witnesscalc_amd/csrc/program_dev.h
--- a/circom-witnesscalc_amd/csrc/program_dev.h
+++ b/circom-witnesscalc_amd/csrc/program_dev.h
@@ -91,6 +91,10 @@
     const uint32_t* pack_entries;
     const uint32_t* pack_ready;
     uint32_t n_inline, n_ready_last;
+    const uint32_t* tail_order[2];
+    const uint32_t* tail_entries[2];
+    const uint32_t* tail_table;
+    uint32_t tail_rows[2];
 };
 static const uint32_t PACK_ENTRY_PAD = 192;
 
diff --git a/circom-witnesscalc_amd/csrc/runtime_internal.hpp b/circom-witnesscalc_amd/csrc/runtime_internal.hpp
--- a/circom-witnesscalc_amd/csrc/runtime_internal.hpp
+++ b/circom-witnesscalc_amd/csrc/runtime_internal.hpp
@@ -33,7 +33,7 @@
 namespace cwc {
 hipError_t launch_interp(uint32_t T, uint32_t W, uint32_t pack, uint32_t n_div_requests, const uint32_t* div_lanes, const ProgramDev& p,
                          const WsTable& wst, const void* inputs, uint32_t* status, uint32_t batch, hipStream_t stream, unsigned long long* prof,
-                         void* out = nullptr, uint32_t n_inline = 0, bool montgomery = false);
+                         void* out = nullptr, uint32_t n_inline = 0, bool montgomery = false, int tail = 2);
 hipError_t launch_pack(uint32_t T, const ProgramDev& p, const WsTable& wst, void* out, uint32_t batch, hipStream_t stream, bool montgomery, uint32_t first = 0);
 hipError_t launch_modmul_ubench(uint32_t n_cus, uint32_t waves_per_simd, uint32_t iters, uint32_t* sink, hipStream_t stream, bool block_multiplier);
 hipError_t launch_fill_consts(uint32_t T, const ProgramDev& p, const WsTable& wst, uint32_t n_tiles, hipStream_t stream);
@@ -68,7 +68,12 @@
     std::vector<uint32_t> order;
     std::vector<uint32_t> ready;
     uint32_t n_inline = 0;
+    std::vector<uint32_t> tail_order[2];
+    uint32_t tail_off[2][MAX_STREAMS + 1] = {{0, 0, 0, 0, 0}, {0, 0, 0, 0, 0}};
+    double stream_end[MAX_STREAMS] = {0, 0, 0, 0};
 };
+enum { kTailReplay = 0, kTailAll = 1, kTailOff = 2 };
+int tail_pack_mode();
 std::string make_pack_schedule(const Program& p, PackSchedule& out);
 
 struct DeviceProgram {
diff --git a/include/graph_witness_batch.h b/include/graph_witness_batch.h
--- a/include/graph_witness_batch.h
+++ b/include/graph_witness_batch.h
@@ -133,6 +133,8 @@
                       uint32_t *n_witness, uint32_t *n_ready, uint32_t *n_inline, gw_status_t *status);
 int gwb_pack_schedule_of_blob(const void *blob, size_t blob_len, uint32_t *pack_order, size_t order_cap, uint32_t *pack_ready, size_t ready_cap,
                               uint32_t *n_witness, uint32_t *n_ready, uint32_t *n_inline, gw_status_t *status);
+int gwb_pack_tails(gwb_graph_t *g, uint32_t program_key, int all, uint32_t *order, size_t order_cap, uint32_t *offsets, double *stream_end,
+                   gw_status_t *status);
 
 size_t gwb_wtns_size(size_t n_witness);
 int gwb_wtns_from_witness(const void *witness_row, size_t n_witness, void *out);
```

New measurement: 92000. 1.2% lower.
